# JoelTankard/web-rwkv-gguf

Hardware: AMD Instinct MI355X
Metric: tokens/sec RWKV-7 1.5B Q4_K_M decode @1 GPU; achieved HBM GB/s vs roofline (higher is better)
Workload: dtype f16; 1 GPU; RWKV-7 World 1.5B Q4_K_M (Q4_K matrices, Q6_K head, F16 LoRA) batch=1 greedy decode, fused kernels under hipGraph; decode_engine=on, streams_per_gpu=1, pipelines_per_gpu=1, streams=1, parallelism=single

## Files before the change

web-rwkv-gguf_amd/csrc/wrk_dmv.hip:

```cpp
#include <cstdlib>

#include "wrk_dmv_body.h"

namespace wrk {

template <int KA, int KB, int XI, int KS>
static dmv_fn pick_dmv_pro(bool r16, int pro) {
#define DMV_P(PRO_) (r16 ? (dmv_fn)dmv_kernel<KA, KB, true, XI, KS, PRO_, 1> : (dmv_fn)dmv_kernel<KA, KB, false, XI, KS, PRO_, 1>)
    if (KS == 4 || pro == 0) return DMV_P(0);
    if (pro == 1) return DMV_P(1);
    if (pro == 2) return DMV_P(2);
    if (KA != KB) return nullptr;
    return pro == 3 ? DMV_P(3) : DMV_P(4);
#undef DMV_P
}

template <int XI, int KS>
static dmv_fn pick_dmv_kind(int ka, bool has_f16, bool r16, int pro) {
#define DMV_K(A)                                                                              \
    if (ka == A) return (has_f16 && KS == 1) ? pick_dmv_pro<A, WRK_MAT_F16, XI, KS>(r16, pro) : pick_dmv_pro<A, A, XI, KS>(r16, pro);
    DMV_K(WRK_MAT_Q4_K)
    DMV_K(WRK_MAT_Q5_K)
    DMV_K(WRK_MAT_Q6_K)
    DMV_K(WRK_MAT_Q8_0)
    DMV_K(WRK_MAT_INT8)
#undef DMV_K
    if (ka == WRK_MAT_F16) return pick_dmv_pro<WRK_MAT_F16, WRK_MAT_F16, XI, KS>(false, pro);
    return nullptr;
}

dmvt_fn pick_dmv_nt2(int ka, int quant2, bool has_f16, bool f16_only, uint32_t xi, int ks, int pro);
dmvt_fn pick_dmv_nt4(int ka, int quant2, bool has_f16, bool f16_only, uint32_t xi, int ks, int pro);
dmvt_fn pick_dmv_tokens(int nt, int ka, int quant2, bool has_f16, bool f16_only, uint32_t xi, int ks, int pro) {
    if (nt == 2) return pick_dmv_nt2(ka, quant2, has_f16, f16_only, xi, ks, pro);
    if (nt == 4) return pick_dmv_nt4(ka, quant2, has_f16, f16_only, xi, ks, pro);
    return nullptr;
}

int launch_dmv(hipStream_t s, const MatvecParams& P, uint32_t total_wg, int quant, bool has_f16, bool r16, bool dry, int quant2) {
    static const bool enabled = [] { const char* e = getenv("WRK_DMV"); return !(e && e[0] == '0'); }();
    if (!enabled) return -1;
    DParams D;
    DParamsT DT;
    uint32_t bounds[7], bmask = 0, xi = 1;
    int pro = -1;
    bool small_wg = true;
    for (int j = 0; j < 7; ++j) bounds[j] = 0xffffffffu;
    auto dense_base = [](const DTensor& t) { return ((size_t)t.offset[2] * t.stride[1] + t.offset[1]) * t.stride[0] + t.offset[0]; };
    auto dense_stack = [](const DTensor& t) { return t.shape[2] == 1 || (t.shape[1] == t.stride[1] && t.offset[1] == 0); };
    const uint32_t ntok = P.jobs[0].in.shape[1] * P.jobs[0].in.shape[2];
    if (ntok == 0 || ntok > 4) return -1;
    const int nt = ntok == 1 ? 1 : (ntok <= 2 ? 2 : 4);
    static const uint32_t max_tok = [] { const char* e = getenv("WRK_DMV_TOKENS"); const int v = e ? atoi(e) : 4; return (uint32_t)(v < 1 ? 1 : v); }();
    if (ntok > max_tok) return -1;
    if (nt > 1 && r16) return -1;
    for (int j = 0; j < P.njobs; ++j) {
        const JobDev& J = P.jobs[j];
        if (J.in.dtype != WRK_F16 || (J.k & 7u) || J.in.shape[1] * J.in.shape[2] != ntok || J.kind == WRK_MAT_NF4) return -1;
        if (nt > 1) {
            if (!dense_stack(J.in) || !dense_stack(J.out) || (J.has_res && !dense_stack(J.res)) || (J.in.stride[0] & 7u)) return -1;
            if (J.kind != WRK_MAT_F16 && J.kind != WRK_MAT_Q4_K && J.kind != WRK_MAT_Q5_K && J.kind != WRK_MAT_Q6_K) return -1;
        }
        if ((J.out.dtype != WRK_F16 && J.out.dtype != WRK_F32) || J.m == 0 || J.rows_per_wg == 0) return -1;
        const size_t ib = dense_base(J.in);
        if (ib & 7u) return -1;
        const int jp = J.pro ? (J.k <= 2048 ? 1 : (J.k <= 4096 ? 2 : 9)) + (J.pro == 2 ? 2 : 0) : 0;
        if (jp >= 9 || (pro >= 0 && jp != pro)) return -1;
        if (J.pro == 2 && (J.k & 63u)) return -1;
        pro = jp;
        if (J.rows_per_wg > 32) small_wg = false;
        const uint32_t kpad = (J.k + 15u) & ~15u;
        uint32_t nch, need;
        if (J.kind == WRK_MAT_F16) { nch = kpad >> 3; need = quant < 0 ? (nch + 63) / 64 : (nch + 255) / 256; bmask |= (quant < 0 ? 0u : 1u << j); }
        else { nch = (J.kind == WRK_MAT_Q8_0 || J.kind == WRK_MAT_INT8) ? (J.k >> 4) : (J.k >> 8) * 8; need = (nch + 63) / 64; }
        xi = need > xi ? need : xi;
        const size_t esz = J.out.dtype == WRK_F32 ? 4 : 2;
        if (J.has_res && J.res.dtype != WRK_F16 && J.res.dtype != WRK_F32) return -1;
        auto fill = [&](auto& d) {
            memset(&d, 0, sizeof d);
            d.w = J.w;
            d.x = (const f16*)J.in.p + ib;
            d.out = (char*)J.out.p + dense_base(J.out) * esz;
            d.flags = J.out.dtype == WRK_F32 ? DJ_OUT32 : 0u;
            if (J.has_res) {
                d.res = (const char*)J.res.p + dense_base(J.res) * (J.res.dtype == WRK_F32 ? 4 : 2);
                d.flags |= DJ_RES | (J.res.dtype == WRK_F32 ? DJ_RES32 : 0u);
            }
            if (J.carry_dst) { d.carry_src = J.carry_src; d.carry_dst = J.carry_dst; d.flags |= DJ_CARRY; }
            if (J.gate) { d.gate = J.gate; d.flags |= DJ_GATE; }
            if (J.amax_val) { d.amax_val = J.amax_val; d.amax_idx = J.amax_idx; d.flags |= DJ_AMAX; }
            if (J.pro) { d.ln_w = J.ln_w; d.ln_b = J.ln_b; d.mixw = J.mixw; d.prev = J.prev; d.ln_out = J.ln_out; d.eps = J.pro_eps; if (J.ln_out) d.flags |= DJ_PUBLISH; }
            d.dbg = J.dbg;
            d.k = J.k; d.m = J.m; d.row_bytes = J.row_bytes; d.rows_per_wg = J.rows_per_wg; d.wg_begin = J.wg_begin; d.act = J.act; d.kind = J.kind;
            d.scale = J.scale;
        };
        if (nt == 1) fill(D.jobs[j]);
        else {
            DJobT& dt = DT.jobs[j];
            fill(dt);
            dt.ntok = ntok; dt.xs = J.in.stride[0]; dt.os = J.out.stride[0]; dt.rs = J.has_res ? J.res.stride[0] : 0;
            dt.mix_s = J.tok_mix_stride; dt.prev_s = J.tok_prev_stride; dt.csrc_s = J.tok_carry_src_stride; dt.cdst_s = J.tok_carry_dst_stride; dt.gate_s = J.tok_gate_stride;
        }
        if (j > 0) bounds[j - 1] = J.wg_begin;
    }
    if (xi > 8) return -1;
    static const size_t max_bytes = [] { const char* e = getenv("WRK_DMV_MAXMB"); return (size_t)(e ? atoi(e) : 24) << 20; }();
    size_t launch_bytes = 0;
    for (int j = 0; j < P.njobs; ++j) launch_bytes += (size_t)P.jobs[j].m * P.jobs[j].row_bytes;
    if (nt == 1 && launch_bytes > max_bytes && xi > 1 && pro != 3 && pro != 4) return -1;
    dmv_fn fn = nullptr;
    const int ka = quant < 0 ? WRK_MAT_F16 : quant;
    const bool mixf = has_f16 && quant >= 0;
    if (nt > 1) {
        int ks = 1;
        uint32_t xk = xi;
        if (quant2 < 0 && !(quant < 0 && xi <= 4) && xi > 2) {
            bool amax = false;
            for (int j = 0; j < P.njobs; ++j) amax = amax || P.jobs[j].amax_val;
            if (mixf || !small_wg || pro != 0 || amax || xi > 8) return -1;
            ks = 4; xk = xi <= 4 ? 1 : 2;
        }
        const dmvt_fn ft = pick_dmv_tokens(nt, ka, quant2, mixf, quant < 0, xk, ks, pro);
        if (!ft) return -1;
        if (!dry) hipLaunchKernelGGL(ft, dim3(total_wg, 1), dim3(256), 0, s, bounds[0], bounds[1], bounds[2], bounds[3], bounds[4], bounds[5], bounds[6], bmask, DT);
        return 0;
    }
    else if (quant2 >= 0) {
        const int k4 = quant == WRK_MAT_Q6_K ? quant2 : quant;
        const int lnpro = xi == 1 ? 1 : 2;
        if ((quant != WRK_MAT_Q6_K && quant2 != WRK_MAT_Q6_K) || (k4 != WRK_MAT_Q4_K && k4 != WRK_MAT_Q5_K) || xi > 2 || (pro != 0 && pro != lnpro)) return -1;
#define DMV3X(A, X, PR) (r16 ? (dmv_fn)dmv3_kernel<A, true, X, PR, 1> : (dmv_fn)dmv3_kernel<A, false, X, PR, 1>)
#define DMV3(A) (xi == 1 ? (pro ? DMV3X(A, 1, 1) : DMV3X(A, 1, 0)) : (pro ? DMV3X(A, 2, 2) : DMV3X(A, 2, 0)))
        fn = k4 == WRK_MAT_Q4_K ? DMV3(WRK_MAT_Q4_K) : DMV3(WRK_MAT_Q5_K);
#undef DMV3
#undef DMV3X
    }
    else if (xi == 1) fn = pick_dmv_kind<1, 1>(ka, mixf, r16, pro);
    else if (xi == 2) fn = pick_dmv_kind<2, 1>(ka, mixf, r16, pro);
    else if (quant < 0 && xi <= 4) fn = pick_dmv_kind<4, 1>(ka, false, false, pro);
    else if (!mixf && small_wg && pro == 0) fn = xi <= 4 ? pick_dmv_kind<1, 4>(ka, false, r16, 0) : pick_dmv_kind<2, 4>(ka, false, r16, 0);
    if (!fn) return -1;
    if (!dry) hipLaunchKernelGGL(fn, dim3(total_wg, 1), dim3(256), 0, s, bounds[0], bounds[1], bounds[2], bounds[3], bounds[4], bounds[5], bounds[6], bmask, D);
    return 0;
}

}
```

web-rwkv-gguf_amd/csrc/wrk_dmv_body.h:

```cpp
#pragma once
#include "wrk_matvec_dev.h"

namespace wrk {

enum { DJ_RES = 1, DJ_RES32 = 2, DJ_CARRY = 4, DJ_GATE = 8, DJ_AMAX = 16, DJ_OUT32 = 32, DJ_PUBLISH = 64 };

#define WRK_DJOB_FIELDS                                                                                                          \
    const uint8_t* w;                                                                                                            \
    const f16* x;                                                                    \
    void* out;                                                       \
    const void* res;                                         \
    const f16* carry_src;                                \
    float* carry_dst;                                                                                                            \
    const f16* gate;                                                                       \
    const f16 *ln_w, *ln_b, *mixw;         \
    const float* prev;                                                                                 \
    f16* ln_out;                                      \
    float* amax_val;                                                                             \
    uint32_t* amax_idx;                                                                                                          \
    unsigned long long* dbg;                                                                                                     \
    uint32_t k, m, row_bytes, rows_per_wg, wg_begin, act, flags, kind;                                                           \
    float scale, eps;
struct DJob {
    WRK_DJOB_FIELDS
};
struct DJobT {
    WRK_DJOB_FIELDS
    uint32_t ntok, xs, os, rs, mix_s, prev_s, csrc_s, cdst_s, gate_s;
};

struct DParams {
    DJob jobs[MAX_JOBS];
};
struct DParamsT {
    DJobT jobs[MAX_JOBS];
};
template <int NT> struct DParamsOf { typedef DParamsT type; };
template <> struct DParamsOf<1> { typedef DParams type; };

template <class JT> struct TokF {
    static __device__ __forceinline__ uint32_t ntok(const JT&) { return 1u; }
    static __device__ __forceinline__ uint32_t xs(const JT&) { return 0u; }
    static __device__ __forceinline__ uint32_t os(const JT&) { return 0u; }
    static __device__ __forceinline__ uint32_t rs(const JT&) { return 0u; }
    static __device__ __forceinline__ uint32_t mix_s(const JT&) { return 0u; }
    static __device__ __forceinline__ uint32_t prev_s(const JT&) { return 0u; }
    static __device__ __forceinline__ uint32_t csrc_s(const JT&) { return 0u; }
    static __device__ __forceinline__ uint32_t cdst_s(const JT&) { return 0u; }
    static __device__ __forceinline__ uint32_t gate_s(const JT&) { return 0u; }
};
template <> struct TokF<DJobT> {
    static __device__ __forceinline__ uint32_t ntok(const DJobT& j) { return j.ntok; }
    static __device__ __forceinline__ uint32_t xs(const DJobT& j) { return j.xs; }
    static __device__ __forceinline__ uint32_t os(const DJobT& j) { return j.os; }
    static __device__ __forceinline__ uint32_t rs(const DJobT& j) { return j.rs; }
    static __device__ __forceinline__ uint32_t mix_s(const DJobT& j) { return j.mix_s; }
    static __device__ __forceinline__ uint32_t prev_s(const DJobT& j) { return j.prev_s; }
    static __device__ __forceinline__ uint32_t csrc_s(const DJobT& j) { return j.csrc_s; }
    static __device__ __forceinline__ uint32_t cdst_s(const DJobT& j) { return j.cdst_s; }
    static __device__ __forceinline__ uint32_t gate_s(const DJobT& j) { return j.gate_s; }
};

template <int KIND, bool R16, int NT, int XI>
__device__ __forceinline__ void dot_raw_tokens(const Raw& r, uint32_t c, const XRegs (&x)[NT][XI], int ci, float (&acc)[NT]) {
    if (KIND == WRK_MAT_F16) {
        const f16x8 wv = __builtin_bit_cast(f16x8, r.w);
#pragma unroll
        for (int t = 0; t < NT; ++t) {
            const f16x8 xv = x[t][ci].v[0];
            float a = 0.0f;
            a = __builtin_amdgcn_fdot2(__builtin_shufflevector(wv, wv, 0, 1), __builtin_shufflevector(xv, xv, 0, 1), a, false);
            a = __builtin_amdgcn_fdot2(__builtin_shufflevector(wv, wv, 2, 3), __builtin_shufflevector(xv, xv, 2, 3), a, false);
            a = __builtin_amdgcn_fdot2(__builtin_shufflevector(wv, wv, 4, 5), __builtin_shufflevector(xv, xv, 4, 5), a, false);
            a = __builtin_amdgcn_fdot2(__builtin_shufflevector(wv, wv, 6, 7), __builtin_shufflevector(xv, xv, 6, 7), a, false);
            acc[t] += a;
        }
        return;
    }
    constexpr bool TWO = KIND != WRK_MAT_Q8_0 && KIND != WRK_MAT_INT8;
    Group lo, hi;
    decode_raw<KIND>(r, c, lo, hi);
    if (R16) { round_group(lo); if (TWO) round_group(hi); }
#pragma unroll
    for (int t = 0; t < NT; ++t) {
        const XRegs& X = x[t][ci];
        float a;
        if (R16) a = dot16r(lo.q, X.v[0], X.v[1]);
        else a = lo.scale * (lo.qmul * dot16r(lo.q, X.v[0], X.v[1]) - lo.off * X.s[0]) - lo.minv * X.s[0];
        if (TWO) {
            if (R16) a += dot16r(hi.q, X.v[2], X.v[3]);
            else a += hi.scale * (hi.qmul * dot16r(hi.q, X.v[2], X.v[3]) - hi.off * X.s[1]) - hi.minv * X.s[1];
        }
        acc[t] += a;
    }
}

template <int KIND, bool R16, int XI, int KS, int PRO, int NT, class JT>
__device__ __forceinline__ void dmv_body(const JT J, unsigned char* smem) {
    typedef TokF<JT> TF;
    constexpr int RB = 4;
    constexpr uint32_t CSTEP = KS == 1 ? 64u : 256u;
    const uint32_t K = J.k, kpad = (K + 15u) & ~15u;
    const uint32_t tid = threadIdx.x, lane = tid & 63;
    const uint32_t wave = (uint32_t)__builtin_amdgcn_readfirstlane((int)(tid >> 6));
    const uint32_t r0 = (blockIdx.x - J.wg_begin) * J.rows_per_wg;
    const uint32_t r1 = min(r0 + J.rows_per_wg, J.m);
    const uint32_t nch = num_chunks<KIND>(K, kpad);
    const uint32_t nrows = KS == 1 ? (r0 + wave < r1 ? (r1 - r0 - wave + 3) >> 2 : 0) : (r1 - r0);
    const uint32_t cbase = KS == 1 ? lane : lane + 64 * wave;
    const uint32_t ntok = NT == 1 ? 1u : TF::ntok(J);
    auto row_of = [&](uint32_t ri) { return KS == 1 ? r0 + wave + 4 * ri : r0 + ri; };
    auto tok_of = [&](uint32_t t) { return NT == 1 ? 0u : min(t, ntok - 1); };
    const uint8_t* __restrict__ W = J.w;
    const uint32_t RBY = J.row_bytes;
    float* part = (float*)smem;
    float* sv = (float*)(smem + 512 * NT);
    uint32_t* si = (uint32_t*)(smem + 528 * NT);
    float* red = (float*)(smem + 544 * NT);
    f16* xs = (f16*)(smem + 576 * NT);

    Raw raw[RB][XI];
    auto issue = [&](uint32_t ri0) {
#pragma unroll
        for (int rb = 0; rb < RB; ++rb) {
            const uint32_t rr = min(row_of(ri0 + rb), r1 - 1);
            const uint32_t phase = KIND == WRK_MAT_INT8 ? (uint32_t)((((size_t)rr * K) >> 4) & 7u) : 0u;
            const uint8_t* rowp = W + (size_t)rr * RBY;
#pragma unroll
            for (int ci = 0; ci < XI; ++ci) raw[rb][ci] = load_raw<KIND>(rowp, K, min(cbase + CSTEP * ci, nch - 1), phase);
        }
    };
    WRK_STAMP(J.dbg, 0);

    const f16* __restrict__ xin = J.x;
    const uint32_t fin_row = min(KS == 1 ? row_of(lane & 3u) : r0 + (tid & 31u), r1 - 1);
    const uint32_t fin_t = NT == 1 ? 0u : (KS == 1 ? (lane >> 2) : (tid >> 5));
    const uint32_t fin_tok = tok_of(fin_t);
    const uint32_t fl = J.flags;
    uint32_t res_bits = 0, carry_bits = 0, gate_bits = 0;
    constexpr int VPT = PRO == 0 ? 1 : ((PRO - 1) % 2 + 1);
    constexpr bool GN = PRO >= 3;
    f16x8 xv[NT][VPT], wv[VPT], bv[VPT], mv[GN ? NT : 1][VPT];
    f32x4 pv[NT][VPT][2];
    f16 c0h[NT];
    XRegs x[NT][XI];
    if (PRO > 0) {
        const uint32_t nvec = K >> 3;
#pragma unroll
        for (int v = 0; v < VPT; ++v) {
            const uint32_t i = min(tid + 256u * v, nvec - 1);
            wv[v] = *(const f16x8*)(J.ln_w + i * 8);
            bv[v] = *(const f16x8*)(J.ln_b + i * 8);
#pragma unroll
            for (int t = 0; t < NT; ++t) {
                const uint32_t tt = tok_of(t);
                xv[t][v] = *(const f16x8*)(xin + (size_t)tt * TF::xs(J) + i * 8);
                if (GN || t == 0) mv[GN ? t : 0][v] = *(const f16x8*)(J.mixw + (size_t)tt * TF::mix_s(J) + i * 8);
                pv[t][v][0] = *(const f32x4*)(J.prev + (size_t)tt * TF::prev_s(J) + i * 8);
                pv[t][v][1] = *(const f32x4*)(J.prev + (size_t)tt * TF::prev_s(J) + i * 8 + 4);
            }
        }
        if (!GN) {
#pragma unroll
            for (int t = 0; t < NT; ++t) c0h[t] = xin[(size_t)tok_of(t) * TF::xs(J)];
        }
    } else {
#pragma unroll
        for (int t = 0; t < NT; ++t)
#pragma unroll
            for (int ci = 0; ci < XI; ++ci) x[t][ci] = load_x<KIND>(xin + (size_t)tok_of(t) * TF::xs(J), min(cbase + CSTEP * ci, nch - 1), true);
    }
    issue(0);
    {
        const bool has_res = (fl & DJ_RES) != 0, has_carry = (fl & DJ_CARRY) != 0, has_gate = (fl & DJ_GATE) != 0;
        const uint16_t* rp = has_res ? (const uint16_t*)J.res : (const uint16_t*)xin;
        const uint32_t re = fin_tok * TF::rs(J) + fin_row;
        const uint32_t ri = has_res ? ((fl & DJ_RES32) ? 2u * re : re) : 0u;
        if (fl & DJ_RES32) res_bits = *(const uint32_t*)(rp + ri);
        else res_bits = rp[ri];
        carry_bits = (has_carry ? (const uint16_t*)J.carry_src : (const uint16_t*)xin)[has_carry ? fin_tok * TF::csrc_s(J) + fin_row : 0u];
        gate_bits = (has_gate ? (const uint16_t*)J.gate : (const uint16_t*)xin)[has_gate ? fin_tok * TF::gate_s(J) + fin_row : 0u];
    }

    if (GN) {
        const uint32_t nvec = K >> 3;
#pragma unroll
        for (int t = 0; t < NT; ++t)
#pragma unroll
            for (int v = 0; v < VPT; ++v) {
                float y[8], s1 = 0.0f;
#pragma unroll
                for (int e = 0; e < 8; ++e) { y[e] = (float)xv[t][v][e]; s1 += y[e]; }
                s1 += dpp_f32<0xB1>(s1); s1 += dpp_f32<0x4E>(s1); s1 += dpp_f32<0x141>(s1);
                const float mean = s1 * (1.0f / 64.0f);
                float s2 = 0.0f;
#pragma unroll
                for (int e = 0; e < 8; ++e) { y[e] -= mean; s2 = __builtin_fmaf(y[e], y[e], s2); }
                s2 += dpp_f32<0xB1>(s2); s2 += dpp_f32<0x4E>(s2); s2 += dpp_f32<0x141>(s2);
                const float dev = 1.0f / sqrtf(s2 * (1.0f / 64.0f) + J.eps);
                f16x8 o;
#pragma unroll
                for (int e = 0; e < 8; ++e) {
                    float u = r16(__builtin_fmaf(y[e] * dev, (float)wv[v][e], (float)bv[v][e]));
                    u = r16(u + pv[t][v][e >> 2][e & 3]);
                    o[e] = (f16)((float)mv[GN ? t : 0][v][e] * u);
                }
                const uint32_t i = tid + 256u * v;
                if (i < nvec) *(f16x8*)(xs + (size_t)t * kpad + i * 8) = o;
            }
        for (uint32_t i = K + tid; i < kpad; i += 256)
#pragma unroll
            for (int t = 0; t < NT; ++t) xs[(size_t)t * kpad + i] = (f16)0.0f;
        __syncthreads();
#pragma unroll
        for (int t = 0; t < NT; ++t)
#pragma unroll
            for (int ci = 0; ci < XI; ++ci) x[t][ci] = load_x<KIND>(xs + (size_t)t * kpad, min(cbase + CSTEP * ci, nch - 1), true);
    }
    if (PRO > 0 && !GN) {
        const uint32_t nvec = K >> 3;
        float s1[NT], s2[NT];
#pragma unroll
        for (int t = 0; t < NT; ++t) {
            const float c0 = (float)c0h[t];
            s1[t] = 0.0f; s2[t] = 0.0f;
#pragma unroll
            for (int v = 0; v < VPT; ++v)
                if (tid + 256u * v < nvec)
#pragma unroll
                    for (int e = 0; e < 8; ++e) { const float dl = (float)xv[t][v][e] - c0; s1[t] += dl; s2[t] = __builtin_fmaf(dl, dl, s2[t]); }
            s1[t] = wave_sum(s1[t]);
            s2[t] = wave_sum(s2[t]);
            if (lane == 0) { red[8 * t + wave] = s1[t]; red[8 * t + 4 + wave] = s2[t]; }
        }
        __syncthreads();
        WRK_STAMP(J.dbg, 4);
        const bool publish = (fl & DJ_PUBLISH) && blockIdx.x == J.wg_begin;
#pragma unroll
        for (int t = 0; t < NT; ++t) {
            const float c0 = (float)c0h[t];
            const float a1 = (red[8 * t + 0] + red[8 * t + 1]) + (red[8 * t + 2] + red[8 * t + 3]);
            const float a2 = (red[8 * t + 4] + red[8 * t + 5]) + (red[8 * t + 6] + red[8 * t + 7]);
            const float md = a1 / (float)K;
            const float mean = c0 + md;
            const float dev = 1.0f / sqrtf(fmaxf(a2 / (float)K - md * md, 0.0f) + J.eps);
#pragma unroll
            for (int v = 0; v < VPT; ++v) {
                const uint32_t i = tid + 256u * v;
                if (i >= nvec) continue;
                f16x8 yv, o;
#pragma unroll
                for (int e = 0; e < 8; ++e) {
                    yv[e] = (f16)__builtin_fmaf(((float)xv[t][v][e] - mean) * dev, (float)wv[v][e], (float)bv[v][e]);
                    o[e] = (f16)wgsl_mix((float)yv[e], pv[t][v][e >> 2][e & 3], (float)mv[0][v][e]);
                }
                *(f16x8*)(xs + (size_t)t * kpad + i * 8) = o;
                if (publish && (uint32_t)t < ntok) *(f16x8*)(J.ln_out + (size_t)t * K + i * 8) = yv;
            }
        }
        for (uint32_t i = K + tid; i < kpad; i += 256)
#pragma unroll
            for (int t = 0; t < NT; ++t) xs[(size_t)t * kpad + i] = (f16)0.0f;
        __syncthreads();
#pragma unroll
        for (int t = 0; t < NT; ++t)
#pragma unroll
            for (int ci = 0; ci < XI; ++ci) x[t][ci] = load_x<KIND>(xs + (size_t)t * kpad, min(cbase + CSTEP * ci, nch - 1), true);
    }
#pragma unroll
    for (int ci = 0; ci < XI; ++ci)
        if (cbase + CSTEP * ci >= nch) {
            const f16x8 z = {0, 0, 0, 0, 0, 0, 0, 0};
#pragma unroll
            for (int t = 0; t < NT; ++t) x[t][ci].v[0] = x[t][ci].v[1] = x[t][ci].v[2] = x[t][ci].v[3] = z;
        }
#pragma unroll
    for (int t = 0; t < NT; ++t)
#pragma unroll
        for (int ci = 0; ci < XI; ++ci) x_sums<KIND>(x[t][ci]);
    WRK_STAMP(J.dbg, 1);

    float best_v = -3.0e38f;
    uint32_t best_i = 0xffffffffu;
    auto finish = [&](uint32_t r, uint32_t tok, float v, uint32_t rbits, uint32_t cbits, uint32_t gbits) {
        float o = act_apply(J.act, v * J.scale);
        const bool o32 = (fl & DJ_OUT32) != 0;
        if (fl & DJ_GATE) o = act_sigmoid(f16bits_to_f32(gbits)) * (o32 ? o : r16(o));
        if (fl & DJ_RES) o = (o32 ? o : r16(o)) + ((fl & DJ_RES32) ? __builtin_bit_cast(float, rbits) : f16bits_to_f32(rbits));
        const size_t oo = (size_t)tok * TF::os(J) + r;
        if (o32) ((float*)J.out)[oo] = o; else ((f16*)J.out)[oo] = (f16)o;
        if (fl & DJ_CARRY) J.carry_dst[(size_t)tok * TF::cdst_s(J) + r] = f16bits_to_f32(cbits);
        if (o > best_v || (o == best_v && r < best_i)) { best_v = o; best_i = r; }
    };
    auto operand_bits = [&](uint32_t r, uint32_t tok, uint32_t& rbits, uint32_t& cbits, uint32_t& gbits) {
        if (fl & DJ_RES) rbits = (fl & DJ_RES32) ? ((const uint32_t*)J.res)[(size_t)tok * TF::rs(J) + r] : (uint32_t)((const uint16_t*)J.res)[(size_t)tok * TF::rs(J) + r];
        if (fl & DJ_CARRY) cbits = ((const uint16_t*)J.carry_src)[(size_t)tok * TF::csrc_s(J) + r];
        if (fl & DJ_GATE) gbits = ((const uint16_t*)J.gate)[(size_t)tok * TF::gate_s(J) + r];
    };
    for (uint32_t ri0 = 0; ri0 < nrows; ri0 += RB) {
        if (ri0 != 0) issue(ri0);
        float acc[RB][NT];
#pragma unroll
        for (int rb = 0; rb < RB; ++rb) {
#pragma unroll
            for (int t = 0; t < NT; ++t) acc[rb][t] = 0.0f;
#pragma unroll
            for (int ci = 0; ci < XI; ++ci) dot_raw_tokens<KIND, R16, NT, XI>(raw[rb][ci], min(cbase + CSTEP * ci, nch - 1), x, ci, acc[rb]);
        }
        WRK_STAMP(J.dbg, 2);
        float mine_v = 0.0f;
#pragma unroll
        for (int t = 0; t < NT; ++t)
#pragma unroll
            for (int rb = 0; rb < RB; ++rb) {
                const float v = wave_sum(acc[rb][t]);
                if (lane == (uint32_t)(rb + RB * t)) mine_v = v;
            }
        const uint32_t frb = lane & 3u;
        if (KS == 1) {
            if (lane < (uint32_t)(RB * NT) && (NT == 1 || fin_t < ntok) && ri0 + frb < nrows) {
                const uint32_t r = row_of(ri0 + frb);
                uint32_t rbits = res_bits, cbits = carry_bits, gbits = gate_bits;
                if (ri0 != 0) operand_bits(r, fin_t, rbits, cbits, gbits);
                finish(r, fin_t, mine_v, rbits, cbits, gbits);
            }
        } else if (lane < (uint32_t)(RB * NT) && ri0 + frb < nrows) part[(((NT == 1 ? 0u : lane >> 2) * 32u) + ri0 + frb) * 4 + wave] = mine_v;
    }
    if (KS == 4) {
        __syncthreads();
        const uint32_t ri = tid & 31u;
        if (NT == 1 ? tid < nrows : (ri < nrows && fin_t < ntok)) {
            const uint32_t p = NT == 1 ? tid : (fin_t * 32u + ri);
            finish(r0 + ri, fin_t, (part[p * 4] + part[p * 4 + 1]) + (part[p * 4 + 2] + part[p * 4 + 3]), res_bits, carry_bits, gate_bits);
        }
    }
    WRK_STAMP(J.dbg, 3);
    if (fl & DJ_AMAX) {
#pragma unroll
        for (int o = (KS == 1 ? 2 : 32); o > 0; o >>= 1) {
            const float ov = __shfl_xor(best_v, o, WAVE);
            const uint32_t oi = __shfl_xor(best_i, o, WAVE);
            if (ov > best_v || (ov == best_v && oi < best_i)) { best_v = ov; best_i = oi; }
        }
        if (KS == 1 ? ((lane & 3u) == 0 && lane < 4u * NT) : lane == 0) { sv[4 * (KS == 1 ? lane >> 2 : 0) + wave] = best_v; si[4 * (KS == 1 ? lane >> 2 : 0) + wave] = best_i; }
        __syncthreads();
        if (tid < ntok) {
            float bv2 = sv[4 * tid];
            uint32_t bi = si[4 * tid];
            for (int w = 1; w < 4; ++w)
                if (sv[4 * tid + w] > bv2 || (sv[4 * tid + w] == bv2 && si[4 * tid + w] < bi)) { bv2 = sv[4 * tid + w]; bi = si[4 * tid + w]; }
            J.amax_val[(size_t)(blockIdx.x - J.wg_begin) * ntok + tid] = bv2;
            J.amax_idx[(size_t)(blockIdx.x - J.wg_begin) * ntok + tid] = bi;
        }
    }
}

template <int PRO, int NT>
constexpr unsigned dmv_smem_bytes() { return 576u * NT + (PRO > 0 ? (unsigned)((PRO - 1) % 2 + 1) * 4096u * NT : 16u); }

template <int KA, int KB, bool R16, int XI, int KS, int PRO, int NT>
__global__ void __launch_bounds__(256) dmv_kernel(uint32_t b1, uint32_t b2, uint32_t b3, uint32_t b4, uint32_t b5, uint32_t b6, uint32_t b7,
                                                  uint32_t kind_b_mask, const typename DParamsOf<NT>::type P) {
    __shared__ __attribute__((aligned(16))) unsigned char smem[dmv_smem_bytes<PRO, NT>()];
    const uint32_t b = blockIdx.x;
    const uint32_t ji = (b >= b1) + (b >= b2) + (b >= b3) + (b >= b4) + (b >= b5) + (b >= b6) + (b >= b7);
    const auto J = P.jobs[ji];
    if (KA == KB || !((kind_b_mask >> ji) & 1u)) dmv_body<KA, (KA != WRK_MAT_F16) && R16, XI, KS, PRO, NT>(J, smem);
    else dmv_body<KB, (KB != WRK_MAT_F16) && R16, (KB == WRK_MAT_F16 ? 4 * XI : XI), 1, PRO, NT>(J, smem);
}

template <int KA, bool R16, int XI, int PRO, int NT>
__global__ void __launch_bounds__(256) dmv3_kernel(uint32_t b1, uint32_t b2, uint32_t b3, uint32_t b4, uint32_t b5, uint32_t b6, uint32_t b7,
                                                   uint32_t, const typename DParamsOf<NT>::type P) {
    __shared__ __attribute__((aligned(16))) unsigned char smem[dmv_smem_bytes<PRO, NT>()];
    const uint32_t b = blockIdx.x;
    const uint32_t ji = (b >= b1) + (b >= b2) + (b >= b3) + (b >= b4) + (b >= b5) + (b >= b6) + (b >= b7);
    const auto J = P.jobs[ji];
    if (J.kind == (uint32_t)KA) dmv_body<KA, R16, XI, 1, PRO, NT>(J, smem);
    else if (J.kind == WRK_MAT_Q6_K) dmv_body<WRK_MAT_Q6_K, R16, XI, 1, PRO, NT>(J, smem);
    else dmv_body<WRK_MAT_F16, false, 4 * XI, 1, PRO, NT>(J, smem);
}

typedef void (*dmv_fn)(uint32_t, uint32_t, uint32_t, uint32_t, uint32_t, uint32_t, uint32_t, uint32_t, const DParams);
typedef void (*dmvt_fn)(uint32_t, uint32_t, uint32_t, uint32_t, uint32_t, uint32_t, uint32_t, uint32_t, const DParamsT);

dmvt_fn pick_dmv_tokens(int nt, int ka, int quant2, bool has_f16, bool f16_only, uint32_t xi, int ks, int pro);

}
```

web-rwkv-gguf_amd/csrc/wrk_internal.h:

```cpp
#pragma once
#include <hip/hip_runtime.h>

#include <atomic>
#include <cmath>
#include <cstdarg>
#include <cstdio>
#include <cstring>
#include <map>
#include <mutex>
#include <string>
#include <thread>
#include <vector>

#include "wrk_hip.h"

struct wrk_ctx {
    int device = 0;
    hipStream_t stream = nullptr;
    hipStream_t read_stream = nullptr;
    hipEvent_t read_event = nullptr;
    std::recursive_mutex mu;
    std::string err;
    std::map<std::thread::id, hipStream_t> sessions;
    std::vector<hipStream_t> capture_pool;
// ... 125 lines not shown
void group_norm(hipStream_t s, const void* w, const void* b, DTensor x, float eps);
void l2_norm(hipStream_t s, DTensor x, float eps);
void token_shift(hipStream_t s, const uint32_t* cursors, DTensor mix, DTensor state, DTensor in, DTensor out, int reversed);
void pre_wkv_v7(hipStream_t s, void* w, void* a, void* k, void* v, void* vv, void* v0, void* n, const void* w0, const void* a0, const void* k_k,
                const void* k_a, const void* v0p, uint32_t D, uint32_t T, bool first_layer, float l2_eps, float* wdec = nullptr);
void post_wkv_v7(hipStream_t s, void* x, const void* r, const void* g, const void* n, const void* gn_w, const void* gn_b, const void* r_k,
                 uint32_t D, uint32_t T, float gn_eps);
void token_shift_multi(hipStream_t s, const uint32_t* cursors, const DTensor* mix, const DTensor* out, int n, DTensor state, DTensor in, int reversed);
void transpose(hipStream_t s, DTensor in, DTensor out);
void time_mix_v6(hipStream_t s, const uint32_t* cursors, DTensor decay, const void* u_f32, DTensor state, DTensor k, DTensor v, DTensor r, DTensor x,
                 uint32_t nseq_hint = 0);
void channel_mix_v6(hipStream_t s, const uint32_t* cursors, DTensor state, DTensor r, DTensor v, DTensor x);
void binary(hipStream_t s, int is_mul, DTensor in, DTensor out, uint32_t ax, uint32_t ay, uint32_t ao);
void lerp(hipStream_t s, DTensor x, DTensor y, DTensor f, int reversed);
void blit(hipStream_t s, DTensor in, DTensor out);
void affine(hipStream_t s, DTensor x, float scale, float bias);
void activate(hipStream_t s, DTensor x, uint32_t act);
void control_k_v7(hipStream_t s, const void* p, DTensor a, DTensor k);
void time_mix_v7(hipStream_t s, const uint32_t* cursors, DTensor state, DTensor r, DTensor w, DTensor n, DTensor x, uint32_t nseq_hint = 0, const float* wdec = nullptr);
void time_first_v7(hipStream_t s, const void* u, DTensor r, DTensor n, DTensor x);
void channel_mix_v7(hipStream_t s, const uint32_t* cursors, DTensor state, DTensor v, DTensor x);
void softmax(hipStream_t s, DTensor x);
void gather_rows_f16(hipStream_t s, const void* table, const uint32_t* ids, void* out, uint32_t d, uint32_t n);
void gather_rows_any(hipStream_t s, DTensor in, const uint32_t* rows, DTensor out, uint32_t n);
void argmax_rows(hipStream_t s, const float* logits, uint32_t v, uint32_t v_stride, uint32_t n, uint32_t* out);

struct SampleParam { float temperature, top_p; uint32_t seed, step_base; };
static constexpr uint32_t SAMPLE_MAX_VOCAB = 1u << 20;
struct RowGate { const uint32_t* flag; uint32_t stride, eq; };
struct SampleFilter { uint32_t top_k; float ln_min_p; };
struct SampleAlt { float tau, eta, mu, typical_p; };
enum : int { SAMPLE_PLAIN = 0, SAMPLE_FILT = 1, SAMPLE_MIRO = 2, SAMPLE_TYP = 3 };
struct SamplePick { int mode; const SampleParam* par; const SampleFilter* filt; SampleAlt* alt; RowGate gate; };
int sample_rows(hipStream_t s, const float* logits, uint32_t v, uint32_t stride, uint32_t n, const SamplePick& pick, const uint32_t* step,
                uint32_t* out);

struct ScorePart { float m, s; uint32_t gt, eq; };
static constexpr uint32_t SCORE_MAX_SLICES = 32;
uint32_t score_slices(uint32_t n, uint32_t v, int num_cu);
int score_rows(hipStream_t s, const float* logits, uint32_t v, uint32_t stride, uint32_t n, const uint32_t* targets, ScorePart* part,
               float* logprob, uint32_t* rank, int num_cu);

static constexpr uint32_t LOGPROB_MAX_TOP = WRK_MAX_TOP_LOGPROBS;
struct LogprobParam { float* logprob; uint32_t* top_ids; float* top_logprobs; uint32_t num_top, cap_rows; };
struct LogprobPart { float m, s; };
inline size_t logprob_part_bytes(uint32_t n) { return (size_t)n * SCORE_MAX_SLICES * sizeof(LogprobPart); }
inline size_t logprob_key_bytes(uint32_t n) { return (size_t)n * SCORE_MAX_SLICES * 4 * LOGPROB_MAX_TOP * 8; }
int logprob_rows(hipStream_t s, const float* logits, uint32_t v, uint32_t stride, uint32_t n, const uint32_t* tokens, const uint32_t* step,
                 const LogprobParam* par, LogprobPart* part, unsigned long long* keys, int num_cu);

struct PenaltyParam { float* count; uint8_t* flags; const float* weight; float presence, frequency, decay; uint32_t pad; };
void penalize_rows(hipStream_t s, const float* src, uint32_t v, uint32_t src_stride, uint32_t n, const PenaltyParam* par, float* dst,
                   uint32_t dst_stride);
void occurrence_update(hipStream_t s, uint32_t v, uint32_t n, const PenaltyParam* par, const uint32_t* tokens, uint32_t ntok, const RowGate& gate);

struct GrammarParam { const uint16_t* token_class; const uint16_t* transitions; uint32_t num_classes, pad; uint32_t* states; };
void constrain_rows(hipStream_t s, const float* src, uint32_t v, uint32_t src_stride, uint32_t n, const GrammarParam* par, float* dst,
                    uint32_t dst_stride);
void grammar_advance(hipStream_t s, uint32_t v, uint32_t n, const GrammarParam* par, const uint32_t* tokens, const RowGate& gate);

struct StopParam { uint32_t ids[WRK_MAX_STOP_TOKENS]; uint32_t count, done, length, end_token; };
struct StopGeom {
    float *state, *head_o, *snap_state, *snap_logits;
    const uint32_t* just_ended; const StopParam* par; const uint32_t* counter; uint32_t* lengths;
    uint32_t layers, num_batch, b0, v;
    size_t slot;
};
void advance_stop(hipStream_t s, const uint32_t* drawn, uint32_t* tokens, uint32_t* history, uint32_t* counter, StopParam* par,
                  uint32_t* just_ended, uint32_t* live, uint32_t b);
void stop_snapshot(hipStream_t s, const StopGeom& g, uint32_t b, int num_cu);
void stop_restore(hipStream_t s, const StopGeom& g, uint32_t b, int num_cu);

struct StopSeqRow { uint32_t count, pad[3]; uint32_t len[WRK_MAX_STOP_SEQUENCES]; uint32_t tok[WRK_MAX_STOP_SEQUENCES][WRK_MAX_STOP_SEQUENCE_LEN]; };
struct StopSeqBufs { const StopSeqRow* rows; uint32_t* tail; uint32_t* match; };
void advance_stop_seq(hipStream_t s, const uint32_t* drawn, uint32_t* tokens, uint32_t* history, uint32_t* counter, StopParam* par,
                      uint32_t* just_ended, uint32_t* live, const StopSeqBufs& q, uint32_t b);
void stop_seq_rows(hipStream_t s, uint32_t n, const StopSeqRow* rows, const StopParam* ids, uint32_t* tail, const uint32_t* tokens, uint32_t* match);

enum : uint32_t { QUEUE_IDLE = 0, QUEUE_PROMPT = 1, QUEUE_REPLY = 2 };
struct QueueReq {
    uint32_t prompt_off, prompt_len, max_new, seed;
    float temperature, top_p, presence, frequency, decay;
    uint32_t stop_count, stop_ids[WRK_MAX_STOP_TOKENS];
    uint32_t top_k; float ln_min_p;
    float tau, eta, typical_p;
};
struct QueueSlot { uint32_t req, pos, reply, phase; };
struct QueueLog { uint32_t length, reason, slot, start_step; };
struct QueueCtl { uint32_t next_request, num_requests, live, pad; const float* init_state; };
struct QueueBufs {
    QueueSlot* slots; const QueueReq* reqs; const uint32_t* pool; QueueLog* log; QueueCtl* ctl;
    uint32_t* started;
    SampleParam* sample_par;
    PenaltyParam* pen_par;
    SampleFilter* filter_par;
    SampleAlt* alt_par = nullptr;
    float* alt_mu = nullptr;
    uint32_t* gram_state = nullptr;
    uint32_t* gram_req = nullptr;
    const StopSeqRow* seq_rows = nullptr;
    uint32_t* seq_tail = nullptr;
    uint32_t* seq_match = nullptr;
};
void advance_queue(hipStream_t s, const uint32_t* drawn, uint32_t* tokens, uint32_t* history, uint32_t* counter, const QueueBufs& q, uint32_t b);
struct QueueGeom { float* state; uint32_t layers, num_batch, b0, v; size_t slot; };
void queue_reset(hipStream_t s, const QueueGeom& g, const QueueBufs& q, uint32_t b, int num_cu);
static constexpr uint32_t QUEUE_NO_ENTRY = 0xFFFFFFFFu;
struct QueueStateCtl { float* states; uint32_t num_entries, turn_count; };
struct QueueTurn { uint32_t slot, save, started, start; };
struct QueueStateBufs {
    const uint32_t *start, *save;
    QueueStateCtl* sctl;
    QueueTurn* turn;
};
void advance_queue_pool(hipStream_t s, const uint32_t* drawn, uint32_t* tokens, uint32_t* history, uint32_t* counter, const QueueBufs& q,
                        const QueueStateBufs& p, uint32_t b);
void queue_turnover(hipStream_t s, const QueueGeom& g, const QueueBufs& q, const QueueStateBufs& p, uint32_t b, int num_cu);

unsigned long long* timing_slot(wrk_ctx* ctx, const char* label);
void timing_report(wrk_ctx* ctx);

struct MatJob {
    const uint8_t* w;
    const uint8_t* aux;
    uint32_t kind, flags;
    uint32_t k, m;
    uint32_t row_bytes;
    DTensor in;
    DTensor out;
    uint32_t act;
    uint32_t sparse;
    uint32_t has_res = 0;
    DTensor res{};
    float* amax_val = nullptr;
    uint32_t* amax_idx = nullptr;
    uint32_t pro = 0;
    float pro_eps = 0.0f;
    const void *ln_w = nullptr, *ln_b = nullptr, *mixw = nullptr;
    const float* prev = nullptr;
    void* ln_out = nullptr;
    const void* carry_src = nullptr;
    float* carry_dst = nullptr;
    float scale = 1.0f;
    const void* gate = nullptr;
    unsigned long long* dbg = nullptr;
    uint32_t tok_prev_stride = 0, tok_mix_stride = 0, tok_carry_src_stride = 0, tok_carry_dst_stride = 0, tok_gate_stride = 0;
    float* ks_part = nullptr;
    uint32_t* ks_cnt = nullptr;
    size_t ks_part_cap = 0;
    uint32_t ks_cnt_cap = 0;
    void* xsum = nullptr;
    size_t xsum_cap = 0;
};
uint32_t matvec_num_wg(const MatJob* jobs, int njobs, int num_cu, uint32_t* rows_per_wg);
int matvec(hipStream_t s, const MatJob* jobs, int njobs, int num_cu, bool dry_run = false, bool no_catchall = false, bool dmv_only = false);
int matvec_grouped(hipStream_t s, const MatJob* jobs, int njobs, int num_cu, bool dry_run = false);
int matmul_mfma(hipStream_t s, const MatJob& job, int num_cu);
int matmul_mfma_multi(hipStream_t s, const MatJob* jobs, int njobs, int num_cu);
uint32_t gemm_min_tokens();
void quantize_int8(hipStream_t s, const void* src_f16, uint8_t* dst, uint32_t k, uint32_t m, uint32_t row_bytes);
void quantize_nf4(hipStream_t s, const void* src_f16, const float* levels, uint8_t* dst, uint32_t k, uint32_t m, uint32_t row_bytes);
size_t repack_row_bytes(uint32_t kind, uint32_t k);
uint32_t int8_row_blocks(uint32_t k);
int repack_rows(uint32_t kind, uint32_t k, uint32_t m, const uint8_t* src, uint8_t* dst);
size_t stored_bytes(uint32_t kind, uint32_t k, uint32_t m);

}

int32_t wrk_sample_pack(wrk_ctx* ctx, const float* temperature, const float* top_p, const uint32_t* seed, uint32_t n,
                        std::vector<wrk::SampleParam>& out);
int32_t wrk_filter_pack(wrk_ctx* ctx, const uint32_t* top_k, const float* min_p, uint32_t n, std::vector<wrk::SampleFilter>& out);
int32_t wrk_mirostat_pack(wrk_ctx* ctx, const float* tau, const float* eta, const float* mu, uint32_t n, std::vector<wrk::SampleAlt>& out);
int32_t wrk_typical_pack(wrk_ctx* ctx, const float* typical_p, uint32_t n, std::vector<wrk::SampleAlt>& out);

struct wrk_score_scratch {
    void* buf = nullptr;
    uint32_t cap = 0;
    uint32_t* targets = nullptr;
    float* logprob = nullptr;
    uint32_t* rank = nullptr;
    wrk::ScorePart* part = nullptr;
    int32_t ensure(wrk_ctx* ctx, uint32_t n, bool* grown);
    void release();
};
int32_t wrk_score_check_targets(wrk_ctx* ctx, const uint32_t* targets, uint32_t n, uint32_t V);

struct wrk_occurrence {
    wrk_ctx* ctx = nullptr;
    uint32_t num_batch = 0, num_vocab = 0;
    void* mem = nullptr;
    float* counts = nullptr;
    float* weights = nullptr;
    uint8_t* flags = nullptr;
    wrk::PenaltyParam row(uint32_t slot, float presence, float frequency, float decay) const;
};
int32_t wrk_penalty_pack(wrk_ctx* ctx, const wrk_occurrence* occ, uint32_t first, uint32_t n, uint32_t V, const float* presence,
                         const float* frequency, const float* decay, std::vector<wrk::PenaltyParam>& out);

struct wrk_grammar {
    wrk_ctx* ctx = nullptr;
    uint32_t num_vocab = 0, num_states = 0, num_classes = 0;
    void* mem = nullptr;
    uint16_t* token_class = nullptr;
    uint16_t* transitions = nullptr;
    wrk::GrammarParam param(uint32_t* states) const;
};
int32_t wrk_grammar_pack(wrk_ctx* ctx, const wrk_grammar* g, const uint32_t* state, uint32_t n, uint32_t V, std::vector<uint32_t>& out);
```

web-rwkv-gguf_amd/csrc/wrk_matvec.hip:

```cpp
#include <algorithm>
#include <cstdlib>

#include "wrk_matvec_dev.h"

namespace wrk {

static inline size_t align16(size_t x) { return (x + 15) & ~(size_t)15; }

uint32_t int8_row_blocks(uint32_t k) { return (k % 128) ? k / 128 + 2 : k / 128; }

size_t repack_row_bytes(uint32_t kind, uint32_t k) {
    const size_t nb = k / 256;
    switch (kind) {
        case WRK_MAT_F16: return align16((size_t)k * 2);
        case WRK_MAT_Q8_0: return align16((size_t)k + (size_t)(k / 32) * 2);
        case WRK_MAT_Q4_K: return align16(nb * 148);
        case WRK_MAT_Q5_K: return align16(nb * 180);
        case WRK_MAT_Q6_K: return align16(nb * 208 + nb * 2);
        case WRK_MAT_INT8: return (k % 16) ? 0 : align16((size_t)k + (size_t)int8_row_blocks(k) * 4);
        case WRK_MAT_NF4: return (k % 64) ? 0 : align16((size_t)k / 2 + (size_t)(k / 64) * 2);
        default: return 0;
    }
}

// ... 516 lines not shown

typedef void (*matvec_fn)(const MatvecParams);

template <int NB, int KA, int KB>
static matvec_fn pick_r16(bool r16) {
    return r16 ? (matvec_fn)matvec_kernel<NB, KA, KB, true> : (matvec_fn)matvec_kernel<NB, KA, KB, false>;
}

template <int NB>
static matvec_fn pick_kernel(int ka, int kb, bool r16) {
#define PAIR(A)                                                                     \
    if (ka == A) return kb == A ? pick_r16<NB, A, A>(r16) : pick_r16<NB, A, WRK_MAT_F16>(r16);
    PAIR(WRK_MAT_Q4_K)
    PAIR(WRK_MAT_Q5_K)
    PAIR(WRK_MAT_Q6_K)
    PAIR(WRK_MAT_Q8_0)
#undef PAIR
    if (ka == WRK_MAT_NF4) return kb == ka ? (matvec_fn)matvec_kernel<NB, WRK_MAT_NF4, WRK_MAT_NF4, false> : (matvec_fn)matvec_kernel<NB, WRK_MAT_NF4, WRK_MAT_F16, false>;
    if (ka == WRK_MAT_INT8) return kb == ka ? (matvec_fn)matvec_kernel<NB, WRK_MAT_INT8, WRK_MAT_INT8, false> : (matvec_fn)matvec_kernel<NB, WRK_MAT_INT8, WRK_MAT_F16, false>;
    if (ka == WRK_MAT_F16) return pick_r16<NB, WRK_MAT_F16, WRK_MAT_F16>(false);
    return (matvec_fn)matvec_kernel<NB, -1, -1, false>;
}

template <int KA, int KB, int XI, int KS>
static matvec_fn pick_reg_r16(bool r16) {
    return r16 ? (matvec_fn)matvec_reg_kernel<KA, KB, true, XI, KS> : (matvec_fn)matvec_reg_kernel<KA, KB, false, XI, KS>;
}

template <int XI, int KS>
static matvec_fn pick_reg_kernel(int ka, int kb, bool r16) {
#define PAIR(A)                                                                     \
    if (ka == A) return (kb == A || KS == 4) ? pick_reg_r16<A, A, XI, KS>(r16) : pick_reg_r16<A, WRK_MAT_F16, XI, 1>(r16);
    PAIR(WRK_MAT_Q4_K)
    PAIR(WRK_MAT_Q5_K)
    PAIR(WRK_MAT_Q6_K)
    PAIR(WRK_MAT_Q8_0)
    PAIR(WRK_MAT_INT8)
#undef PAIR
    return nullptr;
}

static matvec_fn pick_reg(const MatvecParams& P, int quant, bool has_f16, bool r16, int quant2 = -1) {
    uint32_t xi = 1;
    for (int j = 0; j < P.njobs; ++j) {
        const JobDev& J = P.jobs[j];
        if (J.in.dtype != WRK_F16 || (J.k & 7u) || J.in.shape[1] * J.in.shape[2] != 1) return nullptr;
        if (J.pro && J.k > 4096) return nullptr;
        if (J.pro == 2) return nullptr;
        const size_t base = ((size_t)J.in.offset[2] * J.in.stride[1] + J.in.offset[1]) * J.in.stride[0] + J.in.offset[0];
        if (base & 7u) return nullptr;
        const uint32_t kpad = (J.k + 15u) & ~15u;
        uint32_t nch, need;
        if (J.kind == WRK_MAT_F16) { nch = kpad >> 3; need = quant < 0 ? (nch + 63) / 64 : (nch + 255) / 256; }
        else if (J.kind == WRK_MAT_NF4) return nullptr;
        else { nch = (J.kind == WRK_MAT_Q8_0 || J.kind == WRK_MAT_INT8) ? (J.k >> 4) : (J.k >> 8) * 8; need = (nch + 63) / 64; }
        xi = need > xi ? need : xi;
    }
    if (xi > 8) return nullptr;
    bool small_wg = true;
    for (int j = 0; j < P.njobs; ++j) if (P.jobs[j].rows_per_wg > 32) small_wg = false;
    if (quant < 0) {
        if (xi == 1) return (matvec_fn)matvec_reg_kernel<WRK_MAT_F16, WRK_MAT_F16, false, 1, 1>;
        if (xi == 2) return (matvec_fn)matvec_reg_kernel<WRK_MAT_F16, WRK_MAT_F16, false, 2, 1>;
        if (xi <= 4) return (matvec_fn)matvec_reg_kernel<WRK_MAT_F16, WRK_MAT_F16, false, 4, 1>;
        return small_wg ? (matvec_fn)matvec_reg_kernel<WRK_MAT_F16, WRK_MAT_F16, false, 2, 4> : nullptr;
    }
    if (quant2 >= 0) {
        const int ka = quant == WRK_MAT_Q6_K ? quant2 : quant;
        if ((quant != WRK_MAT_Q6_K && quant2 != WRK_MAT_Q6_K) || (ka != WRK_MAT_Q4_K && ka != WRK_MAT_Q5_K) || xi > 2) return nullptr;
        if (ka == WRK_MAT_Q4_K) {
            if (xi == 1) return r16 ? (matvec_fn)matvec_reg3_kernel<WRK_MAT_Q4_K, true, 1> : (matvec_fn)matvec_reg3_kernel<WRK_MAT_Q4_K, false, 1>;
            return r16 ? (matvec_fn)matvec_reg3_kernel<WRK_MAT_Q4_K, true, 2> : (matvec_fn)matvec_reg3_kernel<WRK_MAT_Q4_K, false, 2>;
        }
        if (xi == 1) return r16 ? (matvec_fn)matvec_reg3_kernel<WRK_MAT_Q5_K, true, 1> : (matvec_fn)matvec_reg3_kernel<WRK_MAT_Q5_K, false, 1>;
        return r16 ? (matvec_fn)matvec_reg3_kernel<WRK_MAT_Q5_K, true, 2> : (matvec_fn)matvec_reg3_kernel<WRK_MAT_Q5_K, false, 2>;
    }
    const int kb = has_f16 ? WRK_MAT_F16 : quant;
    if (xi == 1) return pick_reg_kernel<1, 1>(quant, kb, r16);
    if (xi == 2) return pick_reg_kernel<2, 1>(quant, kb, r16);
    if (has_f16 || !small_wg) return nullptr;
    if (xi <= 4) return pick_reg_kernel<1, 4>(quant, quant, r16);
    return pick_reg_kernel<2, 4>(quant, quant, r16);
}

struct KindMix { int quant = -1, quant2 = -1, nquant = 0; bool has_f16 = false, r16 = false, mixed_r16 = false; };
static KindMix classify_kinds(const MatvecParams& P) {
    KindMix c;
    for (int j = 0; j < P.njobs; ++j) {
        const int k = (int)P.jobs[j].kind;
        if (k == WRK_MAT_F16) { c.has_f16 = true; continue; }
        const bool jr = (P.jobs[j].flags & WRK_MATRIX_ROUND_F16) != 0;
        if (c.nquant == 0) { c.quant = k; c.r16 = jr; c.nquant = 1; }
        else {
            if (k != c.quant && k != c.quant2) { c.quant2 = c.quant2 < 0 ? k : c.quant2; c.nquant = (k == c.quant2) ? 2 : 3; }
            if (jr != c.r16) c.mixed_r16 = true;
        }
    }
    return c;
}

template <int NB>
static int launch_matvec(hipStream_t s, const MatvecParams& P, uint32_t total_wg, uint32_t tok_groups, size_t smem, bool dry, bool no_catchall) {
    const KindMix c = classify_kinds(P);
    const int quant = c.quant, quant2 = c.quant2, nquant = c.nquant;
    const bool has_f16 = c.has_f16, r16 = c.r16, mixed_r16 = c.mixed_r16;
    matvec_fn fn = nullptr;
    bool needs_reg = false;
    for (int j = 0; j < P.njobs; ++j) needs_reg = needs_reg || P.jobs[j].pro || P.jobs[j].carry_dst || P.jobs[j].gate;
    if (NB == 1 && tok_groups == 1 && nquant <= 2 && !mixed_r16 && launch_dmv(s, P, total_wg, nquant ? quant : -1, has_f16, r16, dry, nquant == 2 ? quant2 : -1) == 0) return 0;
    if (NB == 1 && tok_groups == 1 && nquant <= 2 && !mixed_r16) {
        fn = pick_reg(P, nquant ? quant : -1, has_f16, r16, nquant == 2 ? quant2 : -1);
        if (fn) {
            if (!dry) hipLaunchKernelGGL(fn, dim3(total_wg, 1), dim3(256), 0, s, P);
            return 0;
        }
    }
    if (needs_reg) return -3;
    if (no_catchall && (nquant >= 2 || mixed_r16)) return -4;
    if (dry) return 0;
    if (nquant >= 2 || mixed_r16) fn = (matvec_fn)matvec_kernel<NB, -1, -1, false>;
    else if (nquant == 0) fn = pick_kernel<NB>(WRK_MAT_F16, WRK_MAT_F16, false);
    else fn = pick_kernel<NB>(quant, has_f16 ? WRK_MAT_F16 : quant, r16);
    if (smem > 64 * 1024) {
        if (hipFuncSetAttribute((const void*)fn, hipFuncAttributeMaxDynamicSharedMemorySize, (int)smem) != hipSuccess) return -1;
    }
    hipLaunchKernelGGL(fn, dim3(total_wg, tok_groups), dim3(256), smem, s, P);
    return 0;
}

static uint32_t matvec_job_rpw(const MatJob* jobs, int njobs, int j, uint32_t rpw) {
    uint32_t min_rb = jobs[0].row_bytes;
    for (int q = 1; q < njobs; ++q) min_rb = jobs[q].row_bytes < min_rb ? jobs[q].row_bytes : min_rb;
    uint32_t r = (uint32_t)((uint64_t)rpw * min_rb / (jobs[j].row_bytes ? jobs[j].row_bytes : 1)) & ~3u;
    return r < 4 ? 4 : r;
}

uint32_t matvec_num_wg(const MatJob* jobs, int njobs, int num_cu, uint32_t* rows_per_wg) {
    uint32_t total_rows = 0;
    for (int j = 0; j < njobs; ++j) total_rows += jobs[j].m;
    static const uint32_t per_cu = [] { const char* e = getenv("WRK_WG_PER_CU"); const int v = e ? atoi(e) : 4; return (uint32_t)(v < 1 ? 1 : (v > 16 ? 16 : v)); }();
    uint32_t rpw = (total_rows + (uint32_t)num_cu * per_cu - 1) / ((uint32_t)num_cu * per_cu);
    rpw = (rpw + 3) & ~3u;
    static const uint32_t rpw_min = [] { const char* e = getenv("WRK_RPW_MIN"); const int v = e ? atoi(e) : 4; return (uint32_t)(v < 4 ? 4 : (v > 32 ? 32 : v)) & ~3u; }();
    rpw = rpw < rpw_min ? rpw_min : (rpw > 32 ? 32 : rpw);
    static const uint32_t pro_rpw = [] { const char* e = getenv("WRK_PRO_RPW"); const int v = e ? atoi(e) : 16; return (uint32_t)(v < 4 ? 4 : (v > 32 ? 32 : v)) & ~3u; }();
    for (int j = 0; j < njobs; ++j)
        if (jobs[j].pro && rpw < pro_rpw) rpw = pro_rpw;
    uint32_t wg = 0;
    for (int j = 0; j < njobs; ++j) { const uint32_t r = matvec_job_rpw(jobs, njobs, j, rpw); wg += (jobs[j].m + r - 1) / r; }
    if (rows_per_wg) *rows_per_wg = rpw;
    return wg;
}

int matvec(hipStream_t s, const MatJob* jobs, int njobs, int num_cu, bool dry_run, bool no_catchall, bool dmv_only) {
    if (njobs <= 0 || njobs > MAX_JOBS) return -1;
    MatvecParams P;
    P.njobs = njobs;
    const uint32_t ntok = jobs[0].in.shape[1] * jobs[0].in.shape[2];
    if (ntok == 0) return 0;
    uint32_t kmax = 0;
    for (int j = 0; j < njobs; ++j) {
        if (jobs[j].in.shape[1] * jobs[j].in.shape[2] != ntok) return -1;
        kmax = jobs[j].k > kmax ? jobs[j].k : kmax;
    }
    uint32_t rpw = 4;
    matvec_num_wg(jobs, njobs, num_cu, &rpw);
    uint32_t wg = 0;
    for (int j = 0; j < njobs; ++j) {
        JobDev& d = P.jobs[j];
        d.w = jobs[j].w; d.aux = (const float*)jobs[j].aux; d.kind = jobs[j].kind; d.flags = jobs[j].flags; d.k = jobs[j].k; d.m = jobs[j].m;
        d.row_bytes = jobs[j].row_bytes; d.act = jobs[j].act; d.rows_per_wg = matvec_job_rpw(jobs, njobs, j, rpw); d.wg_begin = wg;
        d.in = jobs[j].in; d.out = jobs[j].out; d.res = jobs[j].res; d.has_res = jobs[j].has_res;
        d.amax_val = jobs[j].amax_val; d.amax_idx = jobs[j].amax_idx;
        d.pro = jobs[j].pro; d.pro_eps = jobs[j].pro_eps; d.ln_w = (const f16*)jobs[j].ln_w; d.ln_b = (const f16*)jobs[j].ln_b;
        d.mixw = (const f16*)jobs[j].mixw; d.prev = jobs[j].prev; d.ln_out = (f16*)jobs[j].ln_out;
        d.carry_src = (const f16*)jobs[j].carry_src; d.carry_dst = jobs[j].carry_dst; d.gate = (const f16*)jobs[j].gate; d.scale = jobs[j].scale; d.dbg = jobs[j].dbg;
        d.tok_prev_stride = jobs[j].tok_prev_stride; d.tok_mix_stride = jobs[j].tok_mix_stride; d.tok_carry_src_stride = jobs[j].tok_carry_src_stride;
        d.tok_carry_dst_stride = jobs[j].tok_carry_dst_stride; d.tok_gate_stride = jobs[j].tok_gate_stride;
        wg += (jobs[j].m + d.rows_per_wg - 1) / d.rows_per_wg;
    }
    bool f32in = false;
    for (int j = 0; j < njobs; ++j) f32in = f32in || jobs[j].in.dtype == WRK_F32;
    if (f32in) {
        for (int j = 0; j < njobs; ++j)
            if (jobs[j].pro || jobs[j].carry_dst || jobs[j].gate || jobs[j].amax_val) return -3;
        if (dry_run) return 0;
        hipLaunchKernelGGL(matvec_f32in_kernel, dim3(wg, ntok), dim3(256), 0, s, P);
        return 0;
    }
    if (ntok >= 2 && ntok <= 4) {
        const KindMix c = classify_kinds(P);
        if (c.nquant <= 2 && !c.mixed_r16 && launch_dmv(s, P, wg, c.nquant ? c.quant : -1, c.has_f16, c.r16, dry_run, c.nquant == 2 ? c.quant2 : -1) == 0) return 0;
    }
    if (dmv_only && ntok > 1) return -5;
    const uint32_t kpad = (kmax + 15u) & ~15u;
    int nb = ntok >= 8 ? 8 : (ntok >= 4 ? 4 : (ntok >= 2 ? 2 : 1));
    while (nb > 1 && (size_t)nb * kpad * 2 + (size_t)nb * (kpad >> 4) * 4 > 144 * 1024) nb >>= 1;
    size_t smem = (size_t)nb * kpad * 2 + (size_t)nb * (kpad >> 4) * 4 + 64;
    if (smem < 256) smem = 256;
    const uint32_t groups = (ntok + nb - 1) / nb;
    int rc;
    switch (nb) {
        case 8: rc = launch_matvec<8>(s, P, wg, groups, smem, dry_run, no_catchall); break;
        case 4: rc = launch_matvec<4>(s, P, wg, groups, smem, dry_run, no_catchall); break;
        case 2: rc = launch_matvec<2>(s, P, wg, groups, smem, dry_run, no_catchall); break;
        default: rc = launch_matvec<1>(s, P, wg, groups, smem, dry_run, no_catchall); break;
    }
    return rc;
}

int matvec_grouped(hipStream_t s, const MatJob* jobs, int njobs, int num_cu, bool dry_run) {
    if (njobs <= 0 || njobs > MAX_JOBS) return -1;
    uint32_t kinds[MAX_JOBS];
    int nk = 0;
    for (int j = 0; j < njobs; ++j) {
        if (jobs[j].kind == WRK_MAT_F16) continue;
        bool seen = false;
        for (int q = 0; q < nk; ++q) seen = seen || kinds[q] == jobs[j].kind;
        if (!seen) kinds[nk++] = jobs[j].kind;
    }
    if (nk <= 1) return matvec(s, jobs, njobs, num_cu, dry_run);
    {
        const int rc = matvec(s, jobs, njobs, num_cu, dry_run, true);
        if (rc == 0) return 0;
    }
    for (int q = 0; q < nk; ++q) {
        MatJob g[MAX_JOBS];
        int n = 0;
        for (int j = 0; j < njobs; ++j)
            if (jobs[j].kind == kinds[q] || (q == 0 && jobs[j].kind == WRK_MAT_F16)) g[n++] = jobs[j];
        const int rc = matvec(s, g, n, num_cu, dry_run);
        if (rc != 0) return rc;
    }
    return 0;
}

}
```

web-rwkv-gguf_amd/csrc/wrk_matvec_dev.h:

```cpp
#pragma once
#include "wrk_device.h"

namespace wrk {

__device__ __forceinline__ void bytes_to_h2(uint32_t v, f16x2& lo, f16x2& hi) {
    lo = __builtin_bit_cast(f16x2, __builtin_amdgcn_perm(0u, v, 0x0c010c00u));
    hi = __builtin_bit_cast(f16x2, __builtin_amdgcn_perm(0u, v, 0x0c030c02u));
}

__device__ __forceinline__ f16x2 h2(float a) { f16x2 r = {(f16)a, (f16)a}; return r; }

__device__ __forceinline__ float dot16(const f16x2 (&q)[8], const f16* __restrict__ x) {
    const f16x8 xa = *(const f16x8*)x;
    const f16x8 xb = *(const f16x8*)(x + 8);
    float acc = 0.0f;
    acc = __builtin_amdgcn_fdot2(q[0], __builtin_shufflevector(xa, xa, 0, 1), acc, false);
    acc = __builtin_amdgcn_fdot2(q[1], __builtin_shufflevector(xa, xa, 2, 3), acc, false);
    acc = __builtin_amdgcn_fdot2(q[2], __builtin_shufflevector(xa, xa, 4, 5), acc, false);
    acc = __builtin_amdgcn_fdot2(q[3], __builtin_shufflevector(xa, xa, 6, 7), acc, false);
    acc = __builtin_amdgcn_fdot2(q[4], __builtin_shufflevector(xb, xb, 0, 1), acc, false);
    acc = __builtin_amdgcn_fdot2(q[5], __builtin_shufflevector(xb, xb, 2, 3), acc, false);
    acc = __builtin_amdgcn_fdot2(q[6], __builtin_shufflevector(xb, xb, 4, 5), acc, false);
    acc = __builtin_amdgcn_fdot2(q[7], __builtin_shufflevector(xb, xb, 6, 7), acc, false);
    return acc;
// ... 175 lines not shown
        const uint32_t s0 = 2 * j, s1 = 2 * j + 1;
        const uint32_t r0 = (s0 + 28u) & 31u, r1 = (s1 + 28u) & 31u;
#define Q5LO(W, H) (((W) & 0x0f0f0f0fu) | (__builtin_amdgcn_alignbit((H), (H), r0) & 0x10101010u))
#define Q5HI(W, H) ((((W) >> 4) & 0x0f0f0f0fu) | (__builtin_amdgcn_alignbit((H), (H), r1) & 0x10101010u))
        bytes_to_h2(Q5LO(w.x, qh.x), lo.q[0], lo.q[1]);
        bytes_to_h2(Q5LO(w.y, qh.y), lo.q[2], lo.q[3]);
        bytes_to_h2(Q5LO(w.z, qh.z), lo.q[4], lo.q[5]);
        bytes_to_h2(Q5LO(w.w, qh.w), lo.q[6], lo.q[7]);
        bytes_to_h2(Q5HI(w.x, qh.x), hi.q[0], hi.q[1]);
        bytes_to_h2(Q5HI(w.y, qh.y), hi.q[2], hi.q[3]);
        bytes_to_h2(Q5HI(w.z, qh.z), hi.q[4], hi.q[5]);
        bytes_to_h2(Q5HI(w.w, qh.w), hi.q[6], hi.q[7]);
#undef Q5LO
#undef Q5HI
        hi.qmul = Q24;
    }
    lo.scale = d * sc0; lo.minv = dmin * m0; lo.off = 0.0f; lo.qmul = Q24; lo.xoff = b * 256 + j * 64 + h * 16;
    hi.scale = d * sc1; hi.minv = dmin * m1; hi.off = 0.0f; hi.xoff = lo.xoff + 32;
}

template <int KIND>
__device__ __forceinline__ void chunk_xoff(uint32_t c, uint32_t& lo, uint32_t& hi) {
    if (KIND == WRK_MAT_F16) { lo = c * 8; hi = lo; return; }
    if (KIND == WRK_MAT_Q8_0 || KIND == WRK_MAT_INT8) { lo = c * 16; hi = lo; return; }
    if (KIND == WRK_MAT_NF4) { lo = c * 32; hi = lo + 16; return; }
    const uint32_t b = c >> 3, sub = c & 7u;
    if (KIND == WRK_MAT_Q6_K) { lo = b * 256 + (sub >> 2) * 128 + ((sub >> 1) & 1u) * 32 + (sub & 1u) * 16; hi = lo + 64; return; }
    lo = b * 256 + (sub >> 1) * 64 + (sub & 1u) * 16;
    hi = lo + 32;
}

template <int KIND, bool R16, int NB>
__device__ __forceinline__ void dot_raw(const Raw& r, uint32_t c, const f16* xs, const float* xsum, uint32_t kpad, float (&acc)[NB],
                                        const float* __restrict__ levels = nullptr) {
    if (KIND == WRK_MAT_F16) {
        const f16x8 wv = __builtin_bit_cast(f16x8, r.w);
#pragma unroll
        for (int n = 0; n < NB; ++n) {
            const f16x8 x = *(const f16x8*)(xs + (size_t)n * kpad + c * 8);
            float a = acc[n];
            a = __builtin_amdgcn_fdot2(__builtin_shufflevector(wv, wv, 0, 1), __builtin_shufflevector(x, x, 0, 1), a, false);
            a = __builtin_amdgcn_fdot2(__builtin_shufflevector(wv, wv, 2, 3), __builtin_shufflevector(x, x, 2, 3), a, false);
            a = __builtin_amdgcn_fdot2(__builtin_shufflevector(wv, wv, 4, 5), __builtin_shufflevector(x, x, 4, 5), a, false);
            a = __builtin_amdgcn_fdot2(__builtin_shufflevector(wv, wv, 6, 7), __builtin_shufflevector(x, x, 6, 7), a, false);
            acc[n] = a;
        }
        return;
    }
    if (KIND == WRK_MAT_NF4) {
        const float amax = f16bits_to_f32(r.a.x);
        const uint32_t wd[4] = {r.w.x, r.w.y, r.w.z, r.w.w};
#pragma unroll
        for (int wi = 0; wi < 4; ++wi) {
            float wv[8];
#pragma unroll
            for (int i = 0; i < 8; ++i) {
                wv[i] = levels[(wd[wi] >> (4 * i)) & 15u] * amax;
                if (R16) wv[i] = (float)(f16)wv[i];
            }
#pragma unroll
            for (int n = 0; n < NB; ++n) {
                const f16x8 x = *(const f16x8*)(xs + (size_t)n * kpad + c * 32 + wi * 8);
                float a = acc[n];
#pragma unroll
                for (int i = 0; i < 8; ++i) a = fmaf(wv[i], (float)x[i], a);
                acc[n] = a;
            }
        }
        return;
    }
    Group lo, hi;
    decode_raw<KIND>(r, c, lo, hi);
    groups_accumulate<R16, NB>(lo, hi, KIND != WRK_MAT_Q8_0 && KIND != WRK_MAT_INT8, xs, xsum, kpad, acc);
}

struct XRegs {
    f16x8 v[4];
    float s[2];
};

__device__ __forceinline__ float sum8(f16x8 a) {
    const f16x2 one = {(f16)1.0f, (f16)1.0f};
    float s = 0.0f;
    s = __builtin_amdgcn_fdot2(__builtin_shufflevector(a, a, 0, 1), one, s, false);
    s = __builtin_amdgcn_fdot2(__builtin_shufflevector(a, a, 2, 3), one, s, false);
    s = __builtin_amdgcn_fdot2(__builtin_shufflevector(a, a, 4, 5), one, s, false);
    s = __builtin_amdgcn_fdot2(__builtin_shufflevector(a, a, 6, 7), one, s, false);
    return s;
}

template <int KIND>
__device__ __forceinline__ XRegs load_x(const f16* __restrict__ x, uint32_t c, bool valid) {
    XRegs r;
    const f16x8 z = {0, 0, 0, 0, 0, 0, 0, 0};
    r.v[0] = r.v[1] = r.v[2] = r.v[3] = z;
    r.s[0] = r.s[1] = 0.0f;
    if (!valid) return r;
    uint32_t lo, hi;
    chunk_xoff<KIND>(c, lo, hi);
    r.v[0] = *(const f16x8*)(x + lo);
    if (KIND != WRK_MAT_F16) r.v[1] = *(const f16x8*)(x + lo + 8);
    if (KIND != WRK_MAT_F16 && KIND != WRK_MAT_Q8_0 && KIND != WRK_MAT_INT8) { r.v[2] = *(const f16x8*)(x + hi); r.v[3] = *(const f16x8*)(x + hi + 8); }
    return r;
}

template <int KIND>
__device__ __forceinline__ void x_sums(XRegs& r) {
    if (KIND != WRK_MAT_F16) r.s[0] = sum8(r.v[0]) + sum8(r.v[1]);
    if (KIND != WRK_MAT_F16 && KIND != WRK_MAT_Q8_0 && KIND != WRK_MAT_INT8) r.s[1] = sum8(r.v[2]) + sum8(r.v[3]);
}

__device__ __forceinline__ float dot16r(const f16x2 (&q)[8], const f16x8 xa, const f16x8 xb) {
    float acc = 0.0f;
    acc = __builtin_amdgcn_fdot2(q[0], __builtin_shufflevector(xa, xa, 0, 1), acc, false);
    acc = __builtin_amdgcn_fdot2(q[1], __builtin_shufflevector(xa, xa, 2, 3), acc, false);
    acc = __builtin_amdgcn_fdot2(q[2], __builtin_shufflevector(xa, xa, 4, 5), acc, false);
    acc = __builtin_amdgcn_fdot2(q[3], __builtin_shufflevector(xa, xa, 6, 7), acc, false);
    acc = __builtin_amdgcn_fdot2(q[4], __builtin_shufflevector(xb, xb, 0, 1), acc, false);
    acc = __builtin_amdgcn_fdot2(q[5], __builtin_shufflevector(xb, xb, 2, 3), acc, false);
    acc = __builtin_amdgcn_fdot2(q[6], __builtin_shufflevector(xb, xb, 4, 5), acc, false);
    acc = __builtin_amdgcn_fdot2(q[7], __builtin_shufflevector(xb, xb, 6, 7), acc, false);
    return acc;
}

template <bool R16>
__device__ __forceinline__ float group_dot_r(Group& g, const f16x8 xa, const f16x8 xb, float xs16) {
    if (R16) {
        round_group(g);
        return dot16r(g.q, xa, xb);
    }
    return g.scale * (g.qmul * dot16r(g.q, xa, xb) - g.off * xs16) - g.minv * xs16;
}

template <int KIND, bool R16>
__device__ __forceinline__ float dot_raw_reg(const Raw& r, uint32_t c, const XRegs& x) {
    if (KIND == WRK_MAT_F16) {
        const f16x8 wv = __builtin_bit_cast(f16x8, r.w);
        float a = 0.0f;
        a = __builtin_amdgcn_fdot2(__builtin_shufflevector(wv, wv, 0, 1), __builtin_shufflevector(x.v[0], x.v[0], 0, 1), a, false);
        a = __builtin_amdgcn_fdot2(__builtin_shufflevector(wv, wv, 2, 3), __builtin_shufflevector(x.v[0], x.v[0], 2, 3), a, false);
        a = __builtin_amdgcn_fdot2(__builtin_shufflevector(wv, wv, 4, 5), __builtin_shufflevector(x.v[0], x.v[0], 4, 5), a, false);
        a = __builtin_amdgcn_fdot2(__builtin_shufflevector(wv, wv, 6, 7), __builtin_shufflevector(x.v[0], x.v[0], 6, 7), a, false);
        return a;
    }
    Group lo, hi;
    decode_raw<KIND>(r, c, lo, hi);
    float a = group_dot_r<R16>(lo, x.v[0], x.v[1], x.s[0]);
    if (KIND != WRK_MAT_Q8_0 && KIND != WRK_MAT_INT8) a += group_dot_r<R16>(hi, x.v[2], x.v[3], x.s[1]);
    return a;
}


int launch_dmv(hipStream_t s, const MatvecParams& P, uint32_t total_wg, int quant, bool has_f16, bool r16, bool dry, int quant2 = -1);

}
```

web-rwkv-gguf_amd/csrc/wrk_v7.h:

```cpp
#pragma once
#include <string>
#include <vector>

#include "wrk_runner.h"

struct V7Scratch : wrk::FrameIo {
    void *input, *x, *att_x, *att_v0, *rx, *wx, *kx, *vx, *ax, *gx, *r, *w, *k, *v, *a, *g, *o, *kk, *vv, *n;
    void *aux_w, *aux_a, *aux_g, *aux_v, *ffn_x, *ffn_kx, *ffn_k, *ffn_v, *ln_tmp, *head_x;
    float* ks_part; uint32_t* ks_cnt; size_t ks_part_cap; uint32_t ks_cnt_cap;
};

struct wrk_v7_model : wrk_frame_common {
    wrk_v7_model_desc d{};
    std::vector<wrk_v7_layer_desc> layers;
    const wrk_buf *ln0_w = nullptr, *ln0_b = nullptr, *ln_out_w = nullptr, *ln_out_b = nullptr, *emb = nullptr;
    const wrk_matrix* head = nullptr;

    V7Scratch s{};

    float* amax_val = nullptr;
    uint32_t* amax_idx = nullptr;
    size_t amax_cap = 0;

    uint32_t layer_begin = 0, layer_end = 0xffffffffu;
    bool skip_embed = false;
    uint32_t act_dtype = WRK_F16;

    std::vector<wrk_v7_model*> lanes;

    struct wrk_v7_engine* engine = nullptr;
    bool engine_tried = false;
    bool engine_skip_once = false;
    bool engine_blocked = false;
    std::string engine_why;
    int32_t ensure_engine();
    bool engine_on() const;
    Facts facts() const override { return {d.num_vocab, d.num_emb, d.num_layer, emb != nullptr}; }
    wrk::FrameIo& io() override { return s; }
    int32_t ensure_frame(uint32_t B, uint32_t mode) override;
    int32_t enqueue_step(wrk_v7_state* st, uint32_t b0, uint32_t B, uint32_t mode, wrk_step_kind kind) override;
    uint32_t key_bits(uint32_t B, uint32_t mode) const override;
    uint32_t max_lanes() const override { return 255; }
    int32_t lane(uint32_t g, uint32_t groups, wrk_frame_common** out) override;
    void before_loop() override;
    int32_t after_loop(uint32_t groups) override;
    int32_t ensure_scratch(uint32_t T, uint32_t NH);
    int32_t enqueue_ops(wrk_v7_state* st, uint32_t T, uint32_t NH, bool identity_headers, bool merged = false);
    int32_t enqueue_fused_decode(wrk_v7_state* st, uint32_t B, uint32_t NH, bool identity_headers, bool from_tokens,
                                 bool want_argmax, bool advance, uint32_t cursor0_batch, bool contiguous);
    void free_fused();
};

bool split_head_env_on();
bool engine_env_on_public();
```

web-rwkv-gguf_amd/csrc/wrk_v7.hip:

```cpp
#include "wrk_internal.h"
#include "wrk_v7.h"
#include "wrk_v7_engine.h"

#define LOCK(ctx) std::lock_guard<std::recursive_mutex> _lk((ctx)->mu)

static constexpr float LN_EPS = 1.0e-5f;
static constexpr float GN_EPS = 64.0e-5f;
static constexpr float L2_EPS = 1.0e-12f;

using wrk::mat_job;

int32_t wrk_v7_model::ensure_scratch(uint32_t T, uint32_t NH) {
    if (T <= scratch_tokens && NH <= scratch_headers && scratch) return WRK_OK;
    if (ctx->capturing_here()) return wrk_fail(ctx, WRK_E_ARG, "scratch must be sized before capture");
    const uint32_t nt = T > scratch_tokens ? T : scratch_tokens;
    const uint32_t nh = NH > scratch_headers ? NH : scratch_headers;
    WRK_HIP(ctx, hipStreamSynchronize(ctx->stream));
    drop_graphs();
    if (scratch) hipFree(scratch);
    scratch = nullptr;
    const size_t D = d.num_emb, F = d.num_hidden, V = d.num_vocab;
    size_t off = 0;
    auto take = [&](size_t bytes) { size_t o = off; off += wrk_up256(bytes); return o; };
    const size_t esz = act_dtype == WRK_F32 ? 4 : 2;
    const size_t vecT = D * nt * esz;
    size_t o_named[32];
    int ni = 0;
    for (int i = 0; i < 23; ++i) o_named[ni++] = take(vecT);
    const size_t o_n = take(vecT * 4);
    const size_t o_auxw = take((size_t)d.lora_w * nt * esz), o_auxa = take((size_t)d.lora_a * nt * esz);
    const size_t o_auxg = take((size_t)d.lora_g * nt * esz), o_auxv = take((size_t)d.lora_v * nt * esz);
    const size_t o_ffnk = take(F * nt * esz);
    const size_t o_headx = take(D * nh * esz), o_heado = take(V * nh * 4);
    const size_t o_cur = take((size_t)nt * 4), o_tok = take((size_t)nt * 4), o_hdr = take((size_t)nh * 4), o_arg = take((size_t)nh * 4);
    const size_t o_cnt = take(256);
    size_t ks_floats = 0, ks_groups = 0, o_ksp = 0, o_ksc = 0;
    if (nt >= 2 && act_dtype == WRK_F16) {
        const size_t ntp = nt <= 16 ? 16 : (nt <= 32 ? 32 : 64);
        auto tiles = [](size_t m, size_t k) { return ((m + 63) / 64) * (k / 256 ? k / 256 : 1); };
        auto groups = [](size_t m) { return (m + 63) / 64; };
        const size_t lora = tiles(d.lora_w, D) + tiles(d.lora_a, D) + tiles(d.lora_g, D) + tiles(d.lora_v, D);
        const size_t k1 = 3 * tiles(D, D) + lora, k5 = tiles(F, D), k6 = tiles(D, F);
        const size_t most = k1 > k5 ? (k1 > k6 ? k1 : k6) : (k5 > k6 ? k5 : k6);
        ks_floats = most * 64 * ntp;
        ks_groups = 3 * groups(D) + groups(d.lora_w) + groups(d.lora_a) + groups(d.lora_g) + groups(d.lora_v) + groups(F) + 8;
        o_ksp = take(ks_floats * 4);
        o_ksc = take(ks_groups * 4);
    }
    WRK_HIP(ctx, hipMalloc(&scratch, off));
    WRK_HIP(ctx, hipMemsetAsync(scratch, 0, off, ctx->stream));
    if (nt >= 128 && act_dtype == WRK_F16) {
        const size_t widest = std::max<size_t>(3 * D, F);
        const size_t part = (size_t)256 * widest * 4 * 4;
        const int32_t rs = wrk_ctx_reserve_gemm_scratch(ctx, (size_t)nt * (widest / 32) * 4 + 3 * ((size_t)nt * 4 + 256)  + 8 * 1024 + part);
        if (rs != WRK_OK) return rs;
    }
    char* b = (char*)scratch;
    ni = 0;
    s.input = b + o_named[ni++]; s.x = b + o_named[ni++]; s.att_x = b + o_named[ni++]; s.att_v0 = b + o_named[ni++];
    s.rx = b + o_named[ni++]; s.wx = b + o_named[ni++]; s.kx = b + o_named[ni++]; s.vx = b + o_named[ni++];
    s.ax = b + o_named[ni++]; s.gx = b + o_named[ni++];
    s.r = b + o_named[ni++]; s.w = b + o_named[ni++]; s.k = b + o_named[ni++]; s.v = b + o_named[ni++];
    s.a = b + o_named[ni++]; s.g = b + o_named[ni++]; s.o = b + o_named[ni++];
    s.kk = b + o_named[ni++]; s.vv = b + o_named[ni++];
    s.ffn_x = b + o_named[ni++]; s.ffn_kx = b + o_named[ni++]; s.ffn_v = b + o_named[ni++]; s.ln_tmp = b + o_named[ni++];
    s.n = b + o_n;
    s.aux_w = b + o_auxw; s.aux_a = b + o_auxa; s.aux_g = b + o_auxg; s.aux_v = b + o_auxv;
    s.ffn_k = b + o_ffnk;
    s.head_x = b + o_headx; s.head_o = (float*)(b + o_heado);
    s.cursors = (uint32_t*)(b + o_cur); s.tokens = (uint32_t*)(b + o_tok); s.headers = (uint32_t*)(b + o_hdr); s.argmax = (uint32_t*)(b + o_arg);
    s.counter = (uint32_t*)(b + o_cnt);
    s.ks_part = ks_floats ? (float*)(b + o_ksp) : nullptr; s.ks_cnt = ks_floats ? (uint32_t*)(b + o_ksc) : nullptr;
    s.ks_part_cap = ks_floats; s.ks_cnt_cap = (uint32_t)ks_groups;
    scratch_tokens = nt;
    scratch_headers = nh;
    {
        wrk::MatJob hj = mat_job(head, make_dense(s.head_x, WRK_F16, d.num_emb, nh), make_dense(s.head_o, WRK_F32, d.num_vocab, nh), 0);
        const size_t need = (size_t)wrk::matvec_num_wg(&hj, 1, ctx->num_cu, nullptr) * nh;
        if (need > amax_cap) {
            free_fused();
            WRK_HIP(ctx, hipMalloc((void**)&amax_val, need * 4));
            WRK_HIP(ctx, hipMalloc((void**)&amax_idx, need * 4));
            amax_cap = need;
        }
    }
    return WRK_OK;
}

#define MM(...)                                   \
    do {                                          \
        int32_t _r = wrk_mm(ctx, __VA_ARGS__);    \
        if (_r != WRK_OK) return _r;              \
    } while (0)

int32_t wrk_v7_model::enqueue_ops(wrk_v7_state* st, uint32_t T, uint32_t NH, bool identity_headers, bool merged) {
    hipStream_t q = ctx->op_stream();
    const uint32_t D = d.num_emb, F = d.num_hidden, H = d.num_head, S = D / H, V = d.num_vocab;
    const uint32_t AT = act_dtype;
    if (AT != WRK_F16) merged = false;
    auto vec = [&](void* p, uint32_t c = 0) { return make_dense(p, AT, c ? c : D, T); };
    auto heads = [&](void* p) { return make_dense(p, AT, S, H, T); };
    DTensor x = vec(s.x), att_x = vec(s.att_x), v0 = vec(s.att_v0);
    DTensor rx = vec(s.rx), wx = vec(s.wx), kx = vec(s.kx), vx = vec(s.vx), ax = vec(s.ax), gx = vec(s.gx);
    DTensor r = vec(s.r), w = vec(s.w), k = vec(s.k), v = vec(s.v), a = vec(s.a), g = vec(s.g), o = vec(s.o);
    DTensor kk = vec(s.kk), vv = vec(s.vv);
    DTensor ffn_x = vec(s.ffn_x), ffn_kx = vec(s.ffn_kx), ffn_v = vec(s.ffn_v), ffn_k = vec(s.ffn_k, F);
    DTensor aux_w = vec(s.aux_w, d.lora_w), aux_a = vec(s.aux_a, d.lora_a), aux_g = vec(s.aux_g, d.lora_g), aux_v = vec(s.aux_v, d.lora_v);
    DTensor n4 = make_dense(s.n, AT, S, H, T, 4);
    auto nslice = [&](uint32_t i) { DTensor t = make_dense(s.n, AT, D, T, 4); t.shape[2] = 1; t.offset[2] = i; return t; };
    auto bvec = [&](const wrk_buf* b) { return make_dense(b->ptr, WRK_F16, D, 1, 1); };
    const char* mm_env = getenv("WRK_MERGE_MASK");
    const unsigned mask = mm_env ? (unsigned)atoi(mm_env) : 127u;
    const bool wide = merged && S == 64 && T > 0;
    const bool m_shift = merged && (mask & 1u), m_group = merged && (mask & 2u), m_pre = wide && (mask & 4u), m_post = wide && (mask & 8u),
               m_res = merged && (mask & 16u), m_ln = merged && (mask & 32u), m_tail = merged && (mask & 64u);

    if (!skip_embed) {
        DTensor input = make_dense(s.input, WRK_F16, D, T);
        wrk::layer_norm(q, ln0_w->ptr, ln0_b->ptr, input, LN_EPS);
        wrk::blit(q, input, x);
    }

    for (uint32_t li = layer_begin; li < d.num_layer && li < layer_end; ++li) {
        const wrk_v7_layer_desc& L = layers[li];
        DTensor st_att = make_dense(st->layer_ptr(li), WRK_F32, D, S + 2, st->num_batch);
        st_att.shape[1] = S + 1;
        DTensor st_row0 = st_att; st_row0.shape[1] = 1;
        DTensor st_ffn = make_dense(st->layer_ptr(li), WRK_F32, D, S + 2, st->num_batch);
        st_ffn.shape[1] = 1; st_ffn.offset[1] = S + 1;

        if (m_ln) wrk::layer_norm_from(q, L.ln1_w->ptr, L.ln1_b->ptr, x, att_x, LN_EPS);
        else {
            wrk::blit(q, x, att_x);
            wrk::layer_norm(q, L.ln1_w->ptr, L.ln1_b->ptr, att_x, LN_EPS);
        }
        if (m_shift) {
            const DTensor mixes[6] = {bvec(L.x_r), bvec(L.x_w), bvec(L.x_k), bvec(L.x_v), bvec(L.x_a), bvec(L.x_g)};
            const DTensor outs[6] = {rx, wx, kx, vx, ax, gx};
            wrk::token_shift_multi(q, s.cursors, mixes, outs, 6, st_row0, att_x, 1);
        } else {
            wrk::token_shift(q, s.cursors, bvec(L.x_r), st_row0, att_x, rx, 1);
            wrk::token_shift(q, s.cursors, bvec(L.x_w), st_row0, att_x, wx, 1);
            wrk::token_shift(q, s.cursors, bvec(L.x_k), st_row0, att_x, kx, 1);
            wrk::token_shift(q, s.cursors, bvec(L.x_v), st_row0, att_x, vx, 1);
            wrk::token_shift(q, s.cursors, bvec(L.x_a), st_row0, att_x, ax, 1);
            wrk::token_shift(q, s.cursors, bvec(L.x_g), st_row0, att_x, gx, 1);
        }
        if (m_group) {
            wrk::MatJob ja[7] = {mat_job(L.w_r, rx, r, WRK_ACT_NONE), mat_job(L.w_k, kx, k, WRK_ACT_NONE), mat_job(L.w_v, vx, v, WRK_ACT_NONE),
                                 mat_job(L.w1, wx, aux_w, WRK_ACT_TANH), mat_job(L.a1, ax, aux_a, WRK_ACT_NONE), mat_job(L.g1, gx, aux_g, WRK_ACT_SIGMOID),
                                 mat_job(li ? L.v1 : L.a1, li ? vx : ax, li ? aux_v : aux_a, WRK_ACT_NONE)};
            int32_t rg = wrk_mm_group(ctx, ja, li ? 7 : 6);
            if (rg != WRK_OK) return rg;
            wrk::MatJob jb[4] = {mat_job(L.w2, aux_w, w, WRK_ACT_NONE), mat_job(L.a2, aux_a, a, WRK_ACT_NONE), mat_job(L.g2, aux_g, g, WRK_ACT_NONE),
                                 mat_job(li ? L.v2 : L.a2, li ? aux_v : aux_a, li ? vv : a, WRK_ACT_NONE)};
            rg = wrk_mm_group(ctx, jb, li ? 4 : 3);
            if (rg != WRK_OK) return rg;
        } else {
            MM(L.w_r, rx, r, WRK_ACT_NONE);
            MM(L.w_k, kx, k, WRK_ACT_NONE);
            MM(L.w_v, vx, v, WRK_ACT_NONE);
            MM(L.w1, wx, aux_w, WRK_ACT_TANH);
            MM(L.w2, aux_w, w, WRK_ACT_NONE);
            MM(L.a1, ax, aux_a, WRK_ACT_NONE);
            MM(L.a2, aux_a, a, WRK_ACT_NONE);
            MM(L.g1, gx, aux_g, WRK_ACT_SIGMOID);
            MM(L.g2, aux_g, g, WRK_ACT_NONE);
            if (li) {
                MM(L.v1, vx, aux_v, WRK_ACT_NONE);
                MM(L.v2, aux_v, vv, WRK_ACT_NONE);
            }
        }
        float* wdec = ((size_t)F * (act_dtype == WRK_F32 ? 4 : 2) >= (size_t)4 * D && (size_t)wkv_nseq * H < 768) ? (float*)s.ffn_k : nullptr;
        if (m_pre) {
            wrk::pre_wkv_v7(q, s.w, s.a, s.k, s.v, s.vv, s.att_v0, s.n, L.w0->ptr, L.a0->ptr, L.k_k->ptr, L.k_a->ptr, li ? L.v0->ptr : L.a0->ptr,
                            D, T, li == 0, L2_EPS, wdec);
        } else {
            wrk::binary(q, 0, bvec(L.w0), w, 0, 0, 0);
            wrk::binary(q, 0, bvec(L.a0), a, 0, 0, WRK_ACT_SIGMOID);
            wrk::blit(q, k, kk);
            wrk::binary(q, 1, bvec(L.k_k), kk, 0, 0, 0);
            wrk::l2_norm(q, heads(s.kk), L2_EPS);
            wrk::control_k_v7(q, L.k_a->ptr, a, k);
            if (li == 0) {
                wrk::blit(q, v, v0);
            } else {
                wrk::binary(q, 0, bvec(L.v0), vv, 0, 0, WRK_ACT_SIGMOID);
                wrk::lerp(q, v0, v, vv, 1);
            }
            wrk::blit(q, k, nslice(0));
            wrk::blit(q, v, nslice(1));
            wrk::blit(q, a, nslice(2));
            wrk::blit(q, kk, nslice(3));
        }
        wrk::time_mix_v7(q, s.cursors, st_att, heads(s.r), heads(s.w), n4, heads(s.att_x), wkv_nseq, m_pre ? wdec : nullptr);
        if (m_post) wrk::post_wkv_v7(q, s.att_x, s.r, s.g, s.n, L.gn_w->ptr, L.gn_b->ptr, L.r_k->ptr, D, T, GN_EPS);
        else {
            wrk::group_norm(q, L.gn_w->ptr, L.gn_b->ptr, heads(s.att_x), GN_EPS);
            wrk::time_first_v7(q, L.r_k->ptr, heads(s.r), n4, heads(s.att_x));
            wrk::binary(q, 1, g, att_x, 0, 0, 0);
        }
        if (m_res) {
            wrk::MatJob jo = mat_job(L.w_o, att_x, x, WRK_ACT_NONE);
            jo.has_res = 1;
            jo.res = x;
            const int32_t rg = wrk_mm_group(ctx, &jo, 1);
            if (rg != WRK_OK) return rg;
        } else {
            MM(L.w_o, att_x, o, WRK_ACT_NONE);
            wrk::binary(q, 0, o, x, 0, 0, 0);
        }
        if (m_ln) wrk::layer_norm_from(q, L.ln2_w->ptr, L.ln2_b->ptr, x, ffn_x, LN_EPS);
        else {
            wrk::blit(q, x, ffn_x);
            wrk::layer_norm(q, L.ln2_w->ptr, L.ln2_b->ptr, ffn_x, LN_EPS);
        }
        wrk::token_shift(q, s.cursors, bvec(L.ffn_x_k), st_ffn, ffn_x, ffn_kx, 1);
        MM(L.ffn_w_k, ffn_kx, ffn_k, WRK_ACT_SQUARED_RELU);
        if (m_tail) {
            wrk::MatJob jv = mat_job(L.ffn_w_v, ffn_k, x, WRK_ACT_NONE);
            jv.has_res = 1;
            jv.res = x;
            const int32_t rg = wrk_mm_group(ctx, &jv, 1);
            if (rg != WRK_OK) return rg;
// ... 76 lines not shown
        for (hipStream_t s : m->lane_streams) { hipStreamSynchronize(s); hipStreamDestroy(s); }
        m->release_common();
        m->free_fused();
        wrk_v7_engine_destroy(m->engine);
        m->engine = nullptr;
        for (hipEvent_t e : m->lane_events) hipEventDestroy(e);
        m->lane_streams.clear(); m->lane_events.clear();
    }
    for (wrk_v7_model* lane : m->lanes) wrk_v7_model_destroy(lane);
    m->lanes.clear();
    auto fb = [](const wrk_buf* b) { if (b) wrk_buf_release(const_cast<wrk_buf*>(b)); };
    auto fm = [](const wrk_matrix* x) { if (x) wrk_matrix_release(const_cast<wrk_matrix*>(x)); };
    fb(m->ln0_w); fb(m->ln0_b); fb(m->ln_out_w); fb(m->ln_out_b); fb(m->emb); fm(m->head);
    for (auto& L : m->layers) {
        const wrk_buf* vecs[] = {L.ln1_w, L.ln1_b, L.ln2_w, L.ln2_b, L.x_r, L.x_w, L.x_k, L.x_v, L.x_a, L.x_g, L.w0, L.a0, L.v0,
                                 L.r_k, L.k_k, L.k_a, L.gn_w, L.gn_b, L.ffn_x_k};
        for (const wrk_buf* b : vecs) fb(b);
        const wrk_matrix* mats[] = {L.w1, L.w2, L.a1, L.a2, L.g1, L.g2, L.v1, L.v2, L.w_k, L.w_v, L.w_r, L.w_o, L.ffn_w_k, L.ffn_w_v};
        for (const wrk_matrix* x : mats) fm(x);
    }
    delete m;
    return WRK_OK;
}

size_t wrk_v7_model_token_bytes(const wrk_v7_model* m, uint32_t B) {
    if (!m) return 0;
    const size_t D = m->d.num_emb, S = D / m->d.num_head, V = m->d.num_vocab;
    size_t w = wrk_matrix_stream_bytes(m->head) + 4 * D * 2;
    for (uint32_t l = 0; l < m->d.num_layer; ++l) {
        const wrk_v7_layer_desc& L = m->layers[l];
        const wrk_matrix* mats[] = {L.w1, L.w2, L.a1, L.a2, L.g1, L.g2, L.w_k, L.w_v, L.w_r, L.w_o, L.ffn_w_k, L.ffn_w_v};
        for (const wrk_matrix* x : mats) w += wrk_matrix_stream_bytes(x);
        if (l > 0) w += wrk_matrix_stream_bytes(L.v1) + wrk_matrix_stream_bytes(L.v2) + D * 2;
        w += 18 * D * 2;
    }
    return w + 2 * (size_t)m->d.num_layer * D * (S + 2) * 4 * B + (size_t)B * (D * 2 + V * 4);
}

int32_t wrk_v7_state_create(wrk_ctx* ctx, const wrk_v7_model* model, uint32_t num_batch, wrk_v7_state** out) {
    if (!ctx || !model || !out) return WRK_E_ARG;
    LOCK(ctx);
    *out = nullptr;
    WRK_ARG(ctx, num_batch >= 1 && num_batch <= 255, "num_batch must be 1..255 (cursor batch is u8, tensor/mod.rs:53-60)");
    WRK_HIP(ctx, hipSetDevice(ctx->device));
    wrk_v7_state* st = new wrk_v7_state();
    st->ctx = ctx;
    st->num_layer = model->d.num_layer;
    st->num_emb = model->d.num_emb;
    st->head_size = model->d.num_emb / model->d.num_head;
    st->num_batch = num_batch;
    const size_t bytes = st->layer_elems() * st->num_layer * 4;
    hipError_t e = hipMalloc((void**)&st->data, bytes);
    if (e == hipSuccess) e = hipMemsetAsync(st->data, 0, bytes, ctx->stream);
    if (e != hipSuccess) { delete st; return wrk_fail(ctx, e == hipErrorOutOfMemory ? WRK_E_OOM : WRK_E_HIP, "state alloc: %s", hipGetErrorString(e)); }
    *out = st;
    return WRK_OK;
}

int32_t wrk_v7_state_destroy(wrk_v7_state* st) {
    if (!st) return WRK_E_ARG;
    {
        LOCK(st->ctx);
        hipSetDevice(st->ctx->device);
        hipStreamSynchronize(st->ctx->stream);
        hipFree(st->data);
    }
    delete st;
    return WRK_OK;
}

int32_t wrk_v7_state_load(wrk_ctx* ctx, wrk_v7_state* st, uint32_t batch, const float* src) {
    if (!ctx || !st || !src) return WRK_E_ARG;
    LOCK(ctx);
    WRK_ARG(ctx, batch < st->num_batch, "batch %u out of range", batch);
    WRK_HIP(ctx, hipSetDevice(ctx->device));
    const size_t per = (size_t)(st->head_size + 2) * st->num_emb;
    for (uint32_t l = 0; l < st->num_layer; ++l)
        WRK_HIP(ctx, hipMemcpyAsync(st->layer_ptr(l) + batch * per, src + l * per, per * 4, hipMemcpyHostToDevice, ctx->stream));
    WRK_HIP(ctx, hipStreamSynchronize(ctx->stream));
    return WRK_OK;
}

int32_t wrk_v7_state_back(wrk_ctx* ctx, const wrk_v7_state* st, uint32_t batch, float* dst) {
    if (!ctx || !st || !dst) return WRK_E_ARG;
    LOCK(ctx);
    WRK_ARG(ctx, batch < st->num_batch, "batch %u out of range", batch);
    WRK_HIP(ctx, hipSetDevice(ctx->device));
    const size_t per = (size_t)(st->head_size + 2) * st->num_emb;
    for (uint32_t l = 0; l < st->num_layer; ++l)
        WRK_HIP(ctx, hipMemcpyAsync(dst + l * per, st->layer_ptr(l) + batch * per, per * 4, hipMemcpyDeviceToHost, ctx->stream));
    WRK_HIP(ctx, hipStreamSynchronize(ctx->stream));
    return WRK_OK;
}

static int32_t state_d2d(wrk_ctx* ctx, const wrk_v7_state* st, uint32_t batch, const wrk_buf* buf, bool to_state) {
    if (!ctx || !st || !buf) return WRK_E_ARG;
    LOCK(ctx);
    WRK_ARG(ctx, batch < st->num_batch, "batch %u out of range", batch);
    const size_t per = (size_t)(st->head_size + 2) * st->num_emb;
    WRK_ARG(ctx, buf->bytes >= per * st->num_layer * 4, "snapshot buffer holds %zu bytes, a state needs %zu", buf->bytes, per * st->num_layer * 4);
    WRK_HIP(ctx, hipSetDevice(ctx->device));
    for (uint32_t l = 0; l < st->num_layer; ++l) {
        float* slot = st->layer_ptr(l) + batch * per;
        float* snap = (float*)buf->ptr + l * per;
        WRK_HIP(ctx, hipMemcpyAsync(to_state ? slot : snap, to_state ? snap : slot, per * 4, hipMemcpyDeviceToDevice, ctx->op_stream()));
    }
    return WRK_OK;
}

int32_t wrk_v7_state_read(wrk_ctx* ctx, const wrk_v7_state* st, uint32_t batch, wrk_buf* buf) { return state_d2d(ctx, st, batch, buf, false); }
int32_t wrk_v7_state_write(wrk_ctx* ctx, wrk_v7_state* st, uint32_t batch, const wrk_buf* buf) { return state_d2d(ctx, st, batch, buf, true); }

static int32_t v7_job(wrk_ctx* ctx, wrk_v7_model* m, wrk_v7_state* st, const wrk_job_args& a, uint32_t mode) {
    if (!ctx || !m || !st) return WRK_E_ARG;
    LOCK(ctx);
    WRK_HIP(ctx, hipSetDevice(ctx->device));
    const uint32_t T = a.T, NH = a.NH, V = m->d.num_vocab;
    if (T == 0) return WRK_OK;
    WRK_ARG(ctx, a.cursors, "cursors required");
    WRK_ARG(ctx, a.tokens || a.emb_rows, "either token ids or gathered embedding rows are required");
    WRK_ARG(ctx, !a.tokens || m->emb, "token ids given but the model has no device embedding table");
    WRK_ARG(ctx, NH == 0 || a.headers, "headers required");
    WRK_ARG(ctx, st->num_emb == m->d.num_emb && st->num_layer == m->d.num_layer, "state does not belong to this model");
    wrk_job_shape sh;
    int32_t rc = wrk_job_check(ctx, st, a.cursors, T, a.tokens, V, a.headers, NH, &sh);
    if (rc == WRK_OK) rc = wrk_score_check(ctx, a, V, "wrk_v7_score");
    if (rc == WRK_OK) rc = m->ensure_scratch(T, NH ? NH : 1);
    if (rc == WRK_OK && T == 1 && mode == 1) rc = m->ensure_engine();
    if (rc != WRK_OK) return rc;
    const bool fused = (mode == 1 && sh.one_token_each && sh.nseq == T && m->act_dtype == WRK_F16), want_argmax = NH && a.argmax;
    const uint32_t batch0 = a.cursors[0] & 0xffu;
    rc = wrk_job_upload(*m, m->s, m->s.input, m->emb, m->d.num_emb, a, !fused);
    if (rc != WRK_OK) return rc;
    m->wkv_nseq = sh.nseq;
    auto enqueue_job = [&]() -> int32_t {
        int32_t r;
        if (fused) r = m->enqueue_fused_decode(st, T, NH, sh.identity, a.tokens != nullptr, want_argmax, false, batch0, sh.contiguous);
        else {
            r = m->enqueue_ops(st, T, NH, sh.identity, mode == 1);
            if (r == WRK_OK && want_argmax) wrk::argmax_rows(ctx->op_stream(), m->s.head_o, V, V, NH, m->s.argmax);
        }
        if (r == WRK_OK && a.score && NH &&
            wrk::score_rows(ctx->op_stream(), m->s.head_o, V, V, NH, m->score.targets, m->score.part, m->score.logprob, m->score.rank,
                            ctx->num_cu) != 0)
            r = wrk_fail(ctx, WRK_E_UNSUPPORTED, "score: vocabulary of %u tokens", V);
        return r;
    };
    static const bool no_graph = wrk_no_graph();
    if (no_graph || ctx->capturing_here()) rc = enqueue_job();
    else {
        const uint32_t flags = 16u | (m->act_dtype == WRK_F32 ? 64u : 0u) | (fused ? 1u : 0u) | (sh.identity ? 2u : 0u) | (a.tokens ? 4u : 0u) | (want_argmax ? 8u : 0u) |
                               ((!fused && mode == 1) ? 32u : 0u) | (fused ? batch0 << 8 : 0u) | ((fused && sh.contiguous) ? 1u << 16 : 0u) |
                               ((fused && T == 1 && m->engine_on()) ? 1u << 17 : 0u) | (split_head_env_on() ? 0u : 1u << 18) |
                               ((!fused && (size_t)sh.nseq * m->d.num_head >= 768) ? 1u << 19 : 0u) | (a.score ? 1u << 20 : 0u);
        const wrk_v7_model::GraphKey key{st->uid, T, flags, NH};
        if (!m->graphs.count(key) && m->graphs.size() > 64) { WRK_HIP(ctx, hipStreamSynchronize(ctx->stream)); m->drop_graphs(); }
        wrk_program* prog = nullptr;
        rc = wrk_cached_program(ctx, m->graphs, key, enqueue_job, &prog);
        if (rc != WRK_OK) return rc;
        WRK_HIP(ctx, hipGraphLaunch(prog->exec, ctx->stream));
    }
    if (rc == WRK_OK) rc = wrk_job_read_back(*m, m->s, V, a);
    if (rc != WRK_OK || ctx->capturing_here()) return rc;
    return wrk_v7_engine_check(m->engine);
}

int32_t wrk_v7_infer(wrk_ctx* ctx, wrk_v7_model* m, wrk_v7_state* st, const uint32_t* tokens, const uint16_t* emb_rows,
                     const uint32_t* cursors, uint32_t T, const uint32_t* headers, uint32_t NH, float* logits, uint32_t* argmax,
                     uint32_t mode) {
    return v7_job(ctx, m, st, {tokens, emb_rows, cursors, T, headers, NH, logits, argmax, false, nullptr, nullptr, nullptr}, mode);
}

int32_t wrk_v7_score(wrk_ctx* ctx, wrk_v7_model* m, wrk_v7_state* st, const uint32_t* tokens, const uint16_t* emb_rows,
                     const uint32_t* cursors, uint32_t T, const uint32_t* headers, uint32_t NH, const uint32_t* targets, float* logprob,
                     uint32_t* rank, uint32_t mode) {
    return v7_job(ctx, m, st, {tokens, emb_rows, cursors, T, headers, NH, nullptr, nullptr, true, targets, logprob, rank}, mode);
}

int32_t wrk_v7_model_set_frame_dtype(wrk_ctx* ctx, wrk_v7_model* m, uint32_t dtype) {
    if (!ctx || !m) return WRK_E_ARG;
    LOCK(ctx);
    WRK_ARG(ctx, dtype == WRK_F16 || dtype == WRK_F32, "frame dtype must be WRK_F16 or WRK_F32");
    WRK_ARG(ctx, !ctx->capturing_here(), "cannot change the frame inside a capture");
    if (dtype == m->act_dtype) return WRK_OK;
    WRK_HIP(ctx, hipSetDevice(ctx->device));
    WRK_HIP(ctx, hipStreamSynchronize(ctx->stream));
    m->drop_graphs();
    if (m->scratch) hipFree(m->scratch);
    m->scratch = nullptr;
    m->scratch_tokens = m->scratch_headers = 0;
    m->act_dtype = dtype;
    for (hipStream_t ls : m->lane_streams) WRK_HIP(ctx, hipStreamSynchronize(ls));
    std::vector<wrk_v7_model*> old_lanes;
    old_lanes.swap(m->lanes);
    for (wrk_v7_model* lane : old_lanes) wrk_v7_model_destroy(lane);
    return WRK_OK;
}

int32_t wrk_v7_model_engine_status(wrk_ctx* ctx, wrk_v7_model* m, char* why, size_t capacity) {
    if (!ctx || !m) return WRK_E_ARG;
    LOCK(ctx);
    WRK_HIP(ctx, hipSetDevice(ctx->device));
    WRK_ARG(ctx, !ctx->capturing_here(), "not inside a capture");
    const int32_t rc = m->ensure_engine();
    if (rc != WRK_OK) return rc;
    if (why && capacity) {
        const std::string w = m->engine ? std::to_string(wrk_v7_engine_waves(m->engine)) + " compute waves"
                                        : (m->engine_tried ? m->engine_why : std::string("disabled (WRK_ENGINE=0 or f32 frames)"));
        snprintf(why, capacity, "%s", w.c_str());
    }
    return m->engine ? 1 : 0;
}

int32_t wrk_v7_infer_layer(wrk_ctx* ctx, wrk_v7_model* m, wrk_v7_state* st, uint32_t layer, const void* x, const void* v_first,
                           const uint32_t* cursors, uint32_t T, uint32_t mode) {
    if (!ctx || !m || !st || !x || !cursors) return WRK_E_ARG;
    LOCK(ctx);
    WRK_HIP(ctx, hipSetDevice(ctx->device));
    WRK_ARG(ctx, !ctx->capturing_here(), "wrk_v7_infer_layer cannot be captured");
    WRK_ARG(ctx, layer < m->d.num_layer, "layer %u out of range", layer);
    WRK_ARG(ctx, T >= 1, "no tokens");
    WRK_ARG(ctx, layer == 0 || v_first, "layers above 0 read the layer-0 value (att_v0)");
    WRK_ARG(ctx, st->num_emb == m->d.num_emb && st->num_layer == m->d.num_layer, "state does not belong to this model");
    wrk_job_shape sh;
    int32_t rc = wrk_job_check(ctx, st, cursors, T, nullptr, 0, nullptr, 0, &sh);
    if (rc == WRK_OK) rc = m->ensure_scratch(T, 1);
    if (rc == WRK_OK && T == 1 && mode == 1) rc = m->ensure_engine();
    if (rc != WRK_OK) return rc;
    const size_t esz = m->act_dtype == WRK_F32 ? 4 : 2;
    rc = wrk_buf_write_raw(ctx, m->s.cursors, cursors, (size_t)T * 4);
    if (rc == WRK_OK) rc = wrk_buf_write_raw(ctx, m->s.x, x, (size_t)T * m->d.num_emb * esz);
    if (rc == WRK_OK && v_first) rc = wrk_buf_write_raw(ctx, m->s.att_v0, v_first, (size_t)T * m->d.num_emb * esz);
    if (rc != WRK_OK) return rc;
    m->layer_begin = layer; m->layer_end = layer + 1; m->skip_embed = true;
    m->wkv_nseq = sh.nseq;
    { const char* ei = getenv("WRK_ENGINE_INSPECT"); m->engine_skip_once = !(ei && ei[0] == '1'); }
    if (mode == 1 && sh.one_token_each && sh.nseq == T && m->act_dtype == WRK_F16) rc = m->enqueue_fused_decode(st, T, 0, true, false, false, false, cursors[0] & 0xff, sh.contiguous);
    else rc = m->enqueue_ops(st, T, 0, true, mode == 1);
    m->layer_begin = 0; m->layer_end = 0xffffffffu; m->skip_embed = false; m->engine_skip_once = false;
    if (rc != WRK_OK) return rc;
    WRK_LAUNCH_CHECK(ctx);
    WRK_HIP(ctx, hipStreamSynchronize(ctx->stream));
    return wrk_v7_engine_check(m->engine);
}

int32_t wrk_v7_frame_read(wrk_ctx* ctx, wrk_v7_model* m, const char* name, uint32_t T, void* dst, size_t capacity, size_t* bytes) {
    if (!ctx || !m || !name || !bytes) return WRK_E_ARG;
    LOCK(ctx);
    WRK_ARG(ctx, m->scratch && T >= 1 && T <= m->scratch_tokens, "no frame of %u tokens has been run", T);
    const uint32_t D = m->d.num_emb, F = m->d.num_hidden;
    const V7Scratch& s = m->s;
    struct { const char* n; const void* p; uint32_t c; } tab[] = {
        {"x", s.x, D}, {"att_x", s.att_x, D}, {"att_v0", s.att_v0, D}, {"att_rx", s.rx, D}, {"att_wx", s.wx, D}, {"att_kx", s.kx, D},
        {"att_vx", s.vx, D}, {"att_ax", s.ax, D}, {"att_gx", s.gx, D}, {"att_r", s.r, D}, {"att_w", s.w, D}, {"att_k", s.k, D}, {"att_v", s.v, D},
        {"att_a", s.a, D}, {"att_g", s.g, D}, {"att_o", s.o, D}, {"att_kk", s.kk, D}, {"att_vv", s.vv, D}, {"att_n", s.n, 4 * D},
        {"aux_w", s.aux_w, m->d.lora_w}, {"aux_a", s.aux_a, m->d.lora_a}, {"aux_g", s.aux_g, m->d.lora_g}, {"aux_v", s.aux_v, m->d.lora_v},
        {"ffn_x", s.ffn_x, D}, {"ffn_kx", s.ffn_kx, D}, {"ffn_k", s.ffn_k, F}, {"ffn_v", s.ffn_v, D}, {"att_x_ln", s.ln_tmp, D}};
    const size_t esz = m->act_dtype == WRK_F32 ? 4 : 2;
    for (auto& e : tab)
        if (strcmp(e.n, name) == 0) {
            const size_t n = (size_t)e.c * T * esz;
            *bytes = n;
            if (!dst) return WRK_OK;
            WRK_ARG(ctx, capacity >= n, "frame buffer %s needs %zu bytes, capacity %zu", name, n, capacity);
            WRK_HIP(ctx, hipSetDevice(ctx->device));
            WRK_HIP(ctx, hipMemcpyAsync(dst, e.p, n, hipMemcpyDeviceToHost, ctx->stream));
            WRK_HIP(ctx, hipStreamSynchronize(ctx->stream));
            return WRK_OK;
        }
    return wrk_fail(ctx, WRK_E_ARG, "no frame buffer named %s", name);
}

}

int32_t wrk_v7_model::enqueue_step(wrk_v7_state* st, uint32_t b0, uint32_t B, uint32_t mode, wrk_step_kind kind) {
    int32_t rc;
    const bool fused = mode == 1 && act_dtype == WRK_F16, head_picks = fused && !kind.sampled() && !kind.constrained,
               head_advances = head_picks && kind.tail == wrk_step_kind::PLAIN && !kind.logprobs;
    if (fused) rc = enqueue_fused_decode(st, B, B, true, true, head_picks, head_advances, b0, true);
    else {
        wrk::gather_rows_f16(ctx->op_stream(), emb->ptr, s.tokens, s.input, d.num_emb, B);
        rc = enqueue_ops(st, B, B, true);
    }
    if (rc != WRK_OK || head_advances) return rc;
    return wrk_enqueue_pick(*this, B, kind, st, b0, head_picks);
}

int32_t wrk_v7_model::ensure_frame(uint32_t B, uint32_t mode) {
    const int32_t rc = ensure_scratch(B, B);
    return rc == WRK_OK && B == 1 && mode == 1 ? ensure_engine() : rc;
}

uint32_t wrk_v7_model::key_bits(uint32_t B, uint32_t mode) const {
    return mode | (act_dtype == WRK_F32 ? 4u : 0u) | ((B == 1 && mode == 1 && engine_on()) ? 8u : 0u) | (split_head_env_on() ? 0u : 16u);
}

int32_t wrk_v7_model::lane(uint32_t g, uint32_t groups, wrk_frame_common** out) {
    while (lanes.size() + 1 < groups) {
        wrk_v7_model* clone = nullptr;
        const int32_t rc = wrk_v7_model_create(ctx, &d, &clone);
        if (rc != WRK_OK) return rc;
        clone->act_dtype = act_dtype;
        lanes.push_back(clone);
    }
    while (lane_streams.size() < groups) {
        hipStream_t ls = nullptr;
        hipEvent_t e = nullptr;
        WRK_HIP(ctx, hipStreamCreateWithFlags(&ls, hipStreamNonBlocking));
        WRK_HIP(ctx, hipEventCreateWithFlags(&e, hipEventDisableTiming));
        lane_streams.push_back(ls);
        lane_events.push_back(e);
    }
    wrk_v7_model* mdl = g == 0 ? this : lanes[g - 1];
    mdl->engine_blocked = groups > 1;
    *out = mdl;
    return WRK_OK;
}

void wrk_v7_model::before_loop() { wrk::timing_slot(ctx, nullptr); }

int32_t wrk_v7_model::after_loop(uint32_t groups) {
    wrk::timing_report(ctx);
    for (uint32_t g = 0; g < groups; ++g) {
        wrk_v7_engine* e = (g == 0 ? this : lanes[g - 1])->engine;
        wrk_v7_engine_report(e);
        const int32_t rc = wrk_v7_engine_check(e);
        if (rc != WRK_OK) return rc;
    }
    return WRK_OK;
}

extern "C" {

int32_t wrk_v7_generate_greedy(wrk_ctx* ctx, wrk_v7_model* m, wrk_v7_state* st, const uint32_t* first_tokens, uint32_t B,
                               uint32_t steps, uint32_t* out_tokens, float* last_logits, float* elapsed_ms, uint32_t mode_arg) {
    return wrk_generate(ctx, m, st, first_tokens, B, steps, wrk_pick_args{}, out_tokens, last_logits, elapsed_ms, mode_arg);
}

int32_t wrk_v7_generate_sample(wrk_ctx* ctx, wrk_v7_model* m, wrk_v7_state* st, const uint32_t* first_tokens, uint32_t B, uint32_t steps,
                               const float* temperature, const float* top_p, const uint32_t* seed, uint32_t* out_tokens, float* last_logits,
                               float* elapsed_ms, uint32_t mode_arg) {
    wrk_pick_args pick{temperature, top_p, seed};
    pick.need = wrk_pick_args::SAMPLER;
    return wrk_generate(ctx, m, st, first_tokens, B, steps, pick, out_tokens, last_logits, elapsed_ms, mode_arg);
}

int32_t wrk_v7_generate_penalized(wrk_ctx* ctx, wrk_v7_model* m, wrk_v7_state* st, const uint32_t* first_tokens, uint32_t B, uint32_t steps,
                                  const float* temperature, const float* top_p, const uint32_t* seed, const float* presence,
                                  const float* frequency, const float* decay, wrk_occurrence* occ, uint32_t* out_tokens, float* last_logits,
                                  float* elapsed_ms, uint32_t mode_arg) {
    wrk_pick_args pick{temperature, top_p, seed, presence, frequency, decay, occ};
    pick.need = wrk_pick_args::TABLE;
    return wrk_generate(ctx, m, st, first_tokens, B, steps, pick, out_tokens, last_logits, elapsed_ms, mode_arg);
}

int32_t wrk_v7_generate_stop(wrk_ctx* ctx, wrk_v7_model* m, wrk_v7_state* st, const uint32_t* first_tokens, uint32_t B, uint32_t steps,
                             const wrk_generate_options* opt, uint32_t* out_tokens, uint32_t* out_lengths, float* last_logits,
                             uint32_t* steps_run, float* elapsed_ms, uint32_t mode_arg) {
    const wrk_stop_call stop{opt, out_lengths, steps_run};
    return wrk_generate(ctx, m, st, first_tokens, B, steps, opt ? wrk_pick_of(*opt) : wrk_pick_args{}, out_tokens, last_logits, elapsed_ms, mode_arg, &stop);
}

int32_t wrk_v7_generate_queue(wrk_ctx* ctx, wrk_v7_model* m, wrk_v7_state* st, uint32_t B, const wrk_queue_options* opt,
                              const wrk_queue_result* out_arg, float* elapsed_ms, uint32_t mode_arg) {
    return wrk_generate_queue(ctx, m, st, B, opt, out_arg, elapsed_ms, mode_arg, wrk_step_kind::QUEUE, nullptr);
}

int32_t wrk_v7_generate_queue_pool(wrk_ctx* ctx, wrk_v7_model* m, wrk_v7_state* st, uint32_t B, const wrk_queue_options* opt,
                                   const wrk_queue_result* out_arg, float* elapsed_ms, uint32_t mode_arg, const wrk_queue_pool* pool) {
    return wrk_generate_queue(ctx, m, st, B, opt, out_arg, elapsed_ms, mode_arg, wrk_step_kind::QUEUE_POOL, pool);
}

}

static bool engine_env_on() { const char* e = getenv("WRK_ENGINE"); return !(e && e[0] == '0'); }
bool engine_env_on_public() { return engine_env_on(); }
bool wrk_v7_model::engine_on() const { return engine != nullptr && !engine_blocked && engine_env_on() && act_dtype == WRK_F16; }
int32_t wrk_v7_model::ensure_engine() {
    if (engine_tried || !engine_env_on() || act_dtype != WRK_F16) return WRK_OK;
    if (ctx->capturing_here()) return WRK_OK;
    engine_tried = true;
    const std::string keep = ctx->err;
    const int32_t rc = wrk_v7_engine_create(this, &engine);
    if (rc != WRK_OK) { engine = nullptr; engine_why = ctx->err; ctx->err = keep; }
    if (rc != WRK_OK && rc != WRK_E_UNSUPPORTED) return rc;
    return WRK_OK;
}
```

web-rwkv-gguf_amd/csrc/wrk_v7_engine.h:

```cpp
#pragma once
#include <stdint.h>

#include "wrk_internal.h"

namespace wrk {

constexpr int ENG_K1_JOBS = 7;
constexpr uint32_t ENG_NO_HEAD = 0xffffffffu;

struct EngJob {
    uint32_t rows, row_bytes, f16;
    uint32_t act, mix;
    uint32_t wg0, nwg, rows_per_wg;
    uint32_t gbase;
    uint32_t headed;
};

struct EngShape {
    uint32_t D, F, H, nwg;
    uint32_t rw, ra, rg, rv;
    uint32_t rb_d, rb_f;
    uint32_t rb_w2, rb_a2, rb_g2, rb_v2;
    EngJob k1[ENG_K1_JOBS];
    uint32_t k3_rpw, k5_rpw, k6_rpw;
    uint32_t lds_slot1, lds_slot5, lds_slot6, lds_slot3, lds_xraw0, lds_xraw1, lds_xs, lds_ln, lds_misc, lds_total;
    uint32_t g_x, g_k1, g_o, g_x1, g_k, g_total, g_aux;
    float ln_eps, gn_eps, l2_eps;
    uint32_t layer_begin, layer_end, rescale;
    uint32_t batch, state_rows;
    uint32_t x_from_granules;
};

struct EngLayer {
    const uint8_t *w_r, *w_k, *w_v, *w1, *a1, *g1, *v1;
    const uint8_t *w2, *a2, *g2, *v2;
    const uint8_t *w_o, *ffn_k, *ffn_v;
};
enum { ENG_V_LN1W, ENG_V_LN1B, ENG_V_LN2W, ENG_V_LN2B, ENG_V_MIX0, ENG_V_W0 = ENG_V_MIX0 + 6, ENG_V_A0, ENG_V_V0, ENG_V_RK, ENG_V_KK, ENG_V_KA,
       ENG_V_GNW, ENG_V_GNB, ENG_V_FFNXK, ENG_NV };
enum { ENG_S_O = ENG_K1_JOBS, ENG_S_FK, ENG_S_FV, ENG_NS = 16 };

struct EngArgs {
    EngShape S;
    const EngLayer* layers;
    const void* vecs;
    const float* scal;
    unsigned long long* gran;
    const void* x_in;
    const uint32_t* x_row;
    void* x_out;
    void* v_first;
    float* state;
    uint32_t num_batch;
    uint32_t* fail;
    unsigned long long* stamps;
    uint32_t stamp_layer;
};
constexpr int ENG_STAMPS = 32;

constexpr __host__ __device__ uint32_t eng_wave_pairs(uint32_t pairs, uint32_t ncw, uint32_t wave) {
    const uint32_t simd_rank = (wave + 4u - (ncw + 2u) % 4u) % 4u;
    return pairs / ncw + ((wave / 4u) * 4u + simd_rank < pairs % ncw ? 1u : 0u);
}
constexpr __host__ __device__ uint32_t eng_wave_first_pair(uint32_t pairs, uint32_t ncw, uint32_t wave) {
    const uint32_t extra = pairs % ncw, g4 = (wave / 4u) * 4u;
    uint32_t first = wave * (pairs / ncw) + (extra < g4 ? extra : g4);
    for (uint32_t w = g4; w < wave; ++w) first += eng_wave_pairs(pairs, ncw, w) - pairs / ncw;
    return first;
}
constexpr __host__ __device__ void eng_wave_rows(uint32_t nrows, uint32_t ncw, uint32_t wave, uint32_t& begin, uint32_t& end) {
    const uint32_t pairs = (nrows + 1u) / 2u;
    const uint32_t first = eng_wave_first_pair(pairs, ncw, wave), last = first + eng_wave_pairs(pairs, ncw, wave);
    begin = 2u * first < nrows ? 2u * first : nrows;
    end = 2u * last < nrows ? 2u * last : nrows;
}
constexpr bool eng_wave_rows_ok(uint32_t ncw) {
    for (uint32_t nrows = 0; nrows <= 128; nrows += 2) {
        const uint32_t pairs = nrows / 2, most = (pairs + ncw - 1) / ncw;
        uint32_t next = 0, simd[4] = {0, 0, 0, 0};
        for (uint32_t w = 0; w < ncw; ++w) {
            uint32_t b = 0, e = 0;
            eng_wave_rows(nrows, ncw, w, b, e);
            if (b != next || e < b || (b & 1u) || (e & 1u) || (e - b) / 2 > most || (e - b) / 2 < pairs / ncw) return false;
            simd[w % 4] += (e - b) / 2 - pairs / ncw;
            next = e;
        }
        if (next != nrows) return false;
        const uint32_t s0 = (ncw + 2) % 4;
        for (uint32_t i = 0; i + 1 < 4; ++i) {
            const uint32_t a = simd[(s0 + i) % 4], c = simd[(s0 + i + 1) % 4];
            if (c > a || simd[s0] - simd[(s0 + 3) % 4] > 1) return false;
        }
    }
    return true;
}
static_assert(eng_wave_rows_ok(8) && eng_wave_rows_ok(14), "a row pair without exactly one owner wave, or an uneven schedule");

}

struct wrk_v7_model;
struct wrk_v7_state;
struct wrk_v7_engine;
int32_t wrk_v7_engine_create(wrk_v7_model* m, wrk_v7_engine** out);
void wrk_v7_engine_destroy(wrk_v7_engine* e);
int32_t wrk_v7_engine_enqueue(wrk_v7_engine* e, hipStream_t q, wrk_v7_state* st, uint32_t batch, uint32_t l0, uint32_t l1, const void* x_in,
                              void* x_out, void* v_first, const uint32_t* token = nullptr);
bool wrk_v7_engine_has_table(const wrk_v7_engine* e);
int wrk_v7_engine_waves(const wrk_v7_engine* e);
int32_t wrk_v7_engine_check(wrk_v7_engine* e);
void wrk_v7_engine_report(wrk_v7_engine* e);
```

web-rwkv-gguf_amd/csrc/wrk_v7_engine.hip:

```cpp
#include "wrk_device.h"
#include "wrk_v7.h"
#include "wrk_dmv_body.h"
#include "wrk_v7_engine.h"
#include "wrk_lora_dev.h"

#include <algorithm>
#include <string>

namespace wrk {

#define ENG_LDS __attribute__((address_space(3)))
typedef ENG_LDS unsigned char lds_u8;

#define ENG_BAR() asm volatile("s_waitcnt lgkmcnt(0)\n\ts_barrier" ::: "memory")

constexpr uint32_t ENG_SPIN_MAX = 1u << 21;

__device__ __forceinline__ uint32_t eng_tag(uint32_t layer, uint32_t stage) { return layer * 8u + stage + 1u; }

__device__ __forceinline__ void eng_store_granule(unsigned long long* g, uint32_t tag, uint32_t payload) {
    __hip_atomic_store(g, ((unsigned long long)tag << 32) | payload, __ATOMIC_RELAXED, __HIP_MEMORY_SCOPE_AGENT);
}
__device__ __forceinline__ uint32_t pack_h2(float a, float b) {
    const f16x2 h = {(f16)a, (f16)b};
// ... 760 lines not shown

int32_t wrk_v7_engine_create(wrk_v7_model* m, wrk_v7_engine** out) {
    using namespace wrk;
    wrk_ctx* ctx = m->ctx;
    *out = nullptr;
    const auto& d = m->d;
    const uint32_t D = d.num_emb, F = d.num_hidden, H = d.num_head, NWG = (uint32_t)ctx->num_cu;
    auto no = [&](const char* why) { return wrk_fail(ctx, WRK_E_UNSUPPORTED, "decode engine: %s", why); };
    if (m->act_dtype != WRK_F16) return no("f32 frames");
    if (H == 0 || D != H * 64 || D % 256 || D > 4096 || F % 1024 || F != 4 * D) return no("shape");
    if (d.lora_w % 8 || d.lora_a % 8 || d.lora_g % 8 || d.lora_v % 8 || d.lora_w < 8 || d.lora_a < 8 || d.lora_g < 8 || d.lora_v < 8 ||
        d.lora_w > 128 || d.lora_a > 128 || d.lora_v > 128 || d.lora_g > 256 || ((d.lora_w + d.lora_a + d.lora_g + d.lora_v) % 16))
        return no("LoRA ranks");
    if (NWG < 2 * H || NWG < 64) return no("too few compute units");
    uint32_t quant = 0xffffffffu, flags = 0xffffffffu;
    for (size_t li = 0; li < m->layers.size(); ++li) {
        const auto& L = m->layers[li];
        const wrk_matrix* big[] = {L.w_r, L.w_k, L.w_v, L.w_o, L.ffn_w_k, L.ffn_w_v};
        for (const wrk_matrix* q : big) {
            if (quant == 0xffffffffu) { quant = q->kind; flags = q->flags; }
            if (q->kind != quant || q->flags != flags) return no("mixed matrix kinds");
        }
        const wrk_matrix* lo[] = {L.w1, L.a1, L.g1, li ? L.v1 : L.a1, L.w2, L.a2, L.g2, li ? L.v2 : L.a2};
        for (const wrk_matrix* q : lo)
            if (!q || q->kind != WRK_MAT_F16) return no("LoRA matrices must be F16");
        if (L.w_r->k != D || L.w_r->m != D || L.ffn_w_k->m != F || L.ffn_w_v->k != F || L.w1->m != d.lora_w || L.a1->m != d.lora_a ||
            L.g1->m != d.lora_g || (li && L.v1->m != d.lora_v))
            return no("matrix shapes");
    }
    if (quant != WRK_MAT_Q4_K) return no("only Q4_K matrices so far");
    if (m->layers.empty()) return no("no layers");

    wrk_v7_engine* e = new wrk_v7_engine();
    e->m = m;
    e->quant = quant;
    e->r16 = (flags & WRK_MATRIX_ROUND_F16) != 0;
    e->xd = D <= 2048 ? 1 : 2;
    EngShape& S = e->S;
    S.D = D; S.F = F; S.H = H; S.nwg = NWG;
    S.rw = d.lora_w; S.ra = d.lora_a; S.rg = d.lora_g; S.rv = d.lora_v;
    const auto& L0 = m->layers[0];
    const auto& L1 = m->layers[m->layers.size() > 1 ? 1 : 0];
    S.rb_d = (uint32_t)L0.w_r->row_bytes; S.rb_f = (uint32_t)L0.ffn_w_v->row_bytes;
    S.rb_w2 = (uint32_t)L0.w2->row_bytes; S.rb_a2 = (uint32_t)L0.a2->row_bytes; S.rb_g2 = (uint32_t)L0.g2->row_bytes;
    S.rb_v2 = (uint32_t)(m->layers.size() > 1 ? L1.v2->row_bytes : L0.a2->row_bytes);
    for (const auto& L : m->layers) {
        if (L.w_r->row_bytes != S.rb_d || L.w_k->row_bytes != S.rb_d || L.w_v->row_bytes != S.rb_d || L.w_o->row_bytes != S.rb_d ||
            L.ffn_w_k->row_bytes != S.rb_d || L.ffn_w_v->row_bytes != S.rb_f || L.w2->row_bytes != S.rb_w2 || L.a2->row_bytes != S.rb_a2 ||
            L.g2->row_bytes != S.rb_g2) { delete e; return no("row strides differ between layers"); }
    }
    const uint32_t rb_l = (uint32_t)L0.w1->row_bytes;
    struct { uint32_t rows, rb, f16, act, mix, headed, gbase; } jd[ENG_K1_JOBS] = {
        {D, S.rb_d, 0, WRK_ACT_NONE, 0, 1, 0}, {D, S.rb_d, 0, WRK_ACT_NONE, 2, 1, 1}, {D, S.rb_d, 0, WRK_ACT_NONE, 3, 1, 2},
        {S.rw, rb_l, 1, WRK_ACT_TANH, 1, 0, 0}, {S.ra, rb_l, 1, WRK_ACT_NONE, 4, 0, S.rw / 2}, {S.rg, rb_l, 1, WRK_ACT_SIGMOID, 5, 0, (S.rw + S.ra) / 2},
        {S.rv, rb_l, 1, WRK_ACT_NONE, 3, 0, (S.rw + S.ra + S.rg) / 2}};
    double total = 0;
    for (auto& j : jd) total += (double)j.rows * j.rb;
    uint32_t slot1 = 0;
    bool placed = false;
    const uint32_t NK1 = NWG - H;
    for (double target = total / NK1; target < total; target *= 1.03) {
        uint32_t used = 0, worst = 0;
        uint32_t rpw[ENG_K1_JOBS], nw[ENG_K1_JOBS];
        for (int j = 0; j < ENG_K1_JOBS; ++j) {
            uint32_t r = (uint32_t)(target / jd[j].rb);
            r = std::max(2u, r / 2 * 2);
            rpw[j] = r;
            nw[j] = (jd[j].rows + r - 1) / r;
            used += nw[j];
            worst = std::max(worst, std::min(r, jd[j].rows) * jd[j].rb);
        }
        if (used > NK1) continue;
        uint32_t w0 = 0;
        for (int j = 0; j < ENG_K1_JOBS; ++j) {
            S.k1[j] = EngJob{jd[j].rows, jd[j].rb, jd[j].f16, jd[j].act, jd[j].mix, w0, nw[j], rpw[j], jd[j].gbase, jd[j].headed};
            w0 += nw[j];
        }
        slot1 = worst;
        placed = true;
        break;
    }
    if (!placed) { delete e; return no("K1 partition"); }
    S.k3_rpw = std::max(8u, up((D + NWG - 1) / NWG, 8));
    S.k5_rpw = std::max(8u, up((F + NWG - 1) / NWG, 8));
    S.k6_rpw = std::max(2u, up((D + NWG - 1) / NWG, 2));
    if (S.k6_rpw > 32) { delete e; return no("ffn value rows per workgroup"); }
    uint32_t off = 0;
    auto take = [&](uint32_t bytes) { const uint32_t o = off; off += up(bytes, 1024); return o; };
    S.lds_slot1 = take(slot1);
    S.lds_slot5 = take(S.k5_rpw * S.rb_d);
    S.lds_slot6 = take(S.k6_rpw * S.rb_f);
    S.lds_slot3 = take(S.k3_rpw * S.rb_d);
    S.lds_xraw0 = take(D * 2);
    S.lds_xraw1 = take(D * 2);
    const uint32_t naux = S.rw + S.ra + S.rg + S.rv;
    S.lds_xs = take(D * 2 + up((naux + 192) * 2, 16) + 1280 * 4);
    S.lds_ln = take(D * 2);
    S.lds_misc = take(4096);
    S.lds_total = off;
    int lds_max = 0;
    hipDeviceGetAttribute(&lds_max, hipDeviceAttributeMaxSharedMemoryPerBlock, ctx->device);
    if (lds_max < 160 * 1024) lds_max = 160 * 1024;
    if (S.lds_total > (uint32_t)lds_max) { delete e; return no("weights of a layer do not fit the LDS"); }
    S.g_aux = naux / 2;
    uint32_t g = 0;
    auto gtake = [&](uint32_t n) { const uint32_t o = g; g += up(n, 128); return o; };
    S.g_x = gtake(D / 2);
    S.g_k1 = gtake(S.g_aux + H * 96);
    S.g_o = gtake(D / 2);
    S.g_x1 = gtake(D / 2);
    S.g_k = gtake(F / 2);
    S.g_total = g;
    S.ln_eps = 1.0e-5f; S.gn_eps = 64.0e-5f; S.l2_eps = 1.0e-12f;
    S.rescale = d.rescale ? d.rescale : 0xffffffffu;
    S.state_rows = 64 + 2;

    std::vector<float> hs(m->layers.size() * ENG_NS, 1.0f);
    auto fail_alloc = [&](hipError_t er) { wrk_v7_engine_destroy(e); return wrk_fail(ctx, WRK_E_OOM, "decode engine: %s", hipGetErrorString(er)); };
    hipError_t er;
    std::vector<EngLayer> hl(m->layers.size());
    for (size_t li = 0; li < m->layers.size(); ++li) {
        const auto& L = m->layers[li];
        EngLayer& o = hl[li];
        o.w_r = L.w_r->data; o.w_k = L.w_k->data; o.w_v = L.w_v->data; o.w1 = L.w1->data; o.a1 = L.a1->data; o.g1 = L.g1->data;
        o.v1 = li ? L.v1->data : L.a1->data;
        o.w2 = L.w2->data; o.a2 = L.a2->data; o.g2 = L.g2->data; o.v2 = li ? L.v2->data : L.a2->data;
        o.w_o = L.w_o->data; o.ffn_k = L.ffn_w_k->data; o.ffn_v = L.ffn_w_v->data;
        const wrk_matrix* k1m[ENG_K1_JOBS] = {L.w_r, L.w_k, L.w_v, L.w1, L.a1, L.g1, li ? L.v1 : L.a1};
        float* sc = hs.data() + li * ENG_NS;
        for (int j = 0; j < ENG_K1_JOBS; ++j) sc[j] = k1m[j]->out_scale;
        sc[ENG_S_O] = L.w_o->out_scale; sc[ENG_S_FK] = L.ffn_w_k->out_scale; sc[ENG_S_FV] = L.ffn_w_v->out_scale;
    }
    if ((er = hipMalloc((void**)&e->vecs, hl.size() * ENG_NV * D * 2)) != hipSuccess) return fail_alloc(er);
    for (size_t li = 0; li < m->layers.size(); ++li) {
        const auto& L = m->layers[li];
        const wrk_buf* src[ENG_NV] = {L.ln1_w, L.ln1_b, L.ln2_w, L.ln2_b, L.x_r, L.x_w, L.x_k, L.x_v, L.x_a, L.x_g, L.w0, L.a0, li ? L.v0 : L.w0,
                                      L.r_k, L.k_k, L.k_a, L.gn_w, L.gn_b, L.ffn_x_k};
        for (int i = 0; i < ENG_NV; ++i) {
            if (!src[i] || src[i]->bytes < (size_t)D * 2) { wrk_v7_engine_destroy(e); return no("a layer vector is missing"); }
            if ((er = hipMemcpy((char*)e->vecs + (li * ENG_NV + i) * (size_t)D * 2, src[i]->ptr, (size_t)D * 2, hipMemcpyDeviceToDevice)) != hipSuccess) return fail_alloc(er);
        }
    }
    if ((er = hipMalloc((void**)&e->scal, hs.size() * 4)) != hipSuccess) return fail_alloc(er);
    if ((er = hipMemcpy(e->scal, hs.data(), hs.size() * 4, hipMemcpyHostToDevice)) != hipSuccess) return fail_alloc(er);
    if ((er = hipMalloc((void**)&e->layers, hl.size() * sizeof(EngLayer))) != hipSuccess) return fail_alloc(er);
    if ((er = hipMemcpy(e->layers, hl.data(), hl.size() * sizeof(EngLayer), hipMemcpyHostToDevice)) != hipSuccess) return fail_alloc(er);
    std::vector<uint32_t> hh(2 * NWG, ENG_NO_HEAD);
    for (uint32_t h = 0; h < H; ++h) hh[2 * ((size_t)h * NWG / H)] = h;
    for (uint32_t w = 0, r = 0; w < NWG; ++w)
        if (hh[2 * w] == ENG_NO_HEAD) hh[2 * w + 1] = r++;
    if ((er = hipMalloc((void**)&e->wg_head, hh.size() * 4)) != hipSuccess) return fail_alloc(er);
    if ((er = hipMemcpy(e->wg_head, hh.data(), hh.size() * 4, hipMemcpyHostToDevice)) != hipSuccess) return fail_alloc(er);
    if ((er = hipMalloc((void**)&e->gran, (size_t)S.g_total * 8)) != hipSuccess) return fail_alloc(er);
    if ((er = hipMalloc((void**)&e->fail, 256)) != hipSuccess) return fail_alloc(er);
    if ((er = hipMemset(e->fail, 0, 256)) != hipSuccess) return fail_alloc(er);
    const char* tm = getenv("WRK_TIMING");
    if (tm && tm[0] == '1') {
        const size_t n = (size_t)NWG * 16 * 24 * 8 + 64;
        if ((er = hipMalloc((void**)&e->stamps, n)) != hipSuccess) return fail_alloc(er);
        hipMemset(e->stamps, 0, n);
    }
    { const char* ev = getenv("WRK_ENGINE_WAVES"); e->ncw = (ev && atoi(ev) == 14) ? 14 : 8; }
    const void* fn = eng_kernel_fn(e->xd, e->r16, e->ncw);
    if ((er = hipFuncSetAttribute(fn, hipFuncAttributeMaxDynamicSharedMemorySize, (int)S.lds_total)) != hipSuccess) {
        wrk_v7_engine_destroy(e);
        return wrk_fail(ctx, WRK_E_UNSUPPORTED, "decode engine: %u bytes of LDS refused (%s)", S.lds_total, hipGetErrorString(er));
    }
    {
        hipFuncAttributes fa{};
        const int waves = e->ncw + 2, per_simd = (waves + 3) / 4;
        if (hipFuncGetAttributes(&fa, fn) == hipSuccess && fa.numRegs > 0) {
            const int alloc = (fa.numRegs + 7) / 8 * 8;
            if (per_simd * alloc > 512 || fa.maxThreadsPerBlock < waves * 64 || (size_t)fa.sharedSizeBytes + S.lds_total > 160 * 1024) {
                const int regs = fa.numRegs;
                wrk_v7_engine_destroy(e);
                return wrk_fail(ctx, WRK_E_UNSUPPORTED, "decode engine: a workgroup of %d waves x %d registers + %u bytes of LDS does not fit a CU", waves, regs,
                                S.lds_total);
            }
        }
        (void)hipGetLastError();
    }
    {
        const char* te = getenv("WRK_ENGINE_TABLE");
        if (!(te && te[0] == '0') && m->emb && m->ln0_w && m->ln0_b) {
            const size_t bytes = (size_t)d.num_vocab * D * 2;
            if (hipMalloc(&e->emb_ln, bytes) == hipSuccess) {
                LnMixParams P{};
                P.src = (const f16*)m->emb->ptr; P.ln_w = (const f16*)m->ln0_w->ptr; P.ln_b = (const f16*)m->ln0_b->ptr; P.eps = 1.0e-5f;
                P.d = D; P.nmix = 0; P.ln_out = (f16*)e->emb_ln;
                if (ln_mix(ctx->stream, P, d.num_vocab) != 0 || hipStreamSynchronize(ctx->stream) != hipSuccess) { hipFree(e->emb_ln); e->emb_ln = nullptr; }
            } else e->emb_ln = nullptr;
            (void)hipGetLastError();
        }
    }
    *out = e;
    return WRK_OK;
}

bool wrk_v7_engine_has_table(const wrk_v7_engine* e) { return e && e->emb_ln; }
int wrk_v7_engine_waves(const wrk_v7_engine* e) { return e ? e->ncw : 0; }

void wrk_v7_engine_destroy(wrk_v7_engine* e) {
    if (!e) return;
    if (e->emb_ln) hipFree(e->emb_ln);
    if (e->layers) hipFree(e->layers);
    if (e->vecs) hipFree(e->vecs);
    if (e->scal) hipFree(e->scal);
    if (e->wg_head) hipFree(e->wg_head);
    if (e->gran) hipFree(e->gran);
    if (e->fail) hipFree(e->fail);
    if (e->stamps) hipFree(e->stamps);
    delete e;
}

int32_t wrk_v7_engine_enqueue(wrk_v7_engine* e, hipStream_t q, wrk_v7_state* st, uint32_t batch, uint32_t l0, uint32_t l1, const void* x_in, void* x_out,
                              void* v_first, const uint32_t* token) {
    using namespace wrk;
    wrk_ctx* ctx = e->m->ctx;
    EngArgs A{};
    A.S = e->S;
    A.S.layer_begin = l0; A.S.layer_end = l1; A.S.batch = batch;
    A.layers = e->layers; A.vecs = e->vecs; A.scal = e->scal; A.gran = e->gran; A.x_in = x_in; A.x_out = x_out; A.v_first = v_first;
    if (token && e->emb_ln && l0 == 0) { A.x_in = e->emb_ln; A.x_row = token; }
    A.state = st->data; A.num_batch = st->num_batch; A.fail = e->fail; A.stamps = e->stamps; A.stamp_layer = std::min(5u, l1 - 1);
    WRK_HIP(ctx, hipMemsetAsync(e->gran, 0, (size_t)e->S.g_total * 8, q));
    const dim3 grid(e->S.nwg), block((e->ncw + 2) * 64);
    hipLaunchKernelGGL(eng_kernel(e->xd, e->r16, e->ncw), grid, block, e->S.lds_total, q, A, (const uint32_t*)e->wg_head);
    WRK_LAUNCH_CHECK(ctx);
    return WRK_OK;
}

int32_t wrk_v7_engine_check(wrk_v7_engine* e) {
    if (!e) return WRK_OK;
    wrk_ctx* ctx = e->m->ctx;
    uint32_t f = 0;
    WRK_HIP(ctx, hipMemcpy(&f, e->fail, 4, hipMemcpyDeviceToHost));
    if (f) {
        hipMemset(e->fail, 0, 4);
        return wrk_fail(ctx, WRK_E_HIP, "decode engine: a hand-off wait gave up (stage mask 0x%x): workgroups not co-resident or a producer died", f);
    }
    return WRK_OK;
}

void wrk_v7_engine_report(wrk_v7_engine* e) {
    using namespace wrk;
    if (!e || !e->stamps) return;
    const uint32_t NWG = e->S.nwg, NW = (uint32_t)e->ncw + 2;
    std::vector<unsigned long long> h((size_t)NWG * NW * 24);
    if (hipMemcpy(h.data(), e->stamps, h.size() * 8, hipMemcpyDeviceToHost) != hipSuccess) return;
    unsigned long long t0 = ~0ull;
    for (auto v : h) if (v && v < t0) t0 = v;
    std::vector<char> is_head(NWG, 0);
    for (uint32_t hd = 0; hd < e->S.H; ++hd) is_head[(size_t)hd * NWG / e->S.H] = 1;
    auto col = [&](int wave, uint32_t k, const char* label, int cls = -1) {
        std::vector<double> v;
        for (uint32_t w = 0; w < NWG; ++w) {
            if (cls >= 0 && is_head[w] != cls) continue;
            unsigned long long x = 0;
            if (wave >= 0) x = h[((size_t)w * NW + wave) * 24 + k];
            else for (int cw = 0; cw < e->ncw; ++cw) x = std::max(x, h[((size_t)w * NW + cw) * 24 + k]);
            if (x) v.push_back((double)(x - t0) * 0.01);
        }
        if (v.empty()) return;
        std::sort(v.begin(), v.end());
        fprintf(stderr, "  %-62s %4zu WGs  first %7.2f  median %7.2f  last %7.2f us\n", label, v.size(), v.front(), v[v.size() / 2], v.back());
    };
    {
        unsigned long long tail[2] = {0, 0};
        if (hipMemcpy(tail, e->stamps + (size_t)NWG * 16 * 24, 16, hipMemcpyDeviceToHost) == hipSuccess && tail[1])
            fprintf(stderr, "[WRK_TIMING] decode engine: shader clock over the last launch %.0f MHz (%llu cycles in %.1f us)\n",
                    (double)tail[0] / ((double)tail[1] * 0.01), tail[0], (double)tail[1] * 0.01);
    }
    const int G = e->ncw, Ld = e->ncw + 1;
    fprintf(stderr, "[WRK_TIMING] decode engine (%d compute waves), one layer of the last token; us since the layer's first stamp\n", e->ncw);
    col(G, 0, "gather: layer input complete, workgroups without a head", 0);
    col(G, 0, "gather: layer input complete, head workgroups", 1);
    col(0, 1, "K1 start (input + weights in LDS), wave 0, no head", 0);
    col(0, 1, "K1 start (input in LDS), wave 0, head workgroups", 1);
    col(0, 2, "K1 LN + shift done, wave 0");
    col(0, 3, "K1 rows published, wave 0, no head", 0);
    col(-1, 3, "K1 rows published, slowest wave, no head", 0);
    col(-1, 3, "K1 LN + shift done, slowest wave, head workgroups", 1);
    col(G, 4, "gather (heads): LoRA intermediates complete");
    col(G, 1, "gather (heads): K1 outputs complete");
    col(0, 4, "K2 start");
    col(-1, 16, "K2 LoRA dots done, slowest wave");
    col(0, 17, "K2 per-channel stage done");
    col(-1, 18, "K2 state updated, slowest wave");
    col(0, 5, "K2 published");
    col(G, 2, "gather: head outputs complete");
    col(0, 6, "K3 start");
    col(-1, 7, "K3 published, slowest wave");
    col(G, 3, "gather: x1 complete");
    col(0, 8, "K5 start");
    col(0, 14, "K5 LN + shift done, wave 0");
    col(0, 9, "K5 published, wave 0");
    col(-1, 9, "K5 published, slowest wave");
    col(0, 10, "K6 own quarter of the ffn vector swept, wave 0");
    col(-1, 10, "K6 swept, slowest wave");
    col(0, 11, "K6 start");
    col(-1, 12, "K6 partial sums done, slowest wave");
    col(0, 13, "K6 published");
    col(Ld, 0, "loader: K1 slot free, next layer's fill issued");
}
```

web-rwkv-gguf_amd/csrc/wrk_v7_fused.hip:

```cpp
#include "wrk_device.h"
#include "wrk_v7.h"
#include "wrk_v7_engine.h"
#include "wrk_lora_dev.h"

namespace wrk {

__global__ void advance_tokens_kernel(const uint32_t* __restrict__ argmax, uint32_t* __restrict__ tokens,
                                      uint32_t* __restrict__ history, uint32_t* __restrict__ counter, uint32_t b) {
    const uint32_t step = *counter;
    const uint32_t i = threadIdx.x;
    if (i < b) {
        const uint32_t t = argmax[i];
        tokens[i] = t;
        history[(size_t)step * b + i] = t;
    }
    __syncthreads();
    if (i == 0) *counter = step + 1;
}

void advance_tokens(hipStream_t s, const uint32_t* argmax, uint32_t* tokens, uint32_t* history, uint32_t* counter, uint32_t b) {
    advance_tokens_kernel<<<1, 256, 0, s>>>(argmax, tokens, history, counter, b);
}

template <int VPT, int NMIX>
// ... 310 lines not shown
        for (int c = 0; c < 4; ++c) {
            const float s = Sv[c] * wj + kj * sh_v[4 * wave + c] + sa[c] * bj;
            Sv[c] = s;
            y[c] = rj * s;
        }
        *(f32x4*)st = Sv;
#pragma unroll
        for (int c = 0; c < 4; ++c) y[c] = wave_sum(y[c]);
        WRK_STAMP(P.dbg, 3);
        if (lane < 4) {
            const float yv = lane == 0 ? y[0] : (lane == 1 ? y[1] : (lane == 2 ? y[2] : y[3]));
            const uint32_t i = 4 * wave + lane;
            const size_t o = (size_t)t * D + cq + i;
            P.out[o] = (f16)yv;
            tt_out[o] = sh_xx * sh_v[i];
            g_out[o] = (f16)sh_g[i];
        }
    }
    WRK_STAMP(P.dbg, 4);
}

__global__ void __launch_bounds__(256) argmax_finish_kernel(const float* __restrict__ pv, const uint32_t* __restrict__ pi, uint32_t nwg,
                                                             uint32_t ntok, uint32_t* __restrict__ argmax, uint32_t* __restrict__ tokens,
                                                             uint32_t* __restrict__ history, uint32_t* __restrict__ counter) {
    __shared__ float sv[4];
    __shared__ uint32_t si[4];
    const uint32_t step = counter ? *counter : 0;
    for (uint32_t n = 0; n < ntok; ++n) {
        float bv = -3.0e38f;
        uint32_t bi = 0xffffffffu;
        for (uint32_t w = threadIdx.x; w < nwg; w += 256) {
            const float v = pv[(size_t)w * ntok + n];
            const uint32_t i2 = pi[(size_t)w * ntok + n];
            if (v > bv || (v == bv && i2 < bi)) { bv = v; bi = i2; }
        }
#pragma unroll
        for (int o = 32; o > 0; o >>= 1) {
            const float ov = __shfl_xor(bv, o, WAVE);
            const uint32_t oi = __shfl_xor(bi, o, WAVE);
            if (ov > bv || (ov == bv && oi < bi)) { bv = ov; bi = oi; }
        }
        __syncthreads();
        if ((threadIdx.x & 63) == 0) { sv[threadIdx.x >> 6] = bv; si[threadIdx.x >> 6] = bi; }
        __syncthreads();
        if (threadIdx.x == 0) {
            for (int k = 1; k < 4; ++k)
                if (sv[k] > bv || (sv[k] == bv && si[k] < bi)) { bv = sv[k]; bi = si[k]; }
            if (bi == 0xffffffffu) bi = 0;
            argmax[n] = bi;
            if (tokens) { tokens[n] = bi; history[(size_t)step * ntok + n] = bi; }
        }
    }
    if (counter && threadIdx.x == 0) *counter = step + 1;
}

void argmax_finish(hipStream_t s, const float* pv, const uint32_t* pi, uint32_t nwg, uint32_t ntok, uint32_t* argmax, uint32_t* tokens,
                   uint32_t* history, uint32_t* counter) {
    argmax_finish_kernel<<<1, 256, 0, s>>>(pv, pi, nwg, ntok, argmax, tokens, history, counter);
}

}

static constexpr uint32_t TIMED_LAYER = 5;
namespace {
struct TimingState {
    unsigned long long* dev = nullptr;
    std::vector<std::string> labels;
    bool enabled = false, init = false;
} g_timing;
}
unsigned long long* wrk::timing_slot(wrk_ctx* ctx, const char* label) {
    if (!g_timing.init) { const char* e = getenv("WRK_TIMING"); g_timing.enabled = e && e[0] == '1'; g_timing.init = true; }
    if (!g_timing.enabled) return nullptr;
    if (!g_timing.dev) {
        if (hipMalloc((void**)&g_timing.dev, 64 * 16 * 8) != hipSuccess) return nullptr;
        hipMemset(g_timing.dev, 0, 64 * 16 * 8);
    }
    if (!label) return nullptr;
    for (size_t i = 0; i < g_timing.labels.size(); ++i)
        if (g_timing.labels[i] == label) return g_timing.dev + i * 16;
    if (g_timing.labels.size() >= 64) return nullptr;
    g_timing.labels.push_back(label);
    return g_timing.dev + (g_timing.labels.size() - 1) * 16;
}
void wrk::timing_report(wrk_ctx* ctx) {
    if (!g_timing.enabled || !g_timing.dev || g_timing.labels.empty()) return;
    std::vector<unsigned long long> h(64 * 16);
    hipMemcpy(h.data(), g_timing.dev, h.size() * 8, hipMemcpyDeviceToHost);
    unsigned long long t0 = ~0ull;
    for (size_t i = 0; i < g_timing.labels.size() * 16; ++i) if (h[i] && h[i] < t0) t0 = h[i];
    fprintf(stderr, "[WRK_TIMING] layer %u of the last decode step; ns since the first stamp (100 MHz clock); first WG | last WG\n", TIMED_LAYER);
    for (size_t i = 0; i < g_timing.labels.size(); ++i) {
        fprintf(stderr, "  %-40s", g_timing.labels[i].c_str());
        for (int w = 0; w < 2; ++w) {
            for (int k = 0; k < 5; ++k) {
                const unsigned long long v = h[i * 16 + w * 8 + k];
                if (v) fprintf(stderr, " %6llu", (v - t0) * 10); else fprintf(stderr, "      -");
            }
            if (w == 0) fprintf(stderr, "  |");
        }
        fprintf(stderr, "\n");
    }
}

void wrk_v7_model::free_fused() {
    if (amax_val) hipFree(amax_val);
    if (amax_idx) hipFree(amax_idx);
    amax_val = nullptr; amax_idx = nullptr; amax_cap = 0;
}

int32_t wrk_v7_model::enqueue_fused_decode(wrk_v7_state* st, uint32_t T, uint32_t NH, bool identity_headers, bool from_tokens,
                                            bool want_argmax, bool advance, uint32_t cursor0_batch, bool contiguous) {
    using namespace wrk;
    hipStream_t q = ctx->op_stream();
    const uint32_t D = d.num_emb, F = d.num_hidden, H = d.num_head, S = D / H, V = d.num_vocab;
    bool ok = (D % 8 == 0) && D <= 8192 && d.lora_w % 8 == 0 && d.lora_a % 8 == 0 && d.lora_g % 8 == 0 && d.lora_v % 8 == 0 &&
              d.lora_w <= 128 && d.lora_a <= 128 && d.lora_v <= 128 && d.lora_g <= 512;
    for (auto& L : layers) {
        const wrk_matrix* ms[] = {L.w2, L.a2, L.g2, L.v2};
        for (const wrk_matrix* m : ms)
            if (m && m->kind != WRK_MAT_F16) ok = false;
    }
    if (!ok) {
        if (from_tokens) gather_rows_f16(q, emb->ptr, s.tokens, s.input, D, T);
        int32_t rc = enqueue_ops(st, T, NH, identity_headers);
        if (rc != WRK_OK) return rc;
        if (want_argmax && NH) {
            argmax_rows(q, s.head_o, V, V, NH, s.argmax);
            if (advance) advance_tokens(q, s.argmax, s.tokens, history, s.counter, NH);
        }
        return WRK_OK;
    }
    auto vec = [&](void* p, uint32_t c = 0) { return make_dense(p, WRK_F16, c ? c : D, T); };
    bool single = false;
    auto run_jobs = [&](MatJob* jobs, int n) -> int {
        if (!single && T >= gemm_min_tokens()) {
            jobs[0].ks_part = s.ks_part; jobs[0].ks_cnt = s.ks_cnt; jobs[0].ks_part_cap = s.ks_part_cap; jobs[0].ks_cnt_cap = s.ks_cnt_cap;
            jobs[0].xsum = ctx->gemm_scratch; jobs[0].xsum_cap = ctx->gemm_scratch_cap;
            if (matmul_mfma_multi(q, jobs, n, ctx->num_cu) == 0) return 0;
            for (int i = 0; i < n; ++i) {
                int rc = matmul_mfma(q, jobs[i], ctx->num_cu);
                if (rc == -2) rc = matvec(q, &jobs[i], 1, ctx->num_cu);
                if (rc != 0) return rc;
            }
            return 0;
        }
        return matvec_grouped(q, jobs, n, ctx->num_cu);
    };
#define LN(P, n)                                                                             \
    do {                                                                                     \
        if (ln_mix(q, P, n) != 0) return wrk_fail(ctx, WRK_E_UNSUPPORTED, "ln_mix shape");   \
    } while (0)

    if (T >= 2 && s.ks_cnt && s.ks_cnt_cap) WRK_HIP(ctx, hipMemsetAsync(s.ks_cnt, 0, (size_t)s.ks_cnt_cap * 4, q));
    const bool eng_embeds = T == 1 && from_tokens && !skip_embed && layer_begin == 0 && engine_on() && !engine_skip_once && wrk_v7_engine_has_table(engine) &&
                            d.num_layer > 0;
    if (!skip_embed && !eng_embeds) {
        LnMixParams P{};
        if (from_tokens) { P.src = (const f16*)emb->ptr; P.ids = s.tokens; }
        else P.src = (const f16*)s.input;
        P.ln_w = (const f16*)ln0_w->ptr; P.ln_b = (const f16*)ln0_b->ptr; P.eps = 1.0e-5f;
        P.d = D; P.nmix = 0; P.ln_out = (f16*)s.x;
        LN(P, T);
    }
    uint32_t first_launch_layer = layer_begin;
    if (T == 1 && engine_on() && !engine_skip_once) {
        const uint32_t l1 = std::min<uint32_t>(d.num_layer, layer_end);
        if (layer_begin < l1) {
            const int32_t rc = wrk_v7_engine_enqueue(engine, q, st, cursor0_batch, layer_begin, l1, s.x, s.x, s.att_v0, eng_embeds ? s.tokens : nullptr);
            if (rc != WRK_OK) return rc;
        }
        first_launch_layer = l1;
    }
    for (uint32_t li = first_launch_layer; li < d.num_layer && li < layer_end; ++li) {
        const wrk_v7_layer_desc& L = layers[li];
        float* lst = st->layer_ptr(li);
        static const bool fuse_ln = [] { const char* e = getenv("WRK_FUSE_LN"); return !(e && e[0] == '0'); }();
        static const uint32_t few_max = [] { const char* e = getenv("WRK_DMV_TOKENS"); const int v = e ? atoi(e) : 4; return (uint32_t)(v < 1 ? 1 : (v > 4 ? 4 : v)); }();
        single = fuse_ln && (T == 1 || (T <= few_max && contiguous)) && D <= 4096;
        if (single) {
            MatJob k1[7] = {mat_job(L.w_r, vec(s.x), vec(s.r), 0), mat_job(L.w_k, vec(s.x), vec(s.k), 0), mat_job(L.w_v, vec(s.x), vec(s.v), 0),
                            mat_job(L.w1, vec(s.x), vec(s.aux_w, d.lora_w), 0), mat_job(L.a1, vec(s.x), vec(s.aux_a, d.lora_a), 0),
                            mat_job(L.g1, vec(s.x), vec(s.aux_g, d.lora_g), 0), mat_job(li ? L.v1 : L.a1, vec(s.x), vec(s.aux_v, d.lora_v), 0)};
            for (MatJob& j : k1) j.pro = 1;
            MatJob k5 = mat_job(L.ffn_w_k, vec(s.x), vec(s.ffn_k, F), 0);
            k5.pro = 1;
            MatJob k6 = mat_job(L.ffn_w_v, vec(s.ffn_k, F), vec(s.x), 0);
            k6.has_res = 1; k6.res = vec(s.x);
            k6.carry_dst = (float*)s.x;
            single = matvec_grouped(q, k1, li ? 7 : 6, ctx->num_cu, true) == 0 && matvec(q, &k5, 1, ctx->num_cu, true) == 0 &&
                     matvec(q, &k6, 1, ctx->num_cu, true) == 0;
        }
        const bool want_split = split_head_env_on() && !(T == 1 && engine != nullptr && engine_env_on_public() && !engine_skip_once);
        const uint32_t state_stride = (S + 2) * D;
        bool split_head = want_split && single && d.lora_w >= 8 && d.lora_a >= 8 && d.lora_g >= 8 && d.lora_v >= 8 && d.lora_g <= 512;
        if (split_head) {
            MatJob k3 = mat_job(L.w_o, vec(s.att_x), vec(s.x), 0);
            k3.has_res = 1; k3.res = vec(s.x);
            k3.pro = 2; k3.ln_w = L.gn_w->ptr; k3.ln_b = L.gn_b->ptr; k3.mixw = s.g; k3.prev = (const float*)s.n;
            split_head = matvec(q, &k3, 1, ctx->num_cu, true) == 0;
        }
        uint32_t batch0 = 0;
        if (single) batch0 = cursor0_batch;
        float* row0 = lst + (size_t)batch0 * (S + 2) * D;
        if (!single) {
            LnMixParams P{};
            P.src = (const f16*)s.x; P.ln_w = (const f16*)L.ln1_w->ptr; P.ln_b = (const f16*)L.ln1_b->ptr; P.eps = 1.0e-5f;
            P.d = D; P.nmix = 6;
            const wrk_buf* mx[6] = {L.x_r, L.x_w, L.x_k, L.x_v, L.x_a, L.x_g};
            void* outs[6] = {s.rx, s.wx, s.kx, s.vx, s.ax, s.gx};
            for (int i = 0; i < 6; ++i) { P.mix[i] = (const f16*)mx[i]->ptr; P.out[i] = (f16*)outs[i]; }
            P.state_row = lst; P.state_stride = (size_t)(S + 2) * D; P.cursors = s.cursors; P.batch1 = contiguous ? cursor0_batch + 1 : 0;
            LN(P, T);
        }
        {
            MatJob jobs[7] = {mat_job(L.w_r, vec(s.rx), vec(s.r), WRK_ACT_NONE), mat_job(L.w_k, vec(s.kx), vec(s.k), WRK_ACT_NONE),
                              mat_job(L.w_v, vec(s.vx), vec(s.v), WRK_ACT_NONE),
                              mat_job(L.w1, vec(s.wx), vec(s.aux_w, d.lora_w), WRK_ACT_TANH),
                              mat_job(L.a1, vec(s.ax), vec(s.aux_a, d.lora_a), WRK_ACT_NONE),
                              mat_job(L.g1, vec(s.gx), vec(s.aux_g, d.lora_g), WRK_ACT_SIGMOID),
                              mat_job(li ? L.v1 : L.a1, vec(s.vx), vec(s.aux_v, d.lora_v), WRK_ACT_NONE)};
            if (single) {
                const wrk_buf* mx[7] = {L.x_r, L.x_k, L.x_v, L.x_w, L.x_a, L.x_g, L.x_v};
                for (int i = 0; i < 7; ++i) {
                    jobs[i].in = vec(s.x);
                    jobs[i].pro = 1; jobs[i].pro_eps = 1.0e-5f; jobs[i].ln_w = L.ln1_w->ptr; jobs[i].ln_b = L.ln1_b->ptr;
                    jobs[i].mixw = mx[i]->ptr; jobs[i].prev = row0; jobs[i].tok_prev_stride = state_stride;
                }
                jobs[0].ln_out = s.ln_tmp;
            }
            if (li == TIMED_LAYER) jobs[0].dbg = jobs[(li ? 7 : 6) - 1].dbg = wrk::timing_slot(ctx, "K1 r,k,v + LoRA-1 (LN1 prologue)");
            const int rc = run_jobs(jobs, li ? 7 : 6);
            if (rc != 0) return wrk_fail(ctx, WRK_E_ARG, "fused K1 rejected (%d)", rc);
        }
        {
            HeadParams P{};
            P.d = D; P.layer0 = li == 0;
            P.rw = d.lora_w; P.ra = d.lora_a; P.rg = d.lora_g; P.rv = d.lora_v;
            P.w2 = (const f16*)L.w2->data; P.a2 = (const f16*)L.a2->data; P.g2 = (const f16*)L.g2->data;
            P.w2_rb = (uint32_t)L.w2->row_bytes; P.a2_rb = (uint32_t)L.a2->row_bytes; P.g2_rb = (uint32_t)L.g2->row_bytes;
            if (li) { P.v2 = (const f16*)L.v2->data; P.v2_rb = (uint32_t)L.v2->row_bytes; P.v0 = (const f16*)L.v0->ptr; }
            P.w0 = (const f16*)L.w0->ptr; P.a0 = (const f16*)L.a0->ptr;
            P.k_k = (const f16*)L.k_k->ptr; P.k_a = (const f16*)L.k_a->ptr; P.r_k = (const f16*)L.r_k->ptr;
            P.gn_w = (const f16*)L.gn_w->ptr; P.gn_b = (const f16*)L.gn_b->ptr;
            P.aux_w = (const f16*)s.aux_w; P.aux_a = (const f16*)s.aux_a; P.aux_g = (const f16*)s.aux_g; P.aux_v = (const f16*)s.aux_v;
            P.r = (const f16*)s.r; P.k = (const f16*)s.k; P.v = (const f16*)s.v;
            P.v_first = (f16*)s.att_v0; P.out = (f16*)s.att_x;
            P.state = lst; P.cursors = s.cursors; P.gn_eps = 64.0e-5f; P.l2_eps = 1.0e-12f;
            P.shift_src = single ? (const f16*)s.ln_tmp : nullptr;
            P.batch1 = (single || contiguous) ? cursor0_batch + 1 : 0;
            P.dbg = li == TIMED_LAYER ? wrk::timing_slot(ctx, "K2 head: LoRA-2 + WKV7 + group norm") : nullptr;
            if (split_head) {
                if (d.lora_g <= 256) head_split_kernel<2><<<dim3(H * 4, T), 256, 0, q>>>(P, (float*)s.n, (f16*)s.g, H);
                else head_split_kernel<4><<<dim3(H * 4, T), 256, 0, q>>>(P, (float*)s.n, (f16*)s.g, H);
            }
            else if (d.lora_g <= 256) head_kernel<8><<<dim3(H, T), 256, 0, q>>>(P);
            else head_kernel<16><<<dim3(H, T), 256, 0, q>>>(P);
        }
        {
            MatJob j = mat_job(L.w_o, vec(s.att_x), vec(s.x), WRK_ACT_NONE);
            j.has_res = 1; j.res = vec(s.x);
            if (split_head) {
                j.pro = 2; j.pro_eps = 64.0e-5f; j.ln_w = L.gn_w->ptr; j.ln_b = L.gn_b->ptr; j.mixw = s.g; j.prev = (const float*)s.n;
                j.tok_mix_stride = D; j.tok_prev_stride = D;
            }
            if (li == TIMED_LAYER) j.dbg = wrk::timing_slot(ctx, "K3 w_o + residual");
            if (run_jobs(&j, 1) != 0) return wrk_fail(ctx, WRK_E_ARG, "fused K3 rejected");
        }
        float* rowf = lst + ((size_t)batch0 * (S + 2) + (S + 1)) * D;
        if (!single) {
            LnMixParams P{};
            P.src = (const f16*)s.x; P.ln_w = (const f16*)L.ln2_w->ptr; P.ln_b = (const f16*)L.ln2_b->ptr; P.eps = 1.0e-5f;
            P.d = D; P.nmix = 1; P.mix[0] = (const f16*)L.ffn_x_k->ptr; P.out[0] = (f16*)s.ffn_kx;
            P.state_row = lst + (size_t)(S + 1) * D; P.state_stride = (size_t)(S + 2) * D; P.cursors = s.cursors; P.batch1 = contiguous ? cursor0_batch + 1 : 0;
            LN(P, T);
        }
        {
            MatJob j = mat_job(L.ffn_w_k, vec(s.ffn_kx), vec(s.ffn_k, F), WRK_ACT_SQUARED_RELU);
            if (single) {
                j.in = vec(s.x);
                j.pro = 1; j.pro_eps = 1.0e-5f; j.ln_w = L.ln2_w->ptr; j.ln_b = L.ln2_b->ptr; j.mixw = L.ffn_x_k->ptr; j.prev = rowf;
                j.tok_prev_stride = state_stride;
                j.ln_out = s.ffn_x;
            }
            if (li == TIMED_LAYER) j.dbg = wrk::timing_slot(ctx, "K5 ffn key (LN2 prologue)");
            if (run_jobs(&j, 1) != 0) return wrk_fail(ctx, WRK_E_ARG, "fused K5 rejected");
        }
        {
            MatJob j = mat_job(L.ffn_w_v, vec(s.ffn_k, F), vec(s.x), WRK_ACT_NONE);
            j.has_res = 1; j.res = vec(s.x);
            if (single) { j.carry_src = s.ffn_x; j.carry_dst = rowf; j.tok_carry_src_stride = D; j.tok_carry_dst_stride = state_stride; }
            if (li == TIMED_LAYER) j.dbg = wrk::timing_slot(ctx, "K6 ffn value + residual");
            if (run_jobs(&j, 1) != 0) return wrk_fail(ctx, WRK_E_ARG, "fused K6 rejected");
        }
        if ((li + 1) % d.rescale == 0) wrk::affine(q, vec(s.x), 0.5f, 0.0f);
    }
    if (NH > 0) {
        LnMixParams P{};
        P.src = (const f16*)s.x; P.ids = identity_headers ? nullptr : s.headers;
        P.ln_w = (const f16*)ln_out_w->ptr; P.ln_b = (const f16*)ln_out_b->ptr; P.eps = 1.0e-5f;
        P.d = D; P.nmix = 0; P.ln_out = (f16*)s.head_x;
        LN(P, NH);
        MatJob j = mat_job(head, make_dense(s.head_x, WRK_F16, D, NH), make_dense(s.head_o, WRK_F32, V, NH), WRK_ACT_NONE);
        uint32_t nwg = 0;
        bool head_mv = NH < gemm_min_tokens();
        if (!head_mv && NH <= 4) {
            MatJob probe = j;
            if (want_argmax) { probe.amax_val = amax_val; probe.amax_idx = amax_idx; }
            head_mv = (size_t)matvec_num_wg(&j, 1, ctx->num_cu, nullptr) * NH <= amax_cap && matvec(q, &probe, 1, ctx->num_cu, true, false, true) == 0;
        }
        if (!head_mv && matmul_mfma(q, j, ctx->num_cu) == 0) {
            if (want_argmax) {
                wrk::argmax_rows(q, (const float*)s.head_o, V, V, NH, s.argmax);
                if (advance) wrk::advance_tokens(q, s.argmax, s.tokens, history, s.counter, NH);
            }
        } else {
            if (want_argmax) {
                nwg = matvec_num_wg(&j, 1, ctx->num_cu, nullptr);
                if ((size_t)nwg * NH > amax_cap) return wrk_fail(ctx, WRK_E_ARG, "arg-max scratch too small");
                j.amax_val = amax_val; j.amax_idx = amax_idx;
            }
            if (matvec(q, &j, 1, ctx->num_cu) != 0) return wrk_fail(ctx, WRK_E_ARG, "fused head rejected");
            if (want_argmax)
                argmax_finish(q, amax_val, amax_idx, nwg, NH, s.argmax, advance ? s.tokens : nullptr, history, advance ? s.counter : nullptr);
        }
    }
#undef LN
    WRK_LAUNCH_CHECK(ctx);
    return WRK_OK;
}
```

Measured before the change: 1712 tokens/s.

## Fuse output LayerNorm, head matvec, argmax and token advance into one kernel

Adds a dedicated head launch that computes the final LayerNorm as a prologue (new plain-LN prologue mode), the Q6_K head matvec, and a grid-wide argmax. The argmax uses per-workgroup candidates and a two-level ticket counter so the last workgroup finishes the reduction and advances the token/history/counter. The same kernel also zeroes the decode engine's granule counters, replacing a separate memset after the engine launch. This removes several small launches (LN, argmax, advance, memset) per token. In exchange it adds atomic ticket synchronisation and shared state that must be reset on engine failure.

```diff
diff --git a/web-rwkv-gguf_amd/csrc/wrk_dmv.hip b/web-rwkv-gguf_amd/csrc/wrk_dmv.hip
--- a/web-rwkv-gguf_amd/csrc/wrk_dmv.hip
+++ b/web-rwkv-gguf_amd/csrc/wrk_dmv.hip
@@ -144,4 +144,67 @@
     return 0;
 }
 
-}
+template <int KIND, int XI, int VPT>
+__global__ void __launch_bounds__(256) dmv_head_kernel(const DJob J, const HeadTail TL) {
+    __shared__ __attribute__((aligned(16))) unsigned char smem[dmv_smem_bytes<4 + VPT, 1>()];
+    dmv_body<KIND, false, XI, 1, 4 + VPT, 1, DJob, HeadTail>(J, smem, TL);
+}
+
+typedef void (*dmv_head_fn)(const DJob, const HeadTail);
+
+template <int KIND>
+static dmv_head_fn pick_dmv_head(uint32_t xi, int vpt) {
+    constexpr bool KQ = KIND == WRK_MAT_Q4_K || KIND == WRK_MAT_Q5_K || KIND == WRK_MAT_Q6_K;
+    if (xi == 1 && vpt == 1) return dmv_head_kernel<KIND, 1, 1>;
+    if (xi == 2 && vpt == 1 && KIND != WRK_MAT_F16) return dmv_head_kernel<KIND, 2, 1>;
+    if constexpr (KQ)
+        if (xi == 2 && vpt == 2) return dmv_head_kernel<KIND, 2, 2>;
+    return nullptr;
+}
+
+int launch_dmv_head(hipStream_t s, const JobDev& J, uint32_t total_wg, const HeadTail& T, bool dry) {
+    static const bool enabled = [] { const char* e = getenv("WRK_DMV"); return !(e && e[0] == '0'); }();
+    if (!enabled) return -1;
+    auto dense_base = [](const DTensor& t) { return ((size_t)t.offset[2] * t.stride[1] + t.offset[1]) * t.stride[0] + t.offset[0]; };
+    if (J.in.dtype != WRK_F16 || (J.k & 7u) || J.k > 4096 || J.in.shape[1] * J.in.shape[2] != 1 || (J.flags & WRK_MATRIX_ROUND_F16)) return -1;
+    if ((J.out.dtype != WRK_F16 && J.out.dtype != WRK_F32) || J.m == 0 || J.rows_per_wg == 0 || J.pro != 3 || J.has_res || J.carry_dst || J.gate) return -1;
+    const size_t ib = dense_base(J.in);
+    if (ib & 7u) return -1;
+    const int vpt = J.k <= 2048 ? 1 : 2;
+    const uint32_t kpad = (J.k + 15u) & ~15u;
+    uint32_t xi;
+    if (J.kind == WRK_MAT_F16) xi = ((kpad >> 3) + 63) / 64;
+    else if (J.kind == WRK_MAT_Q8_0 || J.kind == WRK_MAT_INT8) xi = ((J.k >> 4) + 63) / 64;
+    else if (J.kind == WRK_MAT_Q4_K || J.kind == WRK_MAT_Q5_K || J.kind == WRK_MAT_Q6_K) xi = ((J.k >> 8) * 8 + 63) / 64;
+    else return -1;
+    if (xi == 0 || (J.kind != WRK_MAT_F16 && J.kind != WRK_MAT_Q8_0 && J.kind != WRK_MAT_INT8 && (J.k & 255u))) return -1;
+    static const size_t max_bytes = [] { const char* e = getenv("WRK_DMV_MAXMB"); return (size_t)(e ? atoi(e) : 24) << 20; }();
+    if ((size_t)J.m * J.row_bytes > max_bytes && xi > 1) return -1;
+    dmv_head_fn fn = nullptr;
+    switch (J.kind) {
+        case WRK_MAT_Q4_K: fn = pick_dmv_head<WRK_MAT_Q4_K>(xi, vpt); break;
+        case WRK_MAT_Q5_K: fn = pick_dmv_head<WRK_MAT_Q5_K>(xi, vpt); break;
+        case WRK_MAT_Q6_K: fn = pick_dmv_head<WRK_MAT_Q6_K>(xi, vpt); break;
+        case WRK_MAT_Q8_0: fn = pick_dmv_head<WRK_MAT_Q8_0>(xi, vpt); break;
+        case WRK_MAT_F16: fn = xi <= 2 ? pick_dmv_head<WRK_MAT_F16>(xi, vpt) : (xi <= 4 && vpt == 1 ? (dmv_head_fn)dmv_head_kernel<WRK_MAT_F16, 4, 1> : nullptr); break;
+        default: break;
+    }
+    if (!fn) return -1;
+    if (dry) return 0;
+    DJob D;
+    memset(&D, 0, sizeof D);
+    D.w = J.w;
+    D.x = (const f16*)J.in.p + ib;
+    D.out = (char*)J.out.p + dense_base(J.out) * (J.out.dtype == WRK_F32 ? 4 : 2);
+    D.flags = (J.out.dtype == WRK_F32 ? DJ_OUT32 : 0u) | (J.ln_out ? DJ_PUBLISH : 0u) | (T.cand ? DJ_FINISH : 0u);
+    D.ln_w = J.ln_w; D.ln_b = J.ln_b; D.ln_out = J.ln_out; D.eps = J.pro_eps;
+    D.dbg = J.dbg;
+    D.k = J.k; D.m = J.m; D.row_bytes = J.row_bytes; D.rows_per_wg = J.rows_per_wg; D.wg_begin = 0; D.act = J.act; D.kind = J.kind;
+    D.scale = J.scale;
+    HeadTail TL = T;
+    TL.nwg = total_wg;
+    hipLaunchKernelGGL(fn, dim3(total_wg, 1), dim3(256), 0, s, D, TL);
+    return 0;
+}
+
+}
diff --git a/web-rwkv-gguf_amd/csrc/wrk_dmv_body.h b/web-rwkv-gguf_amd/csrc/wrk_dmv_body.h
--- a/web-rwkv-gguf_amd/csrc/wrk_dmv_body.h
+++ b/web-rwkv-gguf_amd/csrc/wrk_dmv_body.h
@@ -3,7 +3,7 @@
 
 namespace wrk {
 
-enum { DJ_RES = 1, DJ_RES32 = 2, DJ_CARRY = 4, DJ_GATE = 8, DJ_AMAX = 16, DJ_OUT32 = 32, DJ_PUBLISH = 64 };
+enum { DJ_RES = 1, DJ_RES32 = 2, DJ_CARRY = 4, DJ_GATE = 8, DJ_AMAX = 16, DJ_OUT32 = 32, DJ_PUBLISH = 64, DJ_FINISH = 128 };
 
 #define WRK_DJOB_FIELDS                                                                                                          \
     const uint8_t* w;                                                                                                            \
@@ -38,6 +38,8 @@
 template <int NT> struct DParamsOf { typedef DParamsT type; };
 template <> struct DParamsOf<1> { typedef DParams type; };
 
+struct DNoTail {};
+
 template <class JT> struct TokF {
     static __device__ __forceinline__ uint32_t ntok(const JT&) { return 1u; }
     static __device__ __forceinline__ uint32_t xs(const JT&) { return 0u; }
@@ -95,9 +97,11 @@
     }
 }
 
-template <int KIND, bool R16, int XI, int KS, int PRO, int NT, class JT>
-__device__ __forceinline__ void dmv_body(const JT J, unsigned char* smem) {
+template <int KIND, bool R16, int XI, int KS, int PRO, int NT, class JT, class TAIL = DNoTail>
+__device__ __forceinline__ void dmv_body(const JT J, unsigned char* smem, const TAIL TL = TAIL()) {
     typedef TokF<JT> TF;
+    constexpr bool HAS_TAIL = !__is_same(TAIL, DNoTail);
+    static_assert(!HAS_TAIL || (NT == 1 && KS == 1), "the fused tail belongs to the one-token head launch");
     constexpr int RB = 4;
     constexpr uint32_t CSTEP = KS == 1 ? 64u : 256u;
     const uint32_t K = J.k, kpad = (K + 15u) & ~15u;
@@ -139,7 +143,9 @@
     const uint32_t fl = J.flags;
     uint32_t res_bits = 0, carry_bits = 0, gate_bits = 0;
     constexpr int VPT = PRO == 0 ? 1 : ((PRO - 1) % 2 + 1);
-    constexpr bool GN = PRO >= 3;
+    constexpr bool GN = PRO == 3 || PRO == 4;
+    constexpr bool PLN = PRO >= 5;
+    static_assert(!PLN || NT == 1, "the plain-LN prologue is a one-token prologue");
     f16x8 xv[NT][VPT], wv[VPT], bv[VPT], mv[GN ? NT : 1][VPT];
     f32x4 pv[NT][VPT][2];
     f16 c0h[NT];
@@ -155,12 +161,13 @@
             for (int t = 0; t < NT; ++t) {
                 const uint32_t tt = tok_of(t);
                 xv[t][v] = *(const f16x8*)(xin + (size_t)tt * TF::xs(J) + i * 8);
+                if (PLN) continue;
                 if (GN || t == 0) mv[GN ? t : 0][v] = *(const f16x8*)(J.mixw + (size_t)tt * TF::mix_s(J) + i * 8);
                 pv[t][v][0] = *(const f32x4*)(J.prev + (size_t)tt * TF::prev_s(J) + i * 8);
                 pv[t][v][1] = *(const f32x4*)(J.prev + (size_t)tt * TF::prev_s(J) + i * 8 + 4);
             }
         }
-        if (!GN) {
+        if (!GN && !PLN) {
 #pragma unroll
             for (int t = 0; t < NT; ++t) c0h[t] = xin[(size_t)tok_of(t) * TF::xs(J)];
         }
@@ -217,7 +224,44 @@
 #pragma unroll
             for (int ci = 0; ci < XI; ++ci) x[t][ci] = load_x<KIND>(xs + (size_t)t * kpad, min(cbase + CSTEP * ci, nch - 1), true);
     }
-    if (PRO > 0 && !GN) {
+    if (PLN) {
+        const uint32_t nvec = K >> 3;
+        float s = 0.0f;
+#pragma unroll
+        for (int v = 0; v < VPT; ++v)
+            if (tid + 256 * v < nvec)
+#pragma unroll
+                for (int e = 0; e < 8; ++e) s += (float)xv[0][v][e];
+        const float mean = block_sum<4>(s, red) / (float)K;
+        float q = 0.0f;
+#pragma unroll
+        for (int v = 0; v < VPT; ++v)
+            if (tid + 256 * v < nvec)
+#pragma unroll
+                for (int e = 0; e < 8; ++e) { const float dl = (float)xv[0][v][e] - mean; q += dl * dl; }
+        const float var = block_sum<4>(q, red) / (float)K + J.eps;
+        const float dev = 1.0f / sqrtf(var);
+        WRK_STAMP(J.dbg, 4);
+        const bool publish = (fl & DJ_PUBLISH) && blockIdx.x == J.wg_begin;
+#pragma unroll
+        for (int v = 0; v < VPT; ++v) {
+            const uint32_t i = tid + 256 * v;
+            if (i >= nvec) continue;
+            f16x8 yv;
+#pragma unroll
+            for (int e = 0; e < 8; ++e) {
+                const float value = ((float)xv[0][v][e] - mean) * dev;
+                yv[e] = (f16)__builtin_fmaf(value, (float)wv[v][e], (float)bv[v][e]);
+            }
+            *(f16x8*)(xs + i * 8) = yv;
+            if (publish) *(f16x8*)(J.ln_out + i * 8) = yv;
+        }
+        for (uint32_t i = K + tid; i < kpad; i += 256) xs[i] = (f16)0.0f;
+        __syncthreads();
+#pragma unroll
+        for (int ci = 0; ci < XI; ++ci) x[0][ci] = load_x<KIND>(xs, min(cbase + CSTEP * ci, nch - 1), true);
+    }
+    if (PRO > 0 && !GN && !PLN) {
         const uint32_t nvec = K >> 3;
         float s1[NT], s2[NT];
 #pragma unroll
@@ -335,7 +379,76 @@
         }
     }
     WRK_STAMP(J.dbg, 3);
-    if (fl & DJ_AMAX) {
+    if constexpr (HAS_TAIL) {
+        const uint32_t wg = blockIdx.x - J.wg_begin;
+        if (TL.zero) {
+            const u32x4 z = {0u, 0u, 0u, 0u};
+            for (uint32_t i = wg * 256u + tid; i < TL.zero_vec; i += TL.nwg * 256u) ((u32x4*)TL.zero)[i] = z;
+        }
+        if (fl & DJ_FINISH) {
+#pragma unroll
+            for (int o = 2; o > 0; o >>= 1) {
+                const float ov = __shfl_xor(best_v, o, WAVE);
+                const uint32_t oi = __shfl_xor(best_i, o, WAVE);
+                if (ov > best_v || (ov == best_v && oi < best_i)) { best_v = ov; best_i = oi; }
+            }
+            if (lane == 0) { sv[wave] = best_v; si[wave] = best_i; }
+            __syncthreads();
+            if (tid == 0) {
+                float bv2 = sv[0];
+                uint32_t bi = si[0];
+                for (int w = 1; w < 4; ++w)
+                    if (sv[w] > bv2 || (sv[w] == bv2 && si[w] < bi)) { bv2 = sv[w]; bi = si[w]; }
+                __hip_atomic_store(TL.cand + wg, ((unsigned long long)__builtin_bit_cast(uint32_t, bv2) << 32) | bi, __ATOMIC_RELAXED, __HIP_MEMORY_SCOPE_AGENT);
+            }
+            asm volatile("s_waitcnt vmcnt(0)" ::: "memory");
+            __syncthreads();
+            if (tid == 0) {
+                const uint32_t grp = wg >> 5, ngrp = (TL.nwg + 31u) >> 5, gsize = min(32u, TL.nwg - (grp << 5));
+                uint32_t* gt = TL.ticket + 32u * (grp + 1u);
+                uint32_t last = 0;
+                if (__hip_atomic_fetch_add(gt, 1u, __ATOMIC_RELAXED, __HIP_MEMORY_SCOPE_AGENT) == gsize - 1) {
+                    __hip_atomic_store(gt, 0u, __ATOMIC_RELAXED, __HIP_MEMORY_SCOPE_AGENT);
+                    if (__hip_atomic_fetch_add(TL.ticket, 1u, __ATOMIC_RELAXED, __HIP_MEMORY_SCOPE_AGENT) == ngrp - 1) {
+                        __hip_atomic_store(TL.ticket, 0u, __ATOMIC_RELAXED, __HIP_MEMORY_SCOPE_AGENT);
+                        last = 1;
+                    }
+                }
+                si[0] = last;
+            }
+            __syncthreads();
+            if (si[0] == 0) return;
+            float bv = -3.0e38f;
+            uint32_t bi = 0xffffffffu;
+            for (uint32_t w = tid; w < TL.nwg; w += 256) {
+                const unsigned long long c = __hip_atomic_load(TL.cand + w, __ATOMIC_RELAXED, __HIP_MEMORY_SCOPE_AGENT);
+                const float v = __builtin_bit_cast(float, (uint32_t)(c >> 32));
+                const uint32_t i2 = (uint32_t)c;
+                if (v > bv || (v == bv && i2 < bi)) { bv = v; bi = i2; }
+            }
+#pragma unroll
+            for (int o = 32; o > 0; o >>= 1) {
+                const float ov = __shfl_xor(bv, o, WAVE);
+                const uint32_t oi = __shfl_xor(bi, o, WAVE);
+                if (ov > bv || (ov == bv && oi < bi)) { bv = ov; bi = oi; }
+            }
+            __syncthreads();
+            if (lane == 0) { sv[wave] = bv; si[wave] = bi; }
+            __syncthreads();
+            if (tid == 0) {
+                for (int k = 1; k < 4; ++k)
+                    if (sv[k] > bv || (sv[k] == bv && si[k] < bi)) { bv = sv[k]; bi = si[k]; }
+                if (bi == 0xffffffffu) bi = 0;
+                TL.argmax[0] = bi;
+                if (TL.tokens) {
+                    const uint32_t step = *TL.counter;
+                    TL.tokens[0] = bi;
+                    TL.history[step] = bi;
+                    *TL.counter = step + 1;
+                }
+            }
+        }
+    } else if (fl & DJ_AMAX) {
 #pragma unroll
         for (int o = (KS == 1 ? 2 : 32); o > 0; o >>= 1) {
             const float ov = __shfl_xor(best_v, o, WAVE);
diff --git a/web-rwkv-gguf_amd/csrc/wrk_internal.h b/web-rwkv-gguf_amd/csrc/wrk_internal.h
--- a/web-rwkv-gguf_amd/csrc/wrk_internal.h
+++ b/web-rwkv-gguf_amd/csrc/wrk_internal.h
@@ -301,7 +301,16 @@
     void* xsum = nullptr;
     size_t xsum_cap = 0;
 };
+struct HeadTail {
+    unsigned long long* cand = nullptr;
+    uint32_t* ticket = nullptr;
+    uint32_t *argmax = nullptr, *tokens = nullptr, *history = nullptr, *counter = nullptr;
+    void* zero = nullptr;
+    uint32_t zero_vec = 0;
+    uint32_t nwg = 0;
+};
 uint32_t matvec_num_wg(const MatJob* jobs, int njobs, int num_cu, uint32_t* rows_per_wg);
+int matvec_head_tail(hipStream_t s, const MatJob& job, HeadTail t, int num_cu, bool dry_run = false);
 int matvec(hipStream_t s, const MatJob* jobs, int njobs, int num_cu, bool dry_run = false, bool no_catchall = false, bool dmv_only = false);
 int matvec_grouped(hipStream_t s, const MatJob* jobs, int njobs, int num_cu, bool dry_run = false);
 int matmul_mfma(hipStream_t s, const MatJob& job, int num_cu);
diff --git a/web-rwkv-gguf_amd/csrc/wrk_matvec.hip b/web-rwkv-gguf_amd/csrc/wrk_matvec.hip
--- a/web-rwkv-gguf_amd/csrc/wrk_matvec.hip
+++ b/web-rwkv-gguf_amd/csrc/wrk_matvec.hip
@@ -692,6 +692,27 @@
     return wg;
 }
 
+static void job_dev(JobDev& d, const MatJob& j, uint32_t rows_per_wg, uint32_t wg_begin) {
+    d.w = j.w; d.aux = (const float*)j.aux; d.kind = j.kind; d.flags = j.flags; d.k = j.k; d.m = j.m;
+    d.row_bytes = j.row_bytes; d.act = j.act; d.rows_per_wg = rows_per_wg; d.wg_begin = wg_begin;
+    d.in = j.in; d.out = j.out; d.res = j.res; d.has_res = j.has_res;
+    d.amax_val = j.amax_val; d.amax_idx = j.amax_idx;
+    d.pro = j.pro; d.pro_eps = j.pro_eps; d.ln_w = (const f16*)j.ln_w; d.ln_b = (const f16*)j.ln_b;
+    d.mixw = (const f16*)j.mixw; d.prev = j.prev; d.ln_out = (f16*)j.ln_out;
+    d.carry_src = (const f16*)j.carry_src; d.carry_dst = j.carry_dst; d.gate = (const f16*)j.gate; d.scale = j.scale; d.dbg = j.dbg;
+    d.tok_prev_stride = j.tok_prev_stride; d.tok_mix_stride = j.tok_mix_stride; d.tok_carry_src_stride = j.tok_carry_src_stride;
+    d.tok_carry_dst_stride = j.tok_carry_dst_stride; d.tok_gate_stride = j.tok_gate_stride;
+}
+
+int matvec_head_tail(hipStream_t s, const MatJob& job, HeadTail t, int num_cu, bool dry_run) {
+    if (job.pro != 3 || job.in.shape[1] * job.in.shape[2] != 1) return -1;
+    uint32_t rpw = 4;
+    const uint32_t wg = matvec_num_wg(&job, 1, num_cu, &rpw);
+    JobDev d;
+    job_dev(d, job, matvec_job_rpw(&job, 1, 0, rpw), 0);
+    return launch_dmv_head(s, d, wg, t, dry_run);
+}
+
 int matvec(hipStream_t s, const MatJob* jobs, int njobs, int num_cu, bool dry_run, bool no_catchall, bool dmv_only) {
     if (njobs <= 0 || njobs > MAX_JOBS) return -1;
     MatvecParams P;
@@ -707,16 +728,9 @@
     matvec_num_wg(jobs, njobs, num_cu, &rpw);
     uint32_t wg = 0;
     for (int j = 0; j < njobs; ++j) {
+        if (jobs[j].pro == 3) return -3;
         JobDev& d = P.jobs[j];
-        d.w = jobs[j].w; d.aux = (const float*)jobs[j].aux; d.kind = jobs[j].kind; d.flags = jobs[j].flags; d.k = jobs[j].k; d.m = jobs[j].m;
-        d.row_bytes = jobs[j].row_bytes; d.act = jobs[j].act; d.rows_per_wg = matvec_job_rpw(jobs, njobs, j, rpw); d.wg_begin = wg;
-        d.in = jobs[j].in; d.out = jobs[j].out; d.res = jobs[j].res; d.has_res = jobs[j].has_res;
-        d.amax_val = jobs[j].amax_val; d.amax_idx = jobs[j].amax_idx;
-        d.pro = jobs[j].pro; d.pro_eps = jobs[j].pro_eps; d.ln_w = (const f16*)jobs[j].ln_w; d.ln_b = (const f16*)jobs[j].ln_b;
-        d.mixw = (const f16*)jobs[j].mixw; d.prev = jobs[j].prev; d.ln_out = (f16*)jobs[j].ln_out;
-        d.carry_src = (const f16*)jobs[j].carry_src; d.carry_dst = jobs[j].carry_dst; d.gate = (const f16*)jobs[j].gate; d.scale = jobs[j].scale; d.dbg = jobs[j].dbg;
-        d.tok_prev_stride = jobs[j].tok_prev_stride; d.tok_mix_stride = jobs[j].tok_mix_stride; d.tok_carry_src_stride = jobs[j].tok_carry_src_stride;
-        d.tok_carry_dst_stride = jobs[j].tok_carry_dst_stride; d.tok_gate_stride = jobs[j].tok_gate_stride;
+        job_dev(d, jobs[j], matvec_job_rpw(jobs, njobs, j, rpw), wg);
         wg += (jobs[j].m + d.rows_per_wg - 1) / d.rows_per_wg;
     }
     bool f32in = false;
diff --git a/web-rwkv-gguf_amd/csrc/wrk_matvec_dev.h b/web-rwkv-gguf_amd/csrc/wrk_matvec_dev.h
--- a/web-rwkv-gguf_amd/csrc/wrk_matvec_dev.h
+++ b/web-rwkv-gguf_amd/csrc/wrk_matvec_dev.h
@@ -351,5 +351,6 @@
 
 
 int launch_dmv(hipStream_t s, const MatvecParams& P, uint32_t total_wg, int quant, bool has_f16, bool r16, bool dry, int quant2 = -1);
-
-}
+int launch_dmv_head(hipStream_t s, const JobDev& J, uint32_t total_wg, const HeadTail& T, bool dry);
+
+}
diff --git a/web-rwkv-gguf_amd/csrc/wrk_v7.h b/web-rwkv-gguf_amd/csrc/wrk_v7.h
--- a/web-rwkv-gguf_amd/csrc/wrk_v7.h
+++ b/web-rwkv-gguf_amd/csrc/wrk_v7.h
@@ -8,6 +8,7 @@
     void *input, *x, *att_x, *att_v0, *rx, *wx, *kx, *vx, *ax, *gx, *r, *w, *k, *v, *a, *g, *o, *kk, *vv, *n;
     void *aux_w, *aux_a, *aux_g, *aux_v, *ffn_x, *ffn_kx, *ffn_k, *ffn_v, *ln_tmp, *head_x;
     float* ks_part; uint32_t* ks_cnt; size_t ks_part_cap; uint32_t ks_cnt_cap;
+    unsigned long long* head_cand; uint32_t head_cand_cap; uint32_t* head_ticket;
 };
 
 struct wrk_v7_model : wrk_frame_common {
@@ -21,6 +22,7 @@
     float* amax_val = nullptr;
     uint32_t* amax_idx = nullptr;
     size_t amax_cap = 0;
+    size_t head_ticket_bytes = 0;
 
     uint32_t layer_begin = 0, layer_end = 0xffffffffu;
     bool skip_embed = false;
@@ -35,6 +37,7 @@
     std::string engine_why;
     int32_t ensure_engine();
     bool engine_on() const;
+    int32_t engine_check();
     Facts facts() const override { return {d.num_vocab, d.num_emb, d.num_layer, emb != nullptr}; }
     wrk::FrameIo& io() override { return s; }
     int32_t ensure_frame(uint32_t B, uint32_t mode) override;
@@ -53,3 +56,4 @@
 
 bool split_head_env_on();
 bool engine_env_on_public();
+bool fuse_tail_env_on();
diff --git a/web-rwkv-gguf_amd/csrc/wrk_v7.hip b/web-rwkv-gguf_amd/csrc/wrk_v7.hip
--- a/web-rwkv-gguf_amd/csrc/wrk_v7.hip
+++ b/web-rwkv-gguf_amd/csrc/wrk_v7.hip
@@ -34,6 +34,9 @@
     const size_t o_headx = take(D * nh * esz), o_heado = take(V * nh * 4);
     const size_t o_cur = take((size_t)nt * 4), o_tok = take((size_t)nt * 4), o_hdr = take((size_t)nh * 4), o_arg = take((size_t)nh * 4);
     const size_t o_cnt = take(256);
+    const size_t cand_cap = (V + 3) / 4, o_cand = take(cand_cap * 8);
+    head_ticket_bytes = ((cand_cap + 31) / 32 + 1) * 128;
+    const size_t o_ticket = take(head_ticket_bytes);
     size_t ks_floats = 0, ks_groups = 0, o_ksp = 0, o_ksc = 0;
     if (nt >= 2 && act_dtype == WRK_F16) {
         const size_t ntp = nt <= 16 ? 16 : (nt <= 32 ? 32 : 64);
@@ -70,6 +73,7 @@
     s.head_x = b + o_headx; s.head_o = (float*)(b + o_heado);
     s.cursors = (uint32_t*)(b + o_cur); s.tokens = (uint32_t*)(b + o_tok); s.headers = (uint32_t*)(b + o_hdr); s.argmax = (uint32_t*)(b + o_arg);
     s.counter = (uint32_t*)(b + o_cnt);
+    s.head_cand = (unsigned long long*)(b + o_cand); s.head_cand_cap = (uint32_t)cand_cap; s.head_ticket = (uint32_t*)(b + o_ticket);
     s.ks_part = ks_floats ? (float*)(b + o_ksp) : nullptr; s.ks_cnt = ks_floats ? (uint32_t*)(b + o_ksc) : nullptr;
     s.ks_part_cap = ks_floats; s.ks_cnt_cap = (uint32_t)ks_groups;
     scratch_tokens = nt;
@@ -452,7 +456,8 @@
         const uint32_t flags = 16u | (m->act_dtype == WRK_F32 ? 64u : 0u) | (fused ? 1u : 0u) | (sh.identity ? 2u : 0u) | (a.tokens ? 4u : 0u) | (want_argmax ? 8u : 0u) |
                                ((!fused && mode == 1) ? 32u : 0u) | (fused ? batch0 << 8 : 0u) | ((fused && sh.contiguous) ? 1u << 16 : 0u) |
                                ((fused && T == 1 && m->engine_on()) ? 1u << 17 : 0u) | (split_head_env_on() ? 0u : 1u << 18) |
-                               ((!fused && (size_t)sh.nseq * m->d.num_head >= 768) ? 1u << 19 : 0u) | (a.score ? 1u << 20 : 0u);
+                               ((!fused && (size_t)sh.nseq * m->d.num_head >= 768) ? 1u << 19 : 0u) | (a.score ? 1u << 20 : 0u) |
+                               ((fused && !fuse_tail_env_on()) ? 1u << 21 : 0u);
         const wrk_v7_model::GraphKey key{st->uid, T, flags, NH};
         if (!m->graphs.count(key) && m->graphs.size() > 64) { WRK_HIP(ctx, hipStreamSynchronize(ctx->stream)); m->drop_graphs(); }
         wrk_program* prog = nullptr;
@@ -462,7 +467,7 @@
     }
     if (rc == WRK_OK) rc = wrk_job_read_back(*m, m->s, V, a);
     if (rc != WRK_OK || ctx->capturing_here()) return rc;
-    return wrk_v7_engine_check(m->engine);
+    return m->engine_check();
 }
 
 int32_t wrk_v7_infer(wrk_ctx* ctx, wrk_v7_model* m, wrk_v7_state* st, const uint32_t* tokens, const uint16_t* emb_rows,
@@ -541,7 +546,7 @@
     if (rc != WRK_OK) return rc;
     WRK_LAUNCH_CHECK(ctx);
     WRK_HIP(ctx, hipStreamSynchronize(ctx->stream));
-    return wrk_v7_engine_check(m->engine);
+    return m->engine_check();
 }
 
 int32_t wrk_v7_frame_read(wrk_ctx* ctx, wrk_v7_model* m, const char* name, uint32_t T, void* dst, size_t capacity, size_t* bytes) {
@@ -555,7 +560,7 @@
         {"att_vx", s.vx, D}, {"att_ax", s.ax, D}, {"att_gx", s.gx, D}, {"att_r", s.r, D}, {"att_w", s.w, D}, {"att_k", s.k, D}, {"att_v", s.v, D},
         {"att_a", s.a, D}, {"att_g", s.g, D}, {"att_o", s.o, D}, {"att_kk", s.kk, D}, {"att_vv", s.vv, D}, {"att_n", s.n, 4 * D},
         {"aux_w", s.aux_w, m->d.lora_w}, {"aux_a", s.aux_a, m->d.lora_a}, {"aux_g", s.aux_g, m->d.lora_g}, {"aux_v", s.aux_v, m->d.lora_v},
-        {"ffn_x", s.ffn_x, D}, {"ffn_kx", s.ffn_kx, D}, {"ffn_k", s.ffn_k, F}, {"ffn_v", s.ffn_v, D}, {"att_x_ln", s.ln_tmp, D}};
+        {"ffn_x", s.ffn_x, D}, {"ffn_kx", s.ffn_kx, D}, {"ffn_k", s.ffn_k, F}, {"ffn_v", s.ffn_v, D}, {"att_x_ln", s.ln_tmp, D}, {"head_x", s.head_x, D}};
     const size_t esz = m->act_dtype == WRK_F32 ? 4 : 2;
     for (auto& e : tab)
         if (strcmp(e.n, name) == 0) {
@@ -592,7 +597,8 @@
 }
 
 uint32_t wrk_v7_model::key_bits(uint32_t B, uint32_t mode) const {
-    return mode | (act_dtype == WRK_F32 ? 4u : 0u) | ((B == 1 && mode == 1 && engine_on()) ? 8u : 0u) | (split_head_env_on() ? 0u : 16u);
+    return mode | (act_dtype == WRK_F32 ? 4u : 0u) | ((B == 1 && mode == 1 && engine_on()) ? 8u : 0u) | (split_head_env_on() ? 0u : 16u) |
+           (fuse_tail_env_on() ? 0u : 32u);
 }
 
 int32_t wrk_v7_model::lane(uint32_t g, uint32_t groups, wrk_frame_common** out) {
@@ -622,9 +628,9 @@
 int32_t wrk_v7_model::after_loop(uint32_t groups) {
     wrk::timing_report(ctx);
     for (uint32_t g = 0; g < groups; ++g) {
-        wrk_v7_engine* e = (g == 0 ? this : lanes[g - 1])->engine;
-        wrk_v7_engine_report(e);
-        const int32_t rc = wrk_v7_engine_check(e);
+        wrk_v7_model* lm = g == 0 ? this : lanes[g - 1];
+        wrk_v7_engine_report(lm->engine);
+        const int32_t rc = lm->engine_check();
         if (rc != WRK_OK) return rc;
     }
     return WRK_OK;
@@ -675,6 +681,12 @@
 
 static bool engine_env_on() { const char* e = getenv("WRK_ENGINE"); return !(e && e[0] == '0'); }
 bool engine_env_on_public() { return engine_env_on(); }
+bool fuse_tail_env_on() { const char* e = getenv("WRK_FUSE_TAIL"); return !(e && e[0] == '0'); }
+int32_t wrk_v7_model::engine_check() {
+    const int32_t rc = wrk_v7_engine_check(engine);
+    if (rc != WRK_OK && s.head_ticket) hipMemset(s.head_ticket, 0, head_ticket_bytes);
+    return rc;
+}
 bool wrk_v7_model::engine_on() const { return engine != nullptr && !engine_blocked && engine_env_on() && act_dtype == WRK_F16; }
 int32_t wrk_v7_model::ensure_engine() {
     if (engine_tried || !engine_env_on() || act_dtype != WRK_F16) return WRK_OK;
diff --git a/web-rwkv-gguf_amd/csrc/wrk_v7_engine.h b/web-rwkv-gguf_amd/csrc/wrk_v7_engine.h
--- a/web-rwkv-gguf_amd/csrc/wrk_v7_engine.h
+++ b/web-rwkv-gguf_amd/csrc/wrk_v7_engine.h
@@ -104,7 +104,8 @@
 int32_t wrk_v7_engine_create(wrk_v7_model* m, wrk_v7_engine** out);
 void wrk_v7_engine_destroy(wrk_v7_engine* e);
 int32_t wrk_v7_engine_enqueue(wrk_v7_engine* e, hipStream_t q, wrk_v7_state* st, uint32_t batch, uint32_t l0, uint32_t l1, const void* x_in,
-                              void* x_out, void* v_first, const uint32_t* token = nullptr);
+                              void* x_out, void* v_first, const uint32_t* token = nullptr, bool head_resets = false);
+void* wrk_v7_engine_granules(const wrk_v7_engine* e, uint32_t* vec16);
 bool wrk_v7_engine_has_table(const wrk_v7_engine* e);
 int wrk_v7_engine_waves(const wrk_v7_engine* e);
 int32_t wrk_v7_engine_check(wrk_v7_engine* e);
diff --git a/web-rwkv-gguf_amd/csrc/wrk_v7_engine.hip b/web-rwkv-gguf_amd/csrc/wrk_v7_engine.hip
--- a/web-rwkv-gguf_amd/csrc/wrk_v7_engine.hip
+++ b/web-rwkv-gguf_amd/csrc/wrk_v7_engine.hip
@@ -936,6 +936,7 @@
     if ((er = hipMalloc((void**)&e->wg_head, hh.size() * 4)) != hipSuccess) return fail_alloc(er);
     if ((er = hipMemcpy(e->wg_head, hh.data(), hh.size() * 4, hipMemcpyHostToDevice)) != hipSuccess) return fail_alloc(er);
     if ((er = hipMalloc((void**)&e->gran, (size_t)S.g_total * 8)) != hipSuccess) return fail_alloc(er);
+    if ((er = hipMemset(e->gran, 0, (size_t)S.g_total * 8)) != hipSuccess) return fail_alloc(er);
     if ((er = hipMalloc((void**)&e->fail, 256)) != hipSuccess) return fail_alloc(er);
     if ((er = hipMemset(e->fail, 0, 256)) != hipSuccess) return fail_alloc(er);
     const char* tm = getenv("WRK_TIMING");
@@ -998,7 +999,7 @@
 }
 
 int32_t wrk_v7_engine_enqueue(wrk_v7_engine* e, hipStream_t q, wrk_v7_state* st, uint32_t batch, uint32_t l0, uint32_t l1, const void* x_in, void* x_out,
-                              void* v_first, const uint32_t* token) {
+                              void* v_first, const uint32_t* token, bool head_resets) {
     using namespace wrk;
     wrk_ctx* ctx = e->m->ctx;
     EngArgs A{};
@@ -1007,11 +1008,16 @@
     A.layers = e->layers; A.vecs = e->vecs; A.scal = e->scal; A.gran = e->gran; A.x_in = x_in; A.x_out = x_out; A.v_first = v_first;
     if (token && e->emb_ln && l0 == 0) { A.x_in = e->emb_ln; A.x_row = token; }
     A.state = st->data; A.num_batch = st->num_batch; A.fail = e->fail; A.stamps = e->stamps; A.stamp_layer = std::min(5u, l1 - 1);
-    WRK_HIP(ctx, hipMemsetAsync(e->gran, 0, (size_t)e->S.g_total * 8, q));
     const dim3 grid(e->S.nwg), block((e->ncw + 2) * 64);
     hipLaunchKernelGGL(eng_kernel(e->xd, e->r16, e->ncw), grid, block, e->S.lds_total, q, A, (const uint32_t*)e->wg_head);
     WRK_LAUNCH_CHECK(ctx);
+    if (!head_resets) WRK_HIP(ctx, hipMemsetAsync(e->gran, 0, (size_t)e->S.g_total * 8, q));
     return WRK_OK;
+}
+
+void* wrk_v7_engine_granules(const wrk_v7_engine* e, uint32_t* vec16) {
+    *vec16 = e->S.g_total / 2;
+    return e->gran;
 }
 
 int32_t wrk_v7_engine_check(wrk_v7_engine* e) {
@@ -1021,6 +1027,7 @@
     WRK_HIP(ctx, hipMemcpy(&f, e->fail, 4, hipMemcpyDeviceToHost));
     if (f) {
         hipMemset(e->fail, 0, 4);
+        hipMemset(e->gran, 0, (size_t)e->S.g_total * 8);
         return wrk_fail(ctx, WRK_E_HIP, "decode engine: a hand-off wait gave up (stage mask 0x%x): workgroups not co-resident or a producer died", f);
     }
     return WRK_OK;
diff --git a/web-rwkv-gguf_amd/csrc/wrk_v7_fused.hip b/web-rwkv-gguf_amd/csrc/wrk_v7_fused.hip
--- a/web-rwkv-gguf_amd/csrc/wrk_v7_fused.hip
+++ b/web-rwkv-gguf_amd/csrc/wrk_v7_fused.hip
@@ -486,6 +486,16 @@
         if (ln_mix(q, P, n) != 0) return wrk_fail(ctx, WRK_E_UNSUPPORTED, "ln_mix shape");   \
     } while (0)
 
+    auto head_tail_job = [&]() {
+        MatJob j = mat_job(head, make_dense(s.x, WRK_F16, D, 1), make_dense(s.head_o, WRK_F32, V, 1), WRK_ACT_NONE);
+        j.pro = 3; j.pro_eps = 1.0e-5f; j.ln_w = ln_out_w->ptr; j.ln_b = ln_out_b->ptr; j.ln_out = s.head_x;
+        return j;
+    };
+    bool tail_fused = false;
+    if (fuse_tail_env_on() && T == 1 && NH == 1 && identity_headers && D <= 4096) {
+        const MatJob j = head_tail_job();
+        tail_fused = matvec_num_wg(&j, 1, ctx->num_cu, nullptr) <= s.head_cand_cap && matvec_head_tail(q, j, HeadTail{}, ctx->num_cu, true) == 0;
+    }
     if (T >= 2 && s.ks_cnt && s.ks_cnt_cap) WRK_HIP(ctx, hipMemsetAsync(s.ks_cnt, 0, (size_t)s.ks_cnt_cap * 4, q));
     const bool eng_embeds = T == 1 && from_tokens && !skip_embed && layer_begin == 0 && engine_on() && !engine_skip_once && wrk_v7_engine_has_table(engine) &&
                             d.num_layer > 0;
@@ -498,10 +508,12 @@
         LN(P, T);
     }
     uint32_t first_launch_layer = layer_begin;
+    bool head_resets = false;
     if (T == 1 && engine_on() && !engine_skip_once) {
         const uint32_t l1 = std::min<uint32_t>(d.num_layer, layer_end);
         if (layer_begin < l1) {
-            const int32_t rc = wrk_v7_engine_enqueue(engine, q, st, cursor0_batch, layer_begin, l1, s.x, s.x, s.att_v0, eng_embeds ? s.tokens : nullptr);
+            head_resets = tail_fused;
+            const int32_t rc = wrk_v7_engine_enqueue(engine, q, st, cursor0_batch, layer_begin, l1, s.x, s.x, s.att_v0, eng_embeds ? s.tokens : nullptr, head_resets);
             if (rc != WRK_OK) return rc;
         }
         first_launch_layer = l1;
@@ -629,7 +641,16 @@
         }
         if ((li + 1) % d.rescale == 0) wrk::affine(q, vec(s.x), 0.5f, 0.0f);
     }
-    if (NH > 0) {
+    if (NH > 0 && tail_fused) {
+        MatJob j = head_tail_job();
+        HeadTail t;
+        if (head_resets) t.zero = wrk_v7_engine_granules(engine, &t.zero_vec);
+        if (want_argmax) {
+            t.cand = s.head_cand; t.ticket = s.head_ticket; t.argmax = s.argmax;
+            if (advance) { t.tokens = s.tokens; t.history = history; t.counter = s.counter; }
+        }
+        if (matvec_head_tail(q, j, t, ctx->num_cu) != 0) return wrk_fail(ctx, WRK_E_ARG, "fused head rejected");
+    } else if (NH > 0) {
         LnMixParams P{};
         P.src = (const f16*)s.x; P.ids = identity_headers ? nullptr : s.headers;
         P.ln_w = (const f16*)ln_out_w->ptr; P.ln_b = (const f16*)ln_out_b->ptr; P.eps = 1.0e-5f;
```

Result: faster. 1745 tokens/s, median of 5 (+1.9%).
